# DakeQQ/Text-to-Speech-TTS-ONNX

Hardware: AMD Instinct MI355X
Metric: audio_seconds_per_second (higher is better)
Workload: dtype f32

## Files before the change

### text-to-speech-tts-onnx_amd/csrc/attention.hip

```cpp
#include "common.h"
#include <functional>
#include <map>
#include <mutex>
#include "mfma.h"
#include "f5_kernels.h"
#include "x3_split.h"
#include <type_traits>
#include <string>
#include <algorithm>

namespace mi {

#define ATTN_XCD_MAP                                                                          \
    int bx_ = (int)blockIdx.x, by_ = (int)blockIdx.y;                                         \
    if (xmap) {                                                                               \
        const int l2 = bx_ + (int)gridDim.x * by_, slot = l2 >> 3;                            \
        by_ = (l2 & 7) + 8 * (slot / (int)gridDim.x);                                         \
        bx_ = slot % (int)gridDim.x;                                                          \
    }

#define ATTN_VARLEN_PROLOGUE                                                                  \
    const int NL = VARLEN ? lens[(bh / H) >> 1] : N;                                          \
    const bool dead = VARLEN && (SPLIT2 ? bx_ * 64 : bx_ * 128) >= NL;                        \
    if (dead && blockIdx.z != 0) return;
// ... 226 lines not shown
            } else {
#pragma unroll
                for (int s2 = 0; s2 < 2; ++s2) {
                    T pb[8];
#pragma unroll
                    for (int e = 0; e < 8; ++e) pb[e] = from_f32<T>(p[8 * s2 + e]);
                    const typename MF::Frag bfrag = *reinterpret_cast<const typename MF::Frag*>(pb);
#pragma unroll
                    for (int dt = 0; dt < 2; ++dt) {
                        const T* row = Vs + (dt * 32 + lr) * LDV + kt * 32 + 16 * s2 + 4 * hi;
                        uint2 a2[2];
                        a2[0] = *reinterpret_cast<const uint2*>(row);
                        a2[1] = *reinterpret_cast<const uint2*>(row + 8);
                        oacc[dt] = MF::mma(*reinterpret_cast<const typename MF::Frag*>(a2), bfrag, oacc[dt]);
                    }
                }
            }
        };
        if constexpr (SPLIT2) {
            if (st * KT + (wave & 1) * 32 < NL) tile(wave & 1);
        } else {
#pragma unroll
            for (int kt = 0; kt < KT / 32; ++kt) {
                const int key0 = st * KT + kt * 32;
                if (key0 < NL) tile(kt);
            }
        }
        __syncthreads();
        if (st + 1 < nstage) {
            store_lds();
            __syncthreads();
        }
    }

    bool owner = true;
    if constexpr (SPLIT2) {
        __syncthreads();
        float* comb = reinterpret_cast<float*>(smem);
        float* stats = comb + 2 * 32 * 64;
        static_assert(sizeof(smem) >= (2 * 32 * 64 + 2 * 64 * 2 + 4) * sizeof(float), "merge buffer fits the stage");
        const int grp = wave >> 1;
        owner = !(wave & 1);
        if (!owner) {
            stats[(grp * 64 + lane) * 2] = m_run; stats[(grp * 64 + lane) * 2 + 1] = l_run;
#pragma unroll
            for (int dt = 0; dt < 2; ++dt)
#pragma unroll
                for (int r = 0; r < 16; ++r) comb[((grp * 2 + dt) * 16 + r) * 64 + lane] = oacc[dt][r];
        }
        __syncthreads();
        if (owner) {
            const float m1 = stats[(grp * 64 + lane) * 2], l1 = stats[(grp * 64 + lane) * 2 + 1];
            const float m = fmaxf(m_run, m1);
            const float s0 = m_run == -INFINITY ? 0.f : __builtin_amdgcn_exp2f(m_run - m);
            const float s1 = m1 == -INFINITY ? 0.f : __builtin_amdgcn_exp2f(m1 - m);
            l_run = l_run * s0 + l1 * s1;
            m_run = m;
#pragma unroll
            for (int dt = 0; dt < 2; ++dt)
#pragma unroll
                for (int r = 0; r < 16; ++r) oacc[dt][r] = oacc[dt][r] * s0 + comb[((grp * 2 + dt) * 16 + r) * 64 + lane] * s1;
        }
        const int Z = (int)gridDim.z;
        if (Z > 1) {
            const int z = (int)blockIdx.z;
            const int unit = (int)(by_ * gridDim.x + bx_);
            constexpr int SLOT = 2 * 32 * 64 + 2 * 64 * 2;
            typedef unsigned int u4 __attribute__((ext_vector_type(4)));
            typedef unsigned int u2 __attribute__((ext_vector_type(2)));
            __amdgpu_buffer_rsrc_t rsw = __builtin_amdgcn_make_buffer_rsrc((void*)(ws + (long)unit * Z * SLOT), 0, Z * SLOT * 4, 0x00020000);
            if (owner) {
#pragma unroll
                for (int dt = 0; dt < 2; ++dt)
#pragma unroll
                    for (int g4 = 0; g4 < 4; ++g4) {
                        u4 val;
                        val.x = __float_as_uint(oacc[dt][4 * g4]); val.y = __float_as_uint(oacc[dt][4 * g4 + 1]);
                        val.z = __float_as_uint(oacc[dt][4 * g4 + 2]); val.w = __float_as_uint(oacc[dt][4 * g4 + 3]);
                        __builtin_amdgcn_raw_buffer_store_b128(val, rsw, (z * SLOT + (((grp * 2 + dt) * 4 + g4) * 64 + lane) * 4) * 4, 0, 16);
                    }
                u2 st2; st2.x = __float_as_uint(m_run); st2.y = __float_as_uint(l_run);
                __builtin_amdgcn_raw_buffer_store_b64(st2, rsw, (z * SLOT + 2 * 32 * 64 + (grp * 64 + lane) * 2) * 4, 0, 16);
            }
            asm volatile("s_waitcnt vmcnt(0)" ::: "memory");
            __syncthreads();
            int* ticket = reinterpret_cast<int*>(stats + 2 * 64 * 2);
            if (tid == 0) *ticket = __hip_atomic_fetch_add(cnt + unit, 1, __ATOMIC_RELAXED, __HIP_MEMORY_SCOPE_AGENT);
            __syncthreads();
            if (*ticket != Z - 1) return;
            if (tid == 0) __hip_atomic_store(cnt + unit, 0, __ATOMIC_RELAXED, __HIP_MEMORY_SCOPE_AGENT);
            if (!owner) return;
            float mz[4], lz[4], M = -INFINITY;
#pragma unroll
            for (int zz = 0; zz < 4; ++zz) {
                mz[zz] = -INFINITY; lz[zz] = 0.f;
                if (zz < Z) {
                    if (zz == z) { mz[zz] = m_run; lz[zz] = l_run; }
                    else {
                        const u2 st2 = __builtin_amdgcn_raw_buffer_load_b64(rsw, (zz * SLOT + 2 * 32 * 64 + (grp * 64 + lane) * 2) * 4, 0, 16);
                        mz[zz] = __uint_as_float(st2.x); lz[zz] = __uint_as_float(st2.y);
                    }
                    M = fmaxf(M, mz[zz]);
                }
            }
            f32x16 osum[2];
#pragma unroll
            for (int r = 0; r < 16; ++r) { osum[0][r] = 0.f; osum[1][r] = 0.f; }
            float lsum = 0.f;
#pragma unroll
            for (int zz = 0; zz < 4; ++zz) {
                if (zz >= Z) break;
                const float sc = mz[zz] == -INFINITY ? 0.f : __builtin_amdgcn_exp2f(mz[zz] - M);
                lsum += lz[zz] * sc;
                if (zz == z) {
#pragma unroll
                    for (int dt = 0; dt < 2; ++dt)
#pragma unroll
                        for (int r = 0; r < 16; ++r) osum[dt][r] += oacc[dt][r] * sc;
                } else {
#pragma unroll
                    for (int dt = 0; dt < 2; ++dt)
#pragma unroll
                        for (int g4 = 0; g4 < 4; ++g4) {
                            const u4 val = __builtin_amdgcn_raw_buffer_load_b128(rsw, (zz * SLOT + (((grp * 2 + dt) * 4 + g4) * 64 + lane) * 4) * 4, 0, 16);
                            osum[dt][4 * g4] += __uint_as_float(val.x) * sc; osum[dt][4 * g4 + 1] += __uint_as_float(val.y) * sc;
                            osum[dt][4 * g4 + 2] += __uint_as_float(val.z) * sc; osum[dt][4 * g4 + 3] += __uint_as_float(val.w) * sc;
                        }
                }
            }
            oacc[0] = osum[0]; oacc[1] = osum[1];
            l_run = lsum;
        }
    }
    if (!owner) return;
    const int qr = q0 + lr;
    if (qr < N) {
        const float inv = VARLEN && qr >= NL ? 0.f : 1.0f / l_run;
        const int b = bh / H, h = bh - b * H;
        T* ob = o + ((long)b * N + qr) * H * D + h * D;
#pragma unroll
        for (int dt = 0; dt < 2; ++dt)
#pragma unroll
            for (int g = 0; g < 4; ++g) {
                T vals[4];
#pragma unroll
                for (int e = 0; e < 4; ++e) vals[e] = from_f32<T>(oacc[dt][g * 4 + e] * inv);
                T* dst = ob + dt * 32 + 8 * g + 4 * hi;
                if constexpr (sizeof(T) == 4) *reinterpret_cast<uint4*>(dst) = *reinterpret_cast<const uint4*>(vals);
                else *reinterpret_cast<uint2*>(dst) = *reinterpret_cast<const uint2*>(vals);
            }
    }
}

#if defined(MI355TTS_ATTN_TRACE)
#define TSTAMP(v) do { __builtin_amdgcn_sched_barrier(0); asm volatile("s_memtime %0\n\ts_waitcnt lgkmcnt(0)" : "=s"(v) :: "memory"); __builtin_amdgcn_sched_barrier(0); } while (0)
#define TACC(k, t1, t0) tr_[k] += (t1) - (t0)
#else
#define TSTAMP(v) do { } while (0)
#define TACC(k, t1, t0) do { } while (0)
#endif
template <bool SPLIT2, bool KVP = false, int NP = 3, bool VARLEN = false>
__global__ __launch_bounds__(256, NP == 2 ? 3 : 2) void attn_x3f_kernel(const float* __restrict__ q, const float* __restrict__ k,
                                                       const float* __restrict__ v, float* __restrict__ o, int H, int N,
                                                       float* __restrict__ ws, int* __restrict__ cnt,
                                                       unsigned char* __restrict__ o_planes, int o_np, int xmap = 0,
                                                       int cut1 = 0, int cut2 = 0, int cut3 = 0, const int* __restrict__ lens = nullptr) {
    ATTN_XCD_MAP
    static_assert(NP == 3 || (NP == 2 && KVP), "attn_x3f: the two-plane form reads pre-split K / V");
    using MF = std::conditional_t<NP == 3, Mfma<bf16>, Mfma<f16>>;
    using Frag = typename MF::Frag;
    constexpr int D = 64, KT = 64;
    constexpr int LDK = D + 8, LDV = KT + 4;
    constexpr int KPL = KT * LDK, VPL = D * LDV;
    __shared__ __attribute__((aligned(16))) bf16 smem[NP * KPL + NP * VPL];
    static_assert(sizeof(smem) >= (2 * 32 * 64 + 2 * 64 * 2 + 4) * sizeof(float), "merge buffer fits the stage");
    bf16* Ks = smem;
    bf16* Vs = smem + NP * KPL;

    const int tid = threadIdx.x, wave = tid >> 6, lane = tid & 63, lr = lane & 31, hi = lane >> 5;
    const int bh = by_;
    ATTN_VARLEN_PROLOGUE
    const int q0 = SPLIT2 ? bx_ * 64 + (wave >> 1) * 32 : bx_ * 128 + wave * 32;
    const float* qb = q + (long)bh * N * D;
    const float* kb = k + (long)bh * N * D;
    const long vld = KVP ? (long)((N + 63) / 64 * 64) : (long)((N + 7) / 8 * 8);
    const float* vb = v + (long)bh * D * vld;
    const bf16* kpb = reinterpret_cast<const bf16*>(k) + (long)bh * NP * vld * D;
    const bf16* vpb = reinterpret_cast<const bf16*>(v) + (long)bh * NP * D * vld;

    auto split4 = [&](const float4 a, uint2& w1, uint2& w2, uint2& w3) __attribute__((always_inline)) {
        x3_split_pair(a.x, a.y, w1.x, w2.x, w3.x);
        x3_split_pair(a.z, a.w, w1.y, w2.y, w3.y);
    };
    auto split8 = [&](const float4 a, const float4 b, Frag& f1, Frag& f2, Frag& f3) __attribute__((always_inline)) {
        uint2 a1, a2, a3, b1, b2, b3;
        split4(a, a1, a2, a3); split4(b, b1, b2, b3);
        f1 = __builtin_bit_cast(Frag, x3_u4{a1.x, a1.y, b1.x, b1.y});
        f2 = __builtin_bit_cast(Frag, x3_u4{a2.x, a2.y, b2.x, b2.y});
        f3 = __builtin_bit_cast(Frag, x3_u4{a3.x, a3.y, b3.x, b3.y});
    };

    auto split8h = [&](const float4 a, const float4 b, Frag& f1, Frag& f2) __attribute__((always_inline)) {
        unsigned h[4], l[4];
        x2u_split_pair(a.x, a.y, h[0], l[0]); x2u_split_pair(a.z, a.w, h[1], l[1]);
        x2u_split_pair(b.x, b.y, h[2], l[2]); x2u_split_pair(b.z, b.w, h[3], l[3]);
        f1 = __builtin_bit_cast(Frag, x3_u4{h[0], h[1], h[2], h[3]});
        f2 = __builtin_bit_cast(Frag, x3_u4{l[0], l[1], l[2], l[3]});
    };
    auto split8p = [&](const float4 a, const float4 b, Frag& f1, Frag& f2) __attribute__((always_inline)) {
        unsigned h[4], l[4];
        x2u_split_pair_raw_mix(a.x, a.y, h[0], l[0]); x2u_split_pair_raw_mix(a.z, a.w, h[1], l[1]);
        x2u_split_pair_raw_mix(b.x, b.y, h[2], l[2]); x2u_split_pair_raw_mix(b.z, b.w, h[3], l[3]);
        f1 = __builtin_bit_cast(Frag, x3_u4{h[0], h[1], h[2], h[3]});
        f2 = __builtin_bit_cast(Frag, x3_u4{l[0], l[1], l[2], l[3]});
    };

    Frag qf3[4][NP];
    {
        const int qr = q0 + lr;
        const bool ok = qr < NL;
        constexpr float L2E = 1.4426950408889634f;
#pragma unroll
        for (int ks = 0; ks < 4; ++ks) {
            float4 a = float4{0.f, 0.f, 0.f, 0.f}, b = a;
            if (ok) {
                a = *reinterpret_cast<const float4*>(qb + (long)qr * D + ks * 16 + hi * 8);
                b = *reinterpret_cast<const float4*>(qb + (long)qr * D + ks * 16 + hi * 8 + 4);
            }
            a.x *= L2E; a.y *= L2E; a.z *= L2E; a.w *= L2E; b.x *= L2E; b.y *= L2E; b.z *= L2E; b.w *= L2E;
            if constexpr (NP == 3) split8(a, b, qf3[ks][0], qf3[ks][1], qf3[ks][2]); else split8h(a, b, qf3[ks][0], qf3[ks][1]);
        }
    }

    float4 kreg[KVP ? 1 : 4], vreg[KVP ? 1 : 4];
    constexpr int NU = 2 * NP;
    x3_u4 kpl[KVP ? NU : 1], vpl[KVP ? NU : 1];
    auto load_regs = [&](int key0) {
        if constexpr (KVP) {
#pragma unroll
            for (int i = 0; i < NU; ++i) {
                const int u = tid + i * 256, pl = u >> 9, r = (u & 511) >> 3, c = u & 7;
                kpl[i] = *reinterpret_cast<const x3_u4*>(kpb + ((long)pl * vld + key0 + r) * D + c * 8);
                vpl[i] = *reinterpret_cast<const x3_u4*>(vpb + ((long)pl * D + r) * vld + key0 + c * 8);
            }
            if (key0 + KT > NL) {
#pragma unroll
                for (int i = 0; i < NU; ++i) {
                    const int keep = NL - (key0 + ((tid + i * 256) & 7) * 8);
                    if (keep < 8) {
                        unsigned w[4] = {vpl[i].x, vpl[i].y, vpl[i].z, vpl[i].w};
#pragma unroll
                        for (int e = 0; e < 4; ++e) w[e] &= (2 * e < keep ? 0x0000ffffu : 0u) | (2 * e + 1 < keep ? 0xffff0000u : 0u);
                        vpl[i] = x3_u4{w[0], w[1], w[2], w[3]};
                    }
                }
            }
        } else {
#pragma unroll
        for (int i = 0; i < 4; ++i) {
            const int vi = tid + i * 256;
            const int key = vi >> 4, dv = vi & 15;
            const int d = vi >> 4, kv = vi & 15;
            float4 a = float4{0.f, 0.f, 0.f, 0.f}, b = a;
            if (key0 + key < NL) a = *reinterpret_cast<const float4*>(kb + (long)(key0 + key) * D + dv * 4);
            if (key0 + kv * 4 < NL) b = *reinterpret_cast<const float4*>(vb + (long)d * vld + key0 + kv * 4);
            if constexpr (VARLEN) {
                const int keep = NL - (key0 + kv * 4);
                if (keep < 2) b.y = 0.f;
                if (keep < 3) b.z = 0.f;
                if (keep < 4) b.w = 0.f;
            }
            kreg[i] = a; vreg[i] = b;
        }
        }
    };
    auto store_lds = [&]() {
        if constexpr (KVP) {
#pragma unroll
            for (int i = 0; i < NU; ++i) {
                const int u = tid + i * 256, pl = u >> 9, r = (u & 511) >> 3, c = u & 7;
                *reinterpret_cast<x3_u4*>(Ks + pl * KPL + r * LDK + c * 8) = kpl[i];
                uint2* vd = reinterpret_cast<uint2*>(Vs + pl * VPL + r * LDV + c * 8);
                vd[0] = uint2{vpl[i].x, vpl[i].y}; vd[1] = uint2{vpl[i].z, vpl[i].w};
            }
        } else {
#pragma unroll
        for (int i = 0; i < 4; ++i) {
            const int vi = tid + i * 256;
            const int r = vi >> 4, c = vi & 15;
            uint2 w1, w2, w3;
            split4(kreg[i], w1, w2, w3);
            *reinterpret_cast<uint2*>(Ks + r * LDK + c * 4) = w1;
            *reinterpret_cast<uint2*>(Ks + KPL + r * LDK + c * 4) = w2;
            *reinterpret_cast<uint2*>(Ks + 2 * KPL + r * LDK + c * 4) = w3;
            split4(vreg[i], w1, w2, w3);
            *reinterpret_cast<uint2*>(Vs + r * LDV + c * 4) = w1;
            *reinterpret_cast<uint2*>(Vs + VPL + r * LDV + c * 4) = w2;
            *reinterpret_cast<uint2*>(Vs + 2 * VPL + r * LDV + c * 4) = w3;
        }
        }
    };

    f32x16 oacc[2];
#pragma unroll
    for (int r = 0; r < 16; ++r) { oacc[0][r] = 0.f; oacc[1][r] = 0.f; }
    float m_run = -INFINITY, l_run = 0.f;
#if defined(MI355TTS_ATTN_TRACE)
    unsigned long long tr_[8] = {0, 0, 0, 0, 0, 0, 0, 0}, ta_ = 0, tb_ = 0, tc_ = 0, td_ = 0, te_ = 0, tk_ = 0;
    TSTAMP(tk_);
#endif

    const int nstage_all = dead ? 0 : (NL + KT - 1) / KT;
    int st0 = (int)((long)blockIdx.z * nstage_all / gridDim.z);
    int nstage = (int)((long)(blockIdx.z + 1) * nstage_all / gridDim.z);
    if (cut1 > 0) {
        const int zz = (int)blockIdx.z, ZZ = (int)gridDim.z;
        st0 = zz == 0 ? 0 : zz == 1 ? cut1 : zz == 2 ? cut2 : cut3;
        nstage = zz + 1 == ZZ ? nstage_all : zz == 0 ? cut1 : zz == 1 ? cut2 : cut3;
    }
    if constexpr (VARLEN) { st0 = min(st0, nstage_all); nstage = min(nstage, nstage_all); }
    if (st0 < nstage) {
        load_regs(st0 * KT);
        store_lds();
        __syncthreads();
    }
    constexpr int TA[6] = {0, 1, 2, 0, 1, 0}, TB[6] = {2, 1, 0, 1, 0, 0};
    for (int st = st0; st < nstage; ++st) {
        if (st + 1 < nstage) load_regs((st + 1) * KT);
        auto tile = [&](int kt) {
            const int key0 = st * KT + kt * 32;
            TSTAMP(ta_);
            f32x16 sacc;
#pragma unroll
            for (int r = 0; r < 16; ++r) sacc[r] = 0.f;
#pragma unroll
            for (int ks = 0; ks < 4; ++ks) {
                Frag kf[NP];
#pragma unroll
                for (int pl = 0; pl < NP; ++pl)
                    kf[pl] = *reinterpret_cast<const Frag*>(Ks + pl * KPL + (kt * 32 + lr) * LDK + ks * 16 + hi * 8);
                if constexpr (NP == 3) {
#pragma unroll
                    for (int t = 0; t < 6; ++t) sacc = MF::mma(kf[TA[t]], qf3[ks][TB[t]], sacc);
                } else {
                    sacc = MF::mma(kf[1], qf3[ks][0], sacc);
                    sacc = MF::mma(kf[0], qf3[ks][1], sacc);
                    sacc = MF::mma(kf[0], qf3[ks][0], sacc);
                }
            }
            if (key0 + 32 > NL) {
#pragma unroll
                for (int r = 0; r < 16; ++r) {
                    const int key = key0 + (r & 3) + 8 * (r >> 2) + 4 * hi;
                    if (key >= NL) sacc[r] = -INFINITY;
                }
            }
            float mloc = -INFINITY;
#pragma unroll
            for (int r = 0; r < 16; ++r) mloc = fmaxf(mloc, sacc[r]);
            mloc = xor32_max(mloc);
#if defined(MI355TTS_ATTN_TRACE)
            { const float keep_ = mloc; asm volatile("" :: "v"(keep_)); }
#endif
            TSTAMP(tb_); TACC(0, tb_, ta_);
            float alpha = 1.f;
            if (!__all(mloc - m_run <= 8.0f)) {
                const float m_new = fmaxf(m_run, mloc);
                alpha = __builtin_amdgcn_exp2f(m_run - m_new);
                m_run = m_new;
#pragma unroll
                for (int r = 0; r < 16; ++r) { oacc[0][r] *= alpha; oacc[1][r] *= alpha; }
            }
            typedef float f2 __attribute__((ext_vector_type(2)));
            float p[16];
            f2 ls2 = f2{0.f, 0.f};
            const f2 m2 = f2{m_run, m_run};
#pragma unroll
            for (int r = 0; r < 16; r += 2) {
                const f2 dd = f2{sacc[r], sacc[r + 1]} - m2;
                const f2 e = f2{__builtin_amdgcn_exp2f(dd.x), __builtin_amdgcn_exp2f(dd.y)};
                p[r] = e.x; p[r + 1] = e.y;
                ls2 += e;
            }
            float lsum = ls2.x + ls2.y;
            lsum = xor32_sum(lsum);
            l_run = l_run * alpha + lsum;
#if defined(MI355TTS_ATTN_TRACE)
            { const float keep_ = l_run + p[0] + p[15]; asm volatile("" :: "v"(keep_)); }
#endif
            TSTAMP(tc_); TACC(1, tc_, tb_);
#pragma unroll
            for (int s2 = 0; s2 < 2; ++s2) {
                Frag pf[NP];
                if constexpr (NP == 3)
                    split8(float4{p[8 * s2], p[8 * s2 + 1], p[8 * s2 + 2], p[8 * s2 + 3]},
                           float4{p[8 * s2 + 4], p[8 * s2 + 5], p[8 * s2 + 6], p[8 * s2 + 7]}, pf[0], pf[1], pf[2]);
                else
                    split8p(float4{p[8 * s2], p[8 * s2 + 1], p[8 * s2 + 2], p[8 * s2 + 3]},
                            float4{p[8 * s2 + 4], p[8 * s2 + 5], p[8 * s2 + 6], p[8 * s2 + 7]}, pf[0], pf[1]);
                Frag vf[2][NP];
#pragma unroll
                for (int dt = 0; dt < 2; ++dt)
#pragma unroll
                    for (int pl = 0; pl < NP; ++pl) {
                        const bf16* row = Vs + pl * VPL + (dt * 32 + lr) * LDV + kt * 32 + 16 * s2 + 4 * hi;
                        uint2 a2[2];
                        a2[0] = *reinterpret_cast<const uint2*>(row);
                        a2[1] = *reinterpret_cast<const uint2*>(row + 8);
                        vf[dt][pl] = __builtin_bit_cast(Frag, x3_u4{a2[0].x, a2[0].y, a2[1].x, a2[1].y});
                    }
                if constexpr (NP == 3) {
#pragma unroll
                    for (int t = 0; t < 6; ++t)
#pragma unroll
                        for (int dt = 0; dt < 2; ++dt) oacc[dt] = MF::mma(vf[dt][TA[t]], pf[TB[t]], oacc[dt]);
                } else {
                    oacc[0] = MF::mma(vf[0][1], pf[0], oacc[0]);
                    oacc[1] = MF::mma(vf[1][1], pf[0], oacc[1]);
                    oacc[0] = MF::mma(vf[0][0], pf[1], oacc[0]);
                    oacc[1] = MF::mma(vf[1][0], pf[1], oacc[1]);
                    oacc[0] = MF::mma(vf[0][0], pf[0], oacc[0]);
                    oacc[1] = MF::mma(vf[1][0], pf[0], oacc[1]);
                }
            }
            TSTAMP(td_); TACC(2, td_, tc_);
        };
        if constexpr (SPLIT2) {
            if (st * KT + (wave & 1) * 32 < NL) tile(wave & 1);
        } else {
#pragma unroll
            for (int kt = 0; kt < KT / 32; ++kt) {
                const int key0 = st * KT + kt * 32;
                if (key0 < NL) tile(kt);
            }
        }
        TSTAMP(ta_);
        __syncthreads();
        TSTAMP(tb_); TACC(3, tb_, ta_);
        if (st + 1 < nstage) {
            store_lds();
            TSTAMP(tc_); TACC(4, tc_, tb_);
            __syncthreads();
            TSTAMP(te_); TACC(5, te_, tc_);
        }
    }
#if defined(MI355TTS_ATTN_TRACE)
    TSTAMP(te_);
    if (blockIdx.x == 3 && blockIdx.y == 5 && (threadIdx.x & 63) == 0)
        printf("ATTN_TRACE z %d wave %d stages %d total %llu | S+max %llu exp %llu PV %llu bar1 %llu store %llu bar2 %llu\n", (int)blockIdx.z, wave, nstage - st0,
               te_ - tk_, tr_[0], tr_[1], tr_[2], tr_[3], tr_[4], tr_[5]);
#endif
    bool owner = true;
    constexpr int NG = SPLIT2 ? 2 : 4;
    int grp = wave;
    float* comb = reinterpret_cast<float*>(smem);
    float* stats = comb + 2 * 32 * 64;
    if constexpr (SPLIT2) {
        __syncthreads();
        grp = wave >> 1;
        owner = !(wave & 1);
        if (!owner) {
            stats[(grp * 64 + lane) * 2] = m_run; stats[(grp * 64 + lane) * 2 + 1] = l_run;
#pragma unroll
            for (int dt = 0; dt < 2; ++dt)
#pragma unroll
                for (int r = 0; r < 16; ++r) comb[((grp * 2 + dt) * 16 + r) * 64 + lane] = oacc[dt][r];
        }
        __syncthreads();
        if (owner) {
            const float m1 = stats[(grp * 64 + lane) * 2], l1 = stats[(grp * 64 + lane) * 2 + 1];
            const float m = fmaxf(m_run, m1);
            const float s0 = m_run == -INFINITY ? 0.f : __builtin_amdgcn_exp2f(m_run - m);
            const float s1 = m1 == -INFINITY ? 0.f : __builtin_amdgcn_exp2f(m1 - m);
            l_run = l_run * s0 + l1 * s1;
            m_run = m;
#pragma unroll
            for (int dt = 0; dt < 2; ++dt)
#pragma unroll
                for (int r = 0; r < 16; ++r) oacc[dt][r] = oacc[dt][r] * s0 + comb[((grp * 2 + dt) * 16 + r) * 64 + lane] * s1;
        }
    }
    {
        const int Z = (int)gridDim.z;
        if (Z > 1 && !dead) {
            const int z = (int)blockIdx.z;
            const int unit = (int)(by_ * gridDim.x + bx_);
            constexpr int SLOT = NG * (32 * 64 + 64 * 2);
            typedef unsigned int u4 __attribute__((ext_vector_type(4)));
            typedef unsigned int u2 __attribute__((ext_vector_type(2)));
            __amdgpu_buffer_rsrc_t rsw = __builtin_amdgcn_make_buffer_rsrc((void*)(ws + (long)unit * Z * SLOT), 0, Z * SLOT * 4, 0x00020000);
            if (owner) {
#pragma unroll
                for (int dt = 0; dt < 2; ++dt)
#pragma unroll
                    for (int g4 = 0; g4 < 4; ++g4) {
                        u4 val;
                        val.x = __float_as_uint(oacc[dt][4 * g4]); val.y = __float_as_uint(oacc[dt][4 * g4 + 1]);
                        val.z = __float_as_uint(oacc[dt][4 * g4 + 2]); val.w = __float_as_uint(oacc[dt][4 * g4 + 3]);
                        __builtin_amdgcn_raw_buffer_store_b128(val, rsw, (z * SLOT + (((grp * 2 + dt) * 4 + g4) * 64 + lane) * 4) * 4, 0, 16);
                    }
                u2 st2; st2.x = __float_as_uint(m_run); st2.y = __float_as_uint(l_run);
                __builtin_amdgcn_raw_buffer_store_b64(st2, rsw, (z * SLOT + NG * 32 * 64 + (grp * 64 + lane) * 2) * 4, 0, 16);
            }
            asm volatile("s_waitcnt vmcnt(0)" ::: "memory");
            __syncthreads();
            int* ticket = reinterpret_cast<int*>(stats + 2 * 64 * 2);
            if (tid == 0) *ticket = __hip_atomic_fetch_add(cnt + unit, 1, __ATOMIC_RELAXED, __HIP_MEMORY_SCOPE_AGENT);
            __syncthreads();
            if (*ticket != Z - 1) return;
            if (tid == 0) __hip_atomic_store(cnt + unit, 0, __ATOMIC_RELAXED, __HIP_MEMORY_SCOPE_AGENT);
            if (!owner) return;
            float mz[4], lz[4], M = -INFINITY;
#pragma unroll
            for (int zz = 0; zz < 4; ++zz) {
                mz[zz] = -INFINITY; lz[zz] = 0.f;
                if (zz < Z) {
                    if (zz == z) { mz[zz] = m_run; lz[zz] = l_run; }
                    else {
                        const u2 st2 = __builtin_amdgcn_raw_buffer_load_b64(rsw, (zz * SLOT + NG * 32 * 64 + (grp * 64 + lane) * 2) * 4, 0, 16);
                        mz[zz] = __uint_as_float(st2.x); lz[zz] = __uint_as_float(st2.y);
                    }
                    M = fmaxf(M, mz[zz]);
                }
            }
            f32x16 osum[2];
#pragma unroll
            for (int r = 0; r < 16; ++r) { osum[0][r] = 0.f; osum[1][r] = 0.f; }
            float lsum = 0.f;
#pragma unroll
            for (int zz = 0; zz < 4; ++zz) {
                if (zz >= Z) break;
                const float sc = mz[zz] == -INFINITY ? 0.f : __builtin_amdgcn_exp2f(mz[zz] - M);
                lsum += lz[zz] * sc;
                if (zz == z) {
#pragma unroll
                    for (int dt = 0; dt < 2; ++dt)
#pragma unroll
                        for (int r = 0; r < 16; ++r) osum[dt][r] += oacc[dt][r] * sc;
                } else {
#pragma unroll
                    for (int dt = 0; dt < 2; ++dt)
#pragma unroll
                        for (int g4 = 0; g4 < 4; ++g4) {
                            const u4 val = __builtin_amdgcn_raw_buffer_load_b128(rsw, (zz * SLOT + (((grp * 2 + dt) * 4 + g4) * 64 + lane) * 4) * 4, 0, 16);
                            osum[dt][4 * g4] += __uint_as_float(val.x) * sc; osum[dt][4 * g4 + 1] += __uint_as_float(val.y) * sc;
                            osum[dt][4 * g4 + 2] += __uint_as_float(val.z) * sc; osum[dt][4 * g4 + 3] += __uint_as_float(val.w) * sc;
                        }
                }
            }
            oacc[0] = osum[0]; oacc[1] = osum[1];
            l_run = lsum;
        }
    }
    if (!owner) return;
    const int qr = q0 + lr;
    if (qr < N) {
        const float inv = VARLEN && qr >= NL ? 0.f : 1.0f / l_run;
        const int b = bh / H, h = bh - b * H;
        float* ob = o + ((long)b * N + qr) * H * D + h * D;
        const long row = (long)b * N + qr;
#pragma unroll
        for (int dt = 0; dt < 2; ++dt)
#pragma unroll
            for (int g = 0; g < 4; ++g) {
                float vals[4];
#pragma unroll
                for (int e = 0; e < 4; ++e) vals[e] = (oacc[dt][g * 4 + e] * inv);
                if (o_planes) {
                    uint2 w1, w2, w3;
                    unsigned char* dst = o_planes + x3p_slot_offset(row, h * 8 + dt * 4 + g, (H * D) >> 5, o_np) + 8 * hi;
                    if (o_np == 3) {
                        x3_split_pair(vals[0], vals[1], w1.x, w2.x, w3.x);
                        x3_split_pair(vals[2], vals[3], w1.y, w2.y, w3.y);
                        *reinterpret_cast<uint2*>(dst + 2 * X3P_PLANE) = w3;
                    } else {
                        x2_split_pair(vals[0], vals[1], w1.x, w2.x);
                        x2_split_pair(vals[2], vals[3], w1.y, w2.y);
                    }
                    *reinterpret_cast<uint2*>(dst) = w1;
                    *reinterpret_cast<uint2*>(dst + X3P_PLANE) = w2;
                } else {
                    float* dst = ob + dt * 32 + 8 * g + 4 * hi;
                    *reinterpret_cast<uint4*>(dst) = *reinterpret_cast<const uint4*>(vals);
                }
            }
    }
}

static inline int opt_attn_x3() { const int o = arith_tls().attn_x3; return o >= 0 ? o : (int)opt(OPT_ATTN_F32_X3); }
static inline int opt_attn_np() { const int o = arith_tls().attn_np; return (o == 2 || o == 3) ? o : (int)opt(OPT_ATTN_F32_PLANES); }
long attention_v_ld(int N, int dtype) {
    return (dtype == MI_F32 && opt_attn_x3() != 2) ? 0 : (long)((N + 7) / 8 * 8);
}
bool attention_takes_kv_planes(int N, int BH, int dtype) {
    (void)N; (void)BH;
    return dtype == MI_F32 && opt_attn_x3() == 2 && opt(OPT_ATTN_KV_PLANES) != 0;
}

int attention_kv_planes_format() { return opt_attn_np(); }

bool attention_can_write_planes(int N, int BH, int dtype) {
    (void)N; (void)BH;
    return dtype == MI_F32 && opt_attn_x3() == 2;
}

struct AttnSlices { int Z = 1, cut[3] = {0, 0, 0}; };
static AttnSlices attn_pick_slices(long units, int S, int slots, int zmax) {
    AttnSlices best;
    double best_t = 1e30;
    auto makespan = [&](const int* len, int Z) -> double {
        std::map<double, long> free_at;
        free_at[0.0] = slots;
        double end = 0.0;
        for (int z = 0; z < Z; ++z) {
            const double cost = len[z] + (Z > 1 ? 0.6 : 0.3);
            long left = units;
            while (left > 0) {
                auto it = free_at.begin();
                const long take = std::min(left, it->second);
                const double t = it->first + cost;
                it->second -= take;
                if (it->second == 0) free_at.erase(it);
                free_at[t] += take;
                end = std::max(end, t);
                left -= take;
            }
        }
        return end;
    };
    int len[4];
    for (int Z = 1; Z <= zmax; ++Z) {
        if (S < 2 * Z && Z > 1) break;
        std::function<void(int, int, int)> rec = [&](int i, int left, int cap) {
            if (i == Z - 1) {
                if (left < 1 || left > cap) return;
                len[i] = left;
                const double t = makespan(len, Z);
                if (t < best_t - 1e-9) {
                    best_t = t; best.Z = Z;
                    int acc = 0;
                    for (int c = 0; c < 3; ++c) { acc += c < Z ? len[c] : 0; best.cut[c] = c + 1 < Z ? acc : S; }
                }
                return;
            }
            for (int a = std::min(cap, left - (Z - 1 - i)); a >= (left + (Z - i) - 1) / (Z - i); --a) { len[i] = a; rec(i + 1, left - a, a); }
        };
        rec(0, S, S);
    }
    return best;
}

template <bool SPLIT2, bool KVP, int NP>
static void go_x3f(dim3 grid, hipStream_t s, const void* q, const void* k, const void* v, void* o, int H, int N, float* ws, int* cnt,
                   void* o_planes, int o_np, int xm, int c1, int c2, int c3, const int* lens) {
    const float *qf = (const float*)q, *kf = (const float*)k, *vf = (const float*)v;
    if (lens) prof_kernel_suffix(" + lengths");
    if (lens) hipLaunchKernelGGL((attn_x3f_kernel<SPLIT2, KVP, NP, true>), grid, dim3(256), 0, s, qf, kf, vf, (float*)o, H, N, ws, cnt, (unsigned char*)o_planes, o_np, xm, c1, c2, c3, lens);
    else hipLaunchKernelGGL((attn_x3f_kernel<SPLIT2, KVP, NP>), grid, dim3(256), 0, s, qf, kf, vf, (float*)o, H, N, ws, cnt, (unsigned char*)o_planes, o_np, xm, c1, c2, c3);
}
template <typename T, bool SPLIT2, bool X3S = false, bool REFH = false>
static void go_attn(dim3 grid, hipStream_t s, const void* q, const void* k, const void* v, void* o, int H, int N, float* ws, int* cnt,
                    float sscale, int xm, const int* lens) {
    const T *qt = (const T*)q, *kt = (const T*)k, *vt = (const T*)v;
    if (lens) prof_kernel_suffix(" + lengths");
    if (lens) hipLaunchKernelGGL((attn_kernel<T, SPLIT2, X3S, REFH, true>), grid, dim3(256), 0, s, qt, kt, vt, (T*)o, H, N, ws, cnt, sscale, xm, lens);
    else hipLaunchKernelGGL((attn_kernel<T, SPLIT2, X3S, REFH>), grid, dim3(256), 0, s, qt, kt, vt, (T*)o, H, N, ws, cnt, sscale, xm);
}

void launch_attention(const void* q, const void* k, const void* v, void* o, int BH, int H, int N, int dtype, hipStream_t s,
                      float* ws, long ws_floats, int* cnt, long cnt_n, void* o_planes, int kv_planes, int o_np, float ref_fp16_scale,
                      const int* lens) {
    MI_REQUIRE(ref_fp16_scale == 0.f || (dtype == MI_F16 && ref_fp16_scale > 0.f), "attention: the reference-fp16 score form needs f16 operands");
    MI_REQUIRE(o_np == 2 || o_np == 3, "attention: 2 or 3 output planes");
    MI_REQUIRE(!o_planes || attention_can_write_planes(N, BH, dtype), "attention: panel-plane output needs the fp32 split kernel");
    MI_REQUIRE(!kv_planes || attention_can_write_planes(N, BH, dtype), "attention: pre-split K / V need the fp32 split kernel");
    MI_REQUIRE(kv_planes == 0 || kv_planes == 1 || kv_planes == 2 || kv_planes == 3, "attention: kv_planes is 0, 2 or 3 (1 = 3)");
    MI_REQUIRE(BH % H == 0 && N > 0, "attention: bad shape");
    const double esz = (double)dtype_size(dtype);
    ProfScope ps(FAM_ATTN, s, 4.0 * BH * N * 64.0 * esz, 4.0 * BH * (double)N * N * 64.0);
#define ATTN_LAUNCH(TT, SP, GRID, SSCALE, XM)                                    \
    do {                                                                        \
        prof_set_kernel("attn_kernel<T, " #SP ">", type_label<TT>());           \
        go_attn<TT, SP>(GRID, s, q, k, v, o, H, N, ws, cnt, SSCALE, XM, lens);  \
    } while (0)
    const int xm = (opt(OPT_ATTN_XCD_MAP) != 0 && BH % 8 == 0) ? 1 : 0;
    const int zmax = opt(OPT_ATTN_Z);
    auto pick_z = [&](int zlimit16, bool wide = false) -> int {
        const long units = (long)(wide ? (N + 127) / 128 : (N + 63) / 64) * BH;
        const long slot = wide ? 4 * (32 * 64 + 64 * 2) : 2 * 32 * 64 + 2 * 64 * 2;
        const int nstage = (N + 63) / 64;
        int dev = 0, cus = 256;
        MI_HIP(hipGetDevice(&dev));
        {
            static int cu_count[16] = {0};
            if (!cu_count[dev & 15]) { hipDeviceProp_t pr; MI_HIP(hipGetDeviceProperties(&pr, dev)); cu_count[dev & 15] = pr.multiProcessorCount; }
            cus = cu_count[dev & 15];
        }
        if (opt(OPT_ATTN_Z_FORCE) > 0)
            return (ws && cnt && units * opt(OPT_ATTN_Z_FORCE) * slot <= ws_floats && units <= cnt_n) ? (int)opt(OPT_ATTN_Z_FORCE) : 1;
        int Z = 1;
        double best = 1e30;
        const int zm = dtype == MI_F32 ? zmax : std::min(zmax, zlimit16);
        for (int z = 1; z <= zm; ++z) {
            if (z > 1 && (!ws || !cnt || units * z * slot > ws_floats || units > cnt_n || nstage < 2 * z)) break;
            const double cost = (double)((units * z + cus - 1) / cus) / z * (1.0 + (dtype == MI_F32 ? 0.09 : 0.06) * (z - 1));
            if (cost < best - 1e-9) { best = cost; Z = z; }
        }
        return Z;
    };
    const int z16 = opt(OPT_ATTN_Z16);
    if (dtype == MI_F32) {
        if (opt(OPT_ATTN_SPLIT) && (long)((N + 127) / 128) * BH < 1024 && N >= 64) {
            const bool wide = opt(OPT_ATTN_SPLIT) == 2 && opt_attn_x3() == 2 && kv_planes == 2;
            const int Z = pick_z(1, wide);
            if (wide) {
                AttnSlices sl;
                sl.Z = Z;
                if (opt(OPT_ATTN_LPT) && opt(OPT_ATTN_Z_FORCE) == 0 && Z >= 1 && ws && cnt) {
                    static std::mutex mu;
                    static std::map<std::pair<int, int>, AttnSlices> cache;
                    std::lock_guard<std::mutex> lk(mu);
                    auto key = std::make_pair(N, BH);
                    auto it = cache.find(key);
                    if (it == cache.end()) {
                        int dev = 0, cus = 256;
                        MI_HIP(hipGetDevice(&dev));
                        hipDeviceProp_t pr; MI_HIP(hipGetDeviceProperties(&pr, dev)); cus = pr.multiProcessorCount;
                        const long units = (long)((N + 127) / 128) * BH;
                        const long slot = 4 * (32 * 64 + 64 * 2);
                        int zm = std::min((int)opt(OPT_ATTN_Z), 4);
                        while (zm > 1 && (units * zm * slot > ws_floats || units > cnt_n)) --zm;
                        it = cache.emplace(key, attn_pick_slices(units, (N + 63) / 64, 3 * cus, zm)).first;
                    }
                    sl = it->second;
                    if (const AttnCuts& e = opt_attn_cuts(); e.n) {
                        const int S = (N + 63) / 64, n = e.n;
                        const int* c = e.c;
                        const long units = (long)((N + 127) / 128) * BH;
                        if (n >= 1 && c[0] > 0 && c[0] < S && units * (n + 1) * 4 * (32 * 64 + 64 * 2) <= ws_floats && units <= cnt_n) {
                            sl.Z = n + 1; sl.cut[0] = c[0]; sl.cut[1] = n >= 2 ? c[1] : S; sl.cut[2] = n >= 3 ? c[2] : S;
                        }
                    }
                }
                prof_set_kernel("attn_x3f_kernel<false, pre-split K V, fp16 pairs> + key slices", "", "");
                go_x3f<false, true, 2>(dim3((N + 127) / 128, BH, sl.Z), s, q, k, v, o, H, N, ws, cnt, o_planes, o_np, xm,
                                       sl.Z > 1 ? sl.cut[0] : 0, sl.cut[1], sl.cut[2], lens);
            } else if (opt_attn_x3() == 2) {
                if (kv_planes == 2) {
                    prof_set_kernel("attn_x3f_kernel<true, pre-split K V, fp16 pairs>", "", "");
                    go_x3f<true, true, 2>(dim3((N + 63) / 64, BH, Z), s, q, k, v, o, H, N, ws, cnt, o_planes, o_np, xm, 0, 0, 0, lens);
                } else if (kv_planes) {
                    prof_set_kernel("attn_x3f_kernel<true, pre-split K V>", "", "");
                    go_x3f<true, true, 3>(dim3((N + 63) / 64, BH, Z), s, q, k, v, o, H, N, ws, cnt, o_planes, o_np, 0, 0, 0, 0, lens);
                } else {
                prof_set_kernel("attn_x3f_kernel<true>", "", "");
                go_x3f<true, false, 3>(dim3((N + 63) / 64, BH, Z), s, q, k, v, o, H, N, ws, cnt, o_planes, o_np, 0, 0, 0, 0, lens);
                }
            } else if (opt_attn_x3() == 1) {
                prof_set_kernel("attn_kernel<float, true, x3>", "", "");
                go_attn<float, true, true>(dim3((N + 63) / 64, BH, Z), s, q, k, v, o, H, N, ws, cnt, 1.f, 0, lens);
            } else
                ATTN_LAUNCH(float, true, dim3((N + 63) / 64, BH, Z), 1.f, 0);
        } else if (opt_attn_x3() == 2) {
            if (kv_planes == 2) {
                prof_set_kernel("attn_x3f_kernel<false, pre-split K V, fp16 pairs>", "", "");
                go_x3f<false, true, 2>(dim3((N + 127) / 128, BH), s, q, k, v, o, H, N, ws, cnt, o_planes, o_np, xm, 0, 0, 0, lens);
            } else if (kv_planes) {
                prof_set_kernel("attn_x3f_kernel<false, pre-split K V>", "", "");
                go_x3f<false, true, 3>(dim3((N + 127) / 128, BH), s, q, k, v, o, H, N, ws, cnt, o_planes, o_np, 0, 0, 0, 0, lens);
            } else {
            prof_set_kernel("attn_x3f_kernel<false>", "", "");
            go_x3f<false, false, 3>(dim3((N + 127) / 128, BH), s, q, k, v, o, H, N, ws, cnt, o_planes, o_np, 0, 0, 0, 0, lens);
            }
        } else if (opt_attn_x3() == 1) {
            prof_set_kernel("attn_kernel<float, false, x3>", "", "");
            go_attn<float, false, true>(dim3((N + 127) / 128, BH), s, q, k, v, o, H, N, ws, cnt, 1.f, 0, lens);
        } else
            ATTN_LAUNCH(float, false, dim3((N + 127) / 128, BH), 1.f, 0);
    } else {
        const bool sp = opt(OPT_ATTN_SPLIT) && (long)((N + 127) / 128) * BH < 512 && N >= 64;
        const dim3 grid(sp ? (N + 63) / 64 : (N + 127) / 128, BH, sp ? pick_z(z16) : 1);
        if (dtype == MI_F16 && ref_fp16_scale != 0.f) {
            prof_set_kernel(sp ? "attn_kernel<T, true, reference-fp16 scores>" : "attn_kernel<T, false, reference-fp16 scores>", type_label<f16>());
            if (sp) go_attn<f16, true, false, true>(grid, s, q, k, v, o, H, N, ws, cnt, ref_fp16_scale, 0, lens);
            else go_attn<f16, false, false, true>(grid, s, q, k, v, o, H, N, ws, cnt, ref_fp16_scale, 0, lens);
        } else if (dtype == MI_F16) {
            if (sp) ATTN_LAUNCH(f16, true, grid, 1.f, xm);
            else ATTN_LAUNCH(f16, false, grid, 1.f, xm);
        } else {
            if (sp) ATTN_LAUNCH(bf16, true, grid, 1.f, xm);
            else ATTN_LAUNCH(bf16, false, grid, 1.f, xm);
        }
    }
#undef ATTN_LAUNCH
    MI_HIP(hipGetLastError());
}

}
```

### text-to-speech-tts-onnx_amd/csrc/capi.hip

```cpp
#include "common.h"
#include "bigvgan.h"
#include "f5.h"
#include "gpt.h"
#include "cond.h"
#include <algorithm>
#include <mutex>
#include <exception>

using namespace mi;

struct mi_bigvgan { BigVGAN* impl; std::mutex mu; };
struct mi_f5 { F5* impl; std::mutex mu; };
struct mi_gpt { Gpt* impl; std::mutex mu; };
struct mi_cond { Cond* impl; std::mutex mu; };

template <typename F> static int guard(F&& f, bool exclusive = false) {
    try {
        options_init();
        std::shared_lock<std::shared_mutex> rd(option_lock(), std::defer_lock);
        std::unique_lock<std::shared_mutex> wr(option_lock(), std::defer_lock);
        if (exclusive) wr.lock(); else rd.lock();
        f();
        return MI_OK;
    } catch (const mi::Error& e) {
// ... 121 lines not shown

int mi_bigvgan_forward_latent(mi_bigvgan* h, const float* latent, int T_codes, const float* conds, int64_t n_conds,
                              int16_t* out, float* out_f32, int mem) {
    return guard([&] {
        MI_REQUIRE(h && h->impl, "mi_bigvgan_forward_latent: null handle");
        std::lock_guard<std::mutex> lk_(h->mu);
        MI_REQUIRE(mem == MI_HOST || mem == MI_DEVICE, "mi_bigvgan_forward_latent: bad mem kind");
        h->impl->run_latent(latent, T_codes, conds, (long)n_conds, out_f32, out, mem);
    });
}

static std::vector<int> bigvgan_lengths(const int64_t* lens, int B, int64_t lo, const char* what) {
    MI_REQUIRE(lens && B >= 1, what);
    std::vector<int> v(B);
    for (int b = 0; b < B; ++b) {
        MI_REQUIRE(lens[b] >= lo && lens[b] < (1L << 30), what);
        v[b] = (int)lens[b];
    }
    return v;
}

int mi_bigvgan_forward_ragged(mi_bigvgan* h, int B, const float* mel, const int64_t* frames, int16_t* out_i16, float* out_f32,
                              int64_t out_cap, int64_t* out_lens, int mem) {
    return guard([&] {
        MI_REQUIRE(h && h->impl, "mi_bigvgan_forward_ragged: null handle");
        std::lock_guard<std::mutex> lk_(h->mu);
        MI_REQUIRE(mem == MI_HOST || mem == MI_DEVICE, "mi_bigvgan_forward_ragged: bad mem kind");
        MI_REQUIRE(out_i16, "mi_bigvgan_forward_ragged: null out_i16");
        const std::vector<int> F = bigvgan_lengths(frames, B, 1, "mi_bigvgan_forward_ragged: B >= 1 items of >= 1 frames");
        h->impl->run_ragged(mel, B, F.data(), out_f32, out_i16, (long)out_cap, out_lens, mem);
    });
}

int mi_bigvgan_forward_latent_ragged(mi_bigvgan* h, int B, const float* latent, const int64_t* t_codes, const float* conds,
                                     int64_t n_conds, int16_t* out_i16, float* out_f32, int64_t out_cap, int64_t* out_lens, int mem) {
    return guard([&] {
        MI_REQUIRE(h && h->impl, "mi_bigvgan_forward_latent_ragged: null handle");
        std::lock_guard<std::mutex> lk_(h->mu);
        MI_REQUIRE(mem == MI_HOST || mem == MI_DEVICE, "mi_bigvgan_forward_latent_ragged: bad mem kind");
        MI_REQUIRE(out_i16, "mi_bigvgan_forward_latent_ragged: null out_i16");
        const std::vector<int> T = bigvgan_lengths(t_codes, B, 3, "mi_bigvgan_forward_latent_ragged: B >= 1 items of >= 3 latent rows");
        h->impl->run_latent_ragged(latent, B, T.data(), conds, (long)n_conds, out_f32, out_i16, (long)out_cap, out_lens, mem);
    });
}

int mi_aa_activation1d(const float* x, int B, int C, int T, const float* alpha_log, const float* beta_log,
                       int logscale, int post, int dtype, float* y) {
    return guard([&] {
        MI_REQUIRE(x && y && alpha_log && beta_log && B > 0 && C > 0 && T > 0, "mi_aa_activation1d: bad arguments");
        unit_aa_activation1d(x, B, C, T, alpha_log, beta_log, logscale, post, dtype, y);
    });
}

int mi_aa_conv1d(const float* x, int B, int C, int T, const float* alpha_log, const float* beta_log, int logscale,
                 const float* w, const float* bias, int k, int dilation, const float* res, int dtype, float* y) {
    return guard([&] {
        MI_REQUIRE(x && y && w && bias && alpha_log && beta_log && B > 0 && C > 0 && T > 0 && k > 0 && (k & 1) && dilation > 0,
                   "mi_aa_conv1d: bad arguments");
        unit_aa_conv1d(x, B, C, T, alpha_log, beta_log, logscale, w, bias, k, dilation, res, dtype, 1, y);
    });
}

int mi_conv1d(const float* x, int B, int Cin, int T, const float* w, const float* bias, int Cout, int k, int dilation,
              int padding, int groups, int dtype, float* y) {
    return guard([&] {
        MI_REQUIRE(x && w && y && B > 0 && Cin > 0 && Cout > 0 && T > 0 && k > 0 && dilation > 0 && groups > 0 && padding >= 0,
                   "mi_conv1d: bad arguments");
        unit_conv1d(x, B, Cin, T, w, bias, Cout, k, dilation, padding, groups, dtype, y);
    });
}

int mi_conv_transpose1d(const float* x, int B, int Cin, int T, const float* w, const float* bias, int Cout, int k,
                        int stride, int padding, int dtype, float* y) {
    return guard([&] {
        MI_REQUIRE(x && w && y && B > 0 && Cin > 0 && Cout > 0 && T > 0, "mi_conv_transpose1d: bad arguments");
        unit_conv_transpose1d(x, B, Cin, T, w, bias, Cout, k, stride, padding, dtype, y);
    });
}

int64_t mi_f5_param_count(const int32_t* cfg_i, int n_i, const float* cfg_f, int n_f) {
    int64_t n = -1;
    int rc = guard([&] { n = f5_param_count(parse_f5_cfg(cfg_i, n_i, cfg_f, n_f)); });
    return rc == MI_OK ? n : (int64_t)rc;
}

mi_f5* mi_f5_create(const int32_t* cfg_i, int n_i, const float* cfg_f, int n_f, const float* weights, int64_t n_weights,
                    int dtype, int device) {
    mi_f5* h = nullptr;
    int rc = guard([&] {
        MI_REQUIRE(weights != nullptr, "mi_f5_create: null weights");
        F5Cfg c = parse_f5_cfg(cfg_i, n_i, cfg_f, n_f);
        F5* impl = new F5(c, weights, n_weights, dtype, device);
        h = new mi_f5; h->impl = impl;
    });
    return rc == MI_OK ? h : nullptr;
}

mi_f5* mi_f5_create_mem(const int32_t* cfg_i, int n_i, const float* cfg_f, int n_f, const float* weights, int64_t n_weights,
                        int dtype, int device, int mem) {
    mi_f5* h = nullptr;
    int rc = guard([&] {
        MI_REQUIRE(weights != nullptr && (mem == MI_HOST || mem == MI_DEVICE), "mi_f5_create_mem: null weights / bad mem kind");
        F5Cfg c = parse_f5_cfg(cfg_i, n_i, cfg_f, n_f);
        F5* impl = new F5(c, weights, n_weights, dtype, device, mem);
        h = new mi_f5; h->impl = impl;
    });
    return rc == MI_OK ? h : nullptr;
}

void mi_f5_destroy(mi_f5* h) {
    if (!h) return;
    delete h->impl;
    delete h;
}

struct F5Recover {
    F5* e; int n;
    explicit F5Recover(F5* e_) : e(e_), n(std::uncaught_exceptions()) {}
    ~F5Recover() { if (std::uncaught_exceptions() > n) e->recover(); }
};
#define F5_CHECK(h, mem, name)                                                     \
    MI_REQUIRE((h) && (h)->impl, name ": null handle");                            \
    std::lock_guard<std::mutex> lk_((h)->mu);                                      \
    F5Recover rec_((h)->impl);                                                     \
    ArithScope arith_((h)->impl->arith);                                           \
    MI_REQUIRE((mem) == MI_HOST || (mem) == MI_DEVICE, name ": bad mem kind")

static void copy_out(void* dst, const void* src, size_t bytes, int mem, hipStream_t s) {
    if (!dst) return;
    MI_HIP(hipMemcpyAsync(dst, src, bytes, mem == MI_HOST ? hipMemcpyDeviceToHost : hipMemcpyDeviceToDevice, s));
}

int mi_f5_tables(mi_f5* h, float* time_expand, float* delta_t) {
    return guard([&] {
        MI_REQUIRE(h && h->impl, "mi_f5_tables: null handle");
        std::lock_guard<std::mutex> lk_(h->mu);
        F5& e = *h->impl;
        if (time_expand) std::memcpy(time_expand, e.h_time_expand.data(), e.h_time_expand.size() * 4);
        if (delta_t) std::memcpy(delta_t, e.h_delta.data(), e.h_delta.size() * 4);
    });
}

int64_t mi_f5_info(mi_f5* h, const char* key) {
    int64_t v = -1;
    int rc = guard([&] {
        MI_REQUIRE(h && h->impl && key, "mi_f5_info: null handle / key");
        std::lock_guard<std::mutex> lk_(h->mu);
        F5& e = *h->impl;
        ArithScope as(e.arith);
        const std::string k(key);
        if (k == "f32_arithmetic") v = e.dtype != MI_F32 ? -1 : !gemm_x3_enabled() ? ARITH_NATIVE : (gemm_x3p_enabled() ? e.np : ARITH_BF16X3);
        else if (k == "saturation_events") v = e.sat_events;
        else if (k == "adaln_fold") v = (e.fold_built && e.cfg.ln_fold != 0) ? 1 : 0;
        else MI_REQUIRE(false, "mi_f5_info: unknown key");
    });
    return rc == MI_OK ? v : (int64_t)rc;
}

int mi_f5_preprocess(mi_f5* h, const int16_t* audio, int64_t L, const int32_t* text_ids, int64_t T, int64_t max_duration,
                     const float* noise_in, uint64_t seed, float* noise, float* rope_cos, float* rope_sin,
                     float* cat_mel_text, float* cat_mel_text_drop, int64_t* ref_signal_len, int mem) {
    return guard([&] {
        F5_CHECK(h, mem, "mi_f5_preprocess");
        F5& e = *h->impl;
        MI_REQUIRE(max_duration > 0 && max_duration <= e.cfg.max_len && T >= 0 && T < (1 << 20) && L > 0 && L < (1L << 31),
                   "mi_f5_preprocess: sizes");
        const int N = (int)max_duration;
        const int R = e.preprocess(1, audio, L, text_ids, (int)T, N, noise_in, seed, mem);
        hipStream_t s = e.stream;
        const size_t cd = e.cfg.cond_dim(), D = e.cfg.dim_head;
        copy_out(noise, e.d_noise.p, (size_t)N * e.cfg.mel * 4, mem, s);
        copy_out(rope_cos, e.rope_cos.p, (size_t)N * D * 4, mem, s);
        copy_out(rope_sin, e.rope_sin.p, (size_t)N * D * 4, mem, s);
        copy_out(cat_mel_text, e.d_cmt.p, (size_t)N * cd * 4, mem, s);
        copy_out(cat_mel_text_drop, e.d_cmtd.p, (size_t)N * cd * 4, mem, s);
        MI_HIP(hipStreamSynchronize(s));
        e.finish_call();
        if (ref_signal_len) *ref_signal_len = R;
    });
}

int mi_f5_transformer_step(mi_f5* h, float* noise, const float* cmt, const float* cmtd, int U, int64_t N,
                           int32_t* time_step, int fuse, int mem) {
    return guard([&] {
        F5_CHECK(h, mem, "mi_f5_transformer_step");
        MI_REQUIRE(noise && cmt && cmtd && time_step && fuse >= 1 && U >= 1 && N > 0, "mi_f5_transformer_step: bad arguments");
        F5& e = *h->impl;
        f5_run_checked(e, [&] {
            e.load_cond(noise, cmt, cmtd, U, (int)N, mem);
            e.build_cat_cond(U, (int)N);
            e.steps(U, (int)N, *time_step, fuse);
            MI_HIP(hipStreamSynchronize(e.stream));
        });
        copy_out(noise, e.d_noise.p, (size_t)U * N * e.cfg.mel * 4, mem, e.stream);
        MI_HIP(hipStreamSynchronize(e.stream));
        e.finish_call();
        *time_step += fuse;
    });
}

int mi_f5_sample(mi_f5* h, float* noise, const float* cmt, const float* cmtd, int U, int64_t N, int k0, int n_steps, int mem) {
    return guard([&] {
        F5_CHECK(h, mem, "mi_f5_sample");
        MI_REQUIRE(noise && cmt && cmtd && U >= 1 && N > 0, "mi_f5_sample: bad arguments");
        F5& e = *h->impl;
        f5_run_checked(e, [&] {
            e.load_cond(noise, cmt, cmtd, U, (int)N, mem);
            e.build_cat_cond(U, (int)N);
            e.steps(U, (int)N, k0, n_steps);
            MI_HIP(hipStreamSynchronize(e.stream));
        });
        copy_out(noise, e.d_noise.p, (size_t)U * N * e.cfg.mel * 4, mem, e.stream);
        MI_HIP(hipStreamSynchronize(e.stream));
        e.finish_call();
    });
}

int mi_f5_dit_eval(mi_f5* h, const float* noise, const float* cmt, const float* cmtd, int U, int64_t N, int k, float* pred, int mem) {
    return guard([&] {
        F5_CHECK(h, mem, "mi_f5_dit_eval");
        MI_REQUIRE(noise && cmt && cmtd && pred && U >= 1 && N > 0, "mi_f5_dit_eval: bad arguments");
        F5& e = *h->impl;
        f5_run_checked(e, [&] {
            e.load_cond(noise, cmt, cmtd, U, (int)N, mem);
            e.build_cat_cond(U, (int)N);
            e.dit_eval(U, (int)N, k);
            MI_HIP(hipStreamSynchronize(e.stream));
        });
        copy_out(pred, e.pred_rows(U, (int)N), (size_t)2 * U * N * e.cfg.mel * 4, mem, e.stream);
        MI_HIP(hipStreamSynchronize(e.stream));
        e.finish_call();
    });
}

int mi_f5_decode(mi_f5* h, const float* denoised, int U, int64_t N, int64_t ref_signal_len, int16_t* out, float* out_f32,
                 int64_t* out_len, int mem) {
    return guard([&] {
        F5_CHECK(h, mem, "mi_f5_decode");
        MI_REQUIRE(denoised && (out || out_f32) && U >= 1 && N > 0 && ref_signal_len >= 0 && ref_signal_len < N,
                   "mi_f5_decode: bad arguments");
        F5& e = *h->impl;
        e.load_cond(denoised, nullptr, nullptr, U, (int)N, mem);
        const long len = e.decode(e.d_noise.as<float>(), U, (int)N, (int)ref_signal_len, out_f32 ? e.v_outf.as<float>() : nullptr,
                                  out ? e.v_outi.as<int16_t>() : nullptr);
        copy_out(out, e.v_outi.p, (size_t)U * len * 2, mem, e.stream);
        copy_out(out_f32, e.v_outf.p, (size_t)U * len * 4, mem, e.stream);
        MI_HIP(hipStreamSynchronize(e.stream));
        e.finish_call();
        if (out_len) *out_len = len;
    });
}

int mi_f5_synthesize(mi_f5* h, int U, const int16_t* audio, int64_t L, const int32_t* text_ids, int64_t T,
                     int64_t max_duration, const float* noise_in, uint64_t seed, int16_t* out, int64_t* out_len, int mem) {
    return guard([&] {
        F5_CHECK(h, mem, "mi_f5_synthesize");
        MI_REQUIRE(audio && text_ids && out && U >= 1 && max_duration > 0, "mi_f5_synthesize: bad arguments");
        F5& e = *h->impl;
        const int N = (int)max_duration;
        long len = 0;
        f5_run_checked(e, [&] {
            const int R = e.preprocess(U, audio, L, text_ids, (int)T, N, noise_in, seed, mem);
            e.build_cat_cond(U, N);
            e.steps(U, N, 0, e.cfg.nfe - 1);
            len = e.decode(e.d_noise.as<float>(), U, N, R, nullptr, e.v_outi.as<int16_t>());
            copy_out(out, e.v_outi.p, (size_t)U * len * 2, mem, e.stream);
            MI_HIP(hipStreamSynchronize(e.stream));
        });
        e.finish_call();
        if (out_len) *out_len = len;
    });
}

int mi_f5_synthesize_mel(mi_f5* h, int U, const int16_t* audio, int64_t L, const int32_t* text_ids, int64_t T,
                         int64_t max_duration, const float* noise_in, uint64_t seed, float* mel_out, int64_t* n_frames, int mem) {
    return guard([&] {
        F5_CHECK(h, mem, "mi_f5_synthesize_mel");
        MI_REQUIRE(audio && text_ids && mel_out && U >= 1 && max_duration > 0, "mi_f5_synthesize_mel: bad arguments");
        F5& e = *h->impl;
        const int N = (int)max_duration;
        int F = 0;
        f5_run_checked(e, [&] {
            const int R = e.preprocess(U, audio, L, text_ids, (int)T, N, noise_in, seed, mem);
            const int mel = e.cfg.mel;
            F = N - R;
            MI_REQUIRE(F >= 1, "mi_f5_synthesize_mel: max_duration leaves no generated frames");
            e.build_cat_cond(U, N);
            e.steps(U, N, 0, e.cfg.nfe - 1);
            float* dst = mel_out;
            if (mem == MI_HOST) { e.v_outf.ensure((size_t)U * mel * F * 4); dst = e.v_outf.as<float>(); }
            for (int u = 0; u < U; ++u)
                launch_nlc_to_ncl(e.d_noise.as<float>() + ((size_t)u * N + R) * mel, dst + (size_t)u * mel * F, 1, mel, F, MI_F32, e.stream);
            if (mem == MI_HOST) copy_out(mel_out, dst, (size_t)U * mel * F * 4, mem, e.stream);
            MI_HIP(hipStreamSynchronize(e.stream));
        });
        e.finish_call();
        if (n_frames) *n_frames = F;
    });
}

static std::vector<int> f5_lengths(const int64_t* lens, int U, int64_t lo, int64_t hi, const char* what) {
    MI_REQUIRE(lens && U >= 1, what);
    std::vector<int> v(U);
    for (int u = 0; u < U; ++u) {
        MI_REQUIRE(lens[u] >= lo && lens[u] <= hi, what);
        v[u] = (int)lens[u];
// ... 566 lines not shown
```

### text-to-speech-tts-onnx_amd/csrc/common.h

```cpp
#pragma once
#include <hip/hip_runtime.h>
#include <hip/hip_fp16.h>
#include <cstdint>
#include <cstdio>
#include <cstring>
#include <cmath>
#include <string>
#include <vector>
#include <stdexcept>
#include <map>
#include <shared_mutex>

#include "../../include/mi355tts.h"
#include "options.h"

namespace mi {

struct Error : std::runtime_error {
    int code;
    Error(int c, const std::string& m) : std::runtime_error(m), code(c) {}
};
void set_last_error(const std::string& m);

#define MI_HIP(expr)                                                                              \
    do {                                                                                          \
        hipError_t _e = (expr);                                                                   \
        if (_e != hipSuccess)                                                                     \
            throw mi::Error(MI_EHIP, std::string(#expr) + ": " + hipGetErrorString(_e) + " @" +   \
                                         __FILE__ + ":" + std::to_string(__LINE__));              \
    } while (0)

#define MI_REQUIRE(cond, msg)                                                                     \
    do {                                                                                          \
        if (!(cond)) throw mi::Error(MI_EINVAL, std::string(msg) + " [" #cond "]");               \
    } while (0)

using f16 = _Float16;
using bf16 = __bf16;

template <typename T> struct DT;
template <> struct DT<float> { static constexpr int id = MI_F32; };
template <> struct DT<f16>   { static constexpr int id = MI_F16; };
template <> struct DT<bf16>  { static constexpr int id = MI_BF16; };

inline size_t dtype_size(int dt) { return dt == MI_F32 ? 4 : 2; }

template <typename T> __host__ __device__ inline float to_f32(T v) { return (float)v; }
template <typename T> __host__ __device__ inline T from_f32(float v) { return (T)v; }

struct DevBuf {
    void* p = nullptr;
    size_t bytes = 0;
    DevBuf() = default;
    DevBuf(const DevBuf&) = delete;
    DevBuf& operator=(const DevBuf&) = delete;
    DevBuf(DevBuf&& o) noexcept : p(o.p), bytes(o.bytes) { o.p = nullptr; o.bytes = 0; }
    DevBuf& operator=(DevBuf&& o) noexcept {
        if (this != &o) { release(); p = o.p; bytes = o.bytes; o.p = nullptr; o.bytes = 0; }
        return *this;
    }
    ~DevBuf() { release(); }
    void release() { if (p) { (void)hipFree(p); p = nullptr; bytes = 0; } }
    void ensure(size_t n) {
        if (n <= bytes) return;
        release();
        MI_HIP(hipMalloc(&p, n));
        bytes = n;
    }
    template <typename T> T* as() const { return reinterpret_cast<T*>(p); }
};

void upload_as(DevBuf& dst, const float* src, size_t n, int dt, hipStream_t s);
void upload_f32(DevBuf& dst, const float* src, size_t n, hipStream_t s);

struct BlobReader {
    int mem; hipStream_t s;
    std::vector<std::vector<float>> keep;
    BlobReader(int mem_, hipStream_t s_) : mem(mem_), s(s_) {}
    const float* host(const float* p, size_t n);
    void put(DevBuf& dst, const float* p, size_t n, int dt, size_t dst_off = 0);
};

struct ProfScope {
    int fam; hipStream_t s; hipEvent_t e0 = nullptr, e1 = nullptr; bool on; double bytes_ = 0, flops_ = 0;
    ProfScope(int family, hipStream_t stream, double bytes, double flops);
    ~ProfScope();
};
enum { FAM_CONV_GEMM = 0, FAM_AA = 1, FAM_CONV_POST = 2, FAM_ATTN = 3, FAM_NORM = 4, FAM_OTHER = 5, FAM_COUNT = 6 };
void prof_set_kernel(const char* expr, const char* t = nullptr, const char* to = nullptr);
void prof_kernel_suffix(const char* sfx);
template <typename T> inline const char* type_label();
template <> inline const char* type_label<float>() { return "float"; }
template <> inline const char* type_label<f16>() { return "_Float16"; }
template <> inline const char* type_label<bf16>() { return "__bf16"; }
#define MI_LAUNCH(K, T_, TO_, grid, blk, lds, s, ...)                                                  \
    do {                                                                                               \
        mi::prof_set_kernel(#K, mi::type_label<T_>(), mi::type_label<TO_>());                          \
        hipLaunchKernelGGL(K, grid, blk, lds, s, __VA_ARGS__);                                         \
    } while (0)
void prof_collect();
unsigned prof_mask();

enum Act { ACT_NONE = 0, ACT_GELU_TANH = 1, ACT_GELU_ERF = 2, ACT_MISH = 3, ACT_SILU = 4 };
enum EpiMode { EPI_PLAIN = 0, EPI_CONVT = 1, EPI_QKV_ROPE = 2 };

struct ConvGemm {
    int dtype = MI_F32;
    int out_dtype = -1;
    const void* x = nullptr;
    const void* w = nullptr;
    const float* bias = nullptr;
    void* out = nullptr;
    const void* res = nullptr;
    const float* gate = nullptr;
    long gate_bstride = 0;
    int B = 1, G = 1;
    int T_in = 0;
    int M = 0, N = 0, Cin = 0, taps = 1, dil = 1, pad = 0;
    long x_bstride = 0, x_rstride = 0;
    long out_bstride = 0, out_rstride = 0;
    long x_goff = 0;
    int act = ACT_NONE;
    float alpha = 1.f;
    int accumulate = 0;
    int epi = EPI_PLAIN;
    int u = 1, Cout = 0, padT = 0, T_out = 0;
    const float* rope_cos = nullptr; const float* rope_sin = nullptr; int heads = 0, head_dim = 0;
    const void* rope_pack = nullptr;
    void* out2 = nullptr; void* out3 = nullptr;
    int rows_per_item = 0;
    int m_off = 0;
    long v_ld = 0;
    int kv_planes = 0; long k_ld = 0;
    float* sk_ws = nullptr; int* sk_flags = nullptr; int sk_slots = 0;
    const void* w3 = nullptr;
    const void* xp = nullptr; const void* w3p = nullptr; int np = 3;
    const void* gcp_w = nullptr;
    void* out_planes = nullptr;
    const float* ln_scale = nullptr; void* ln_out = nullptr; float* ln_stats_out = nullptr; int ln_out_np = 0;
    const float* ln_stats_in = nullptr; const float* ln_p = nullptr; const float* ln_c = nullptr; int ln_dim = 0; float ln_eps = 0.f;
    int ln_final = 0;
    int* sat = nullptr;
    const int* lens = nullptr; int len_mul = 1, len_add = 0;
};
constexpr int LN_BLK = 32;
void launch_conv_gemm(const ConvGemm& p, hipStream_t s);
bool gemm_ln_fold_ok(const ConvGemm& p);
constexpr int X3P_PLANE = 128 * 32 * 2;
constexpr int X3P_CHUNK = 3 * X3P_PLANE;
__host__ __device__ inline int x3p_chunk_bytes(int np) { return np * X3P_PLANE; }
__host__ __device__ inline long x3p_slot_offset(long row, int s8, int nch, int np = 3) {
    const int r = (int)(row & 127);
    return ((row >> 7) * nch + (s8 >> 2)) * (long)(np * X3P_PLANE) + r * 64 + (((s8 & 3) ^ ((r >> 2) & 3)) << 4);
}
long x3p_bytes(long rows, long K, int np = 3);
void x3p_split_rows(const float* x, long ld, void* planes, int rows, int K, hipStream_t s, int np = 3, int* sat = nullptr);
size_t gconv_pairs_planes_bytes(int G, int taps);
void gconv_pairs_split_weights(const float* w, void* wp, int G, int taps, hipStream_t s);
size_t gconv16_image_bytes(int G, int taps);
void gconv16_build_weights(const void* w, int dtype, void* img, int G, int taps, hipStream_t s);
int x3p_planes();
bool gemm_x3p_enabled();
bool gemm_x3p_would_run(const ConvGemm& p);
bool gemm_x3p_can_write_planes(const ConvGemm& p);
struct SkWorkspace {
    DevBuf ws, flags; int slots = 0;
    void ensure(int n_slots, hipStream_t s);
    void reset(hipStream_t s);
    bool tripped() const;
    void attach(ConvGemm& g) const { g.sk_ws = ws.as<float>(); g.sk_flags = flags.as<int>(); g.sk_slots = slots; }
};

struct ArithOverride {
    int gemm_x3 = -1;
    int gemm_x3p = -1;
    int planes = -1;
    int n64_pairs = -1;
    int gconv = -1;
    int attn_x3 = -1;
    int attn_np = -1;
};
enum { ARITH_DEFAULT = -1, ARITH_NATIVE = 0, ARITH_PAIRS = 2, ARITH_BF16X3 = 3 };
ArithOverride arith_for(int kind);
ArithOverride& arith_tls();
struct ArithScope {
    ArithOverride saved;
    explicit ArithScope(const ArithOverride& a) : saved(arith_tls()) { arith_tls() = a; }
    ~ArithScope() { arith_tls() = saved; }
    ArithScope(const ArithScope&) = delete;
    ArithScope& operator=(const ArithScope&) = delete;
};

struct AAAct {
    int dtype = MI_F32;
    const void* x = nullptr; void* y = nullptr;
    const float* alpha = nullptr;
    const float* inv_beta = nullptr;
    int B = 1, T = 0, C = 0;
    int post = 0;
    const int* lens = nullptr; int len_mul = 1, len_add = 0;
};
void launch_aa_act(const AAAct& p, hipStream_t s);
const float* aa_filter_host();

struct AAConv {
    int dtype = MI_F32;
    const void* x = nullptr; const void* w = nullptr;
    const float* bias = nullptr;
    const float* snake_alpha = nullptr; const float* snake_inv_beta = nullptr;
    void* out = nullptr; const void* res = nullptr;
    int B = 1, T = 0, C = 0, k = 3, dil = 1;
    float alpha = 1.f; int accumulate = 0;
    const int* lens = nullptr; int len_mul = 1, len_add = 0;
};
void launch_aa_conv(const AAConv& p, hipStream_t s);
void split3_planes(const float* w, void* planes, long n, hipStream_t s);
bool gemm_x3_enabled();

void launch_ncl_to_nlc(const float* x, void* y, int B, int C, int T, int Cpad, int dtype, hipStream_t s);
void launch_ncl_to_nlc_len(const float* x, void* y, int B, int C, int T, int Cpad, int dtype, const int* lens, const long* offs,
                           hipStream_t s);
void launch_nlc_to_ncl(const void* x, float* y, int B, int C, int T, int dtype, hipStream_t s);
void launch_conv_post(const void* x, const float* w , float bias, int B, int T, int C, int dtype,
                      int use_tanh, float* out_f32, int16_t* out_i16, hipStream_t s);
void launch_conv_post_len(const void* x, const float* w, float bias, int B, int T, int C, int dtype, int use_tanh, float* out_f32,
                          int16_t* out_i16, const int* lens, int len_mul, int len_add, const long* offs, hipStream_t s);

}
```

### text-to-speech-tts-onnx_amd/csrc/f5.hip

```cpp
#include "f5.h"

namespace mi {

static int rup(int a, int b) { return (a + b - 1) / b * b; }

F5Cfg parse_f5_cfg(const int32_t* ci, int ni, const float* cf, int nf) {
    MI_REQUIRE(ci && ni >= 21 && ni <= 24 && cf && (nf == 2 || nf == 3),
               "f5 cfg: expected 21 ints (+ up to 3 optional: fp32 arithmetic, mel type, AdaLN fold) + 2 floats (+ the optional attention score scale)");
    F5Cfg c;
    int i = 0;
    c.dim = ci[i++]; c.depth = ci[i++]; c.heads = ci[i++]; c.dim_head = ci[i++]; c.ff_mult = ci[i++]; c.mel = ci[i++];
    c.text_dim = ci[i++]; c.vocab = ci[i++]; c.conv_layers = ci[i++]; c.conv_mult = ci[i++]; c.pos_k = ci[i++];
    c.pos_g = ci[i++]; c.freq_dim = ci[i++]; c.nfe = ci[i++]; c.max_len = ci[i++]; c.n_fft = ci[i++]; c.hop = ci[i++];
    c.sr = ci[i++]; c.vd = ci[i++]; c.vi = ci[i++]; c.vlayers = ci[i++];
    if (ni > 21) c.f32_arith = ci[21];
    if (ni > 22) c.mel_type = ci[22];
    if (ni > 23) c.ln_fold = ci[23];
    MI_REQUIRE(c.f32_arith == ARITH_DEFAULT || c.f32_arith == ARITH_NATIVE || c.f32_arith == ARITH_PAIRS || c.f32_arith == ARITH_BF16X3,
               "f5 cfg: fp32 arithmetic is -1 (process default), 0 (native fp32 MFMA), 2 (fp16 pairs) or 3 (three bf16 planes)");
    MI_REQUIRE((c.mel_type == 0 || c.mel_type == 1) && c.ln_fold >= -1 && c.ln_fold <= 1, "f5 cfg: mel type is 0 (vocos) or 1 (bigvgan); AdaLN fold is -1, 0 or 1");
    c.cfg_strength = cf[0]; c.sway = cf[1];
    if (nf == 3) { c.score_scale = cf[2]; MI_REQUIRE(c.score_scale > 0.f && c.score_scale <= 1e4f, "f5 cfg: attention score scale"); }
    MI_REQUIRE(c.dim == c.heads * c.dim_head, "f5 cfg: dim != heads*dim_head");
    MI_REQUIRE(c.dim_head == 64, "f5: the attention kernel is built for head_dim 64");
// ... 525 lines not shown
    if (mem == MI_HOST)
        for (long i = 0; i < (long)U * T; ++i) {
            const long id = (long)text_ids[i] + 1;
            MI_REQUIRE(id >= 0 && id <= c.vocab, "f5_preprocess: text id out of range");
        }
    MI_HIP(hipSetDevice(device));
    ensure_workspace(U, N);
    hipStream_t s = stream;
    const int nf = c.n_fft, nb = c.nb(), ldm = rup(nb, 8), cd = c.cond_dim();
    const long Lp = L + nf;
    p_audio.ensure((size_t)U * L * 2); p_pad.ensure((size_t)U * Lp * 4 + 64);
    p_spec.ensure((size_t)U * R * 2 * nb * 4); p_mag.ensure((size_t)U * R * ldm * 4); p_mel.ensure((size_t)U * R * c.mel * 4);
    p_tid.ensure((size_t)U * std::max(T, 1) * 4); p_err.ensure(4);
    const int16_t* da = audio;
    const int32_t* dt_ids = text_ids;
    if (mem == MI_HOST) {
        MI_HIP(hipMemcpyAsync(p_audio.p, audio, (size_t)U * L * 2, hipMemcpyHostToDevice, s));
        da = p_audio.as<int16_t>();
        if (T > 0) MI_HIP(hipMemcpyAsync(p_tid.p, text_ids, (size_t)U * T * 4, hipMemcpyHostToDevice, s));
        dt_ids = p_tid.as<int32_t>();
    }
    MI_HIP(hipMemsetAsync(p_err.p, 0, 4, s));
    stft(da, U, L, mel_pad);
    launch_spec_mag(p_spec.as<float>(), p_mag.as<float>(), U * R, nb, ldm, c.mel_type == 1 ? 1e-9f : 0.f, s);
    {
        ConvGemm g;
        g.dtype = MI_F32; g.x = p_mag.p; g.w = fbank.p; g.out = p_mel.p;
        g.B = 1; g.T_in = U * R; g.M = U * R; g.N = c.mel; g.Cin = ldm; g.x_rstride = ldm; g.out_rstride = c.mel;
        launch_conv_gemm(g, s);
    }
    launch_logmel(p_mel.as<float>(), d_cmt.as<float>(), d_cmtd.as<float>(), U, N, R, c.mel, cd, s);
    const int td = c.text_dim, ti = td * c.conv_mult;
    int* dids = p_ids.as<int>();
    launch_text_ids(dt_ids, dids, U, T, N, c.vocab, p_err.as<int>(), s);
    float* tx = p_tx.as<float>(); float* ty = p_ty.as<float>(); float* ty2 = p_ty2.as<float>();
    launch_text_gather(dids, text_emb.as<float>(), text_pos.as<float>(), tx, U, N, td, s);
    const int B2 = 2 * U;
    for (auto& tb : tblocks) {
        launch_dwconv7(tx, ty, tb.dw_w.as<float>(), tb.dw_b.as<float>(), B2, N, td, s);
        launch_rownorm(NORM_LN_AFFINE, ty, ty, MI_F32, tb.ln_w.as<float>(), tb.ln_b.as<float>(), (long)B2 * N, td, 1e-6f, s);
        gemm(MI_F32, ty, (long)N * td, td, td, tb.pw1, ty2, MI_F32, (long)N * ti, ti, B2, N, ACT_GELU_ERF);
        launch_grn(ty2, p_ss.as<float>(), tb.grn_g.as<float>(), tb.grn_b.as<float>(), B2, N, ti, s);
        gemm(MI_F32, ty2, (long)N * ti, ti, ti, tb.pw2, tx, MI_F32, (long)N * td, td, B2, N, ACT_NONE, tx);
        launch_mask_rows(dids, tx, B2, N, td, s);
    }
    for (int u = 0; u < U; ++u) {
        launch_copy2d(tx + (size_t)(2 * u) * N * td, td, d_cmt.as<float>() + (size_t)u * N * cd + c.mel, cd, N, td, MI_F32, s);
        launch_copy2d(tx + (size_t)(2 * u + 1) * N * td, td, d_cmtd.as<float>() + (size_t)u * N * cd + c.mel, cd, N, td, MI_F32, s);
    }
    const size_t nn = (size_t)N * c.mel;
    if (noise_in) {
        MI_HIP(hipMemcpyAsync(d_noise.p, noise_in, (size_t)U * nn * 4, mem == MI_HOST ? hipMemcpyHostToDevice : hipMemcpyDeviceToDevice, s));
    } else {
        h_noise.resize((size_t)U * nn);
        for (int u = 0; u < U; ++u) host_normal(h_noise.data() + (size_t)u * nn, nn, seed + (uint64_t)u);
        MI_HIP(hipMemcpyAsync(d_noise.p, h_noise.data(), h_noise.size() * 4, hipMemcpyHostToDevice, s));
    }
    return R;
}

void F5::stft(const int16_t* audio_dev, int U, long L, int pad) {
    const F5Cfg& c = cfg;
    if (pad < 0) pad = c.n_fft / 2;
    const int nf = c.n_fft, nb = c.nb(), R = (int)((L + 2 * pad - nf) / c.hop) + 1;
    const long Lp = L + 2 * pad;
    launch_pad_reflect(audio_dev, p_pad.as<float>(), U, L, pad, stream);
    ConvGemm g;
    g.dtype = MI_F32; g.x = p_pad.p; g.w = stft_w.p; g.out = p_spec.p;
    g.B = U; g.T_in = R; g.M = R; g.N = 2 * nb; g.Cin = nf; g.x_rstride = c.hop; g.x_bstride = Lp;
    g.out_rstride = 2 * nb; g.out_bstride = (long)R * 2 * nb;
    launch_conv_gemm(g, stream);
}

void F5::check_text_ids() {
    if (sk.tripped()) {
        recover();
        MI_REQUIRE(false, "f5: a split-tile hand-off timed out on the device (workspace reset; results of this call discarded)");
    }
    if (!p_err.p) return;
    int flag = 0;
    MI_HIP(hipMemcpy(&flag, p_err.p, 4, hipMemcpyDeviceToHost));
    if (flag != 0) {
        MI_HIP(hipMemset(p_err.p, 0, 4));
        MI_REQUIRE(false, "f5_preprocess: text id out of range");
    }
}

void F5::load_cond(const float* noise, const float* cmt, const float* cmtd, int U, int N, int mem) {
    const F5Cfg& c = cfg;
    MI_REQUIRE(U > 0 && N > 0 && N <= c.max_len, "f5: bad batch / length");
    MI_HIP(hipSetDevice(device));
    ensure_workspace(U, N);
    const hipMemcpyKind kind = mem == MI_HOST ? hipMemcpyHostToDevice : hipMemcpyDeviceToDevice;
    if (noise && noise != d_noise.p) MI_HIP(hipMemcpyAsync(d_noise.p, noise, (size_t)U * N * c.mel * 4, kind, stream));
    if (cmt && cmt != d_cmt.p) MI_HIP(hipMemcpyAsync(d_cmt.p, cmt, (size_t)U * N * c.cond_dim() * 4, kind, stream));
    if (cmtd && cmtd != d_cmtd.p) MI_HIP(hipMemcpyAsync(d_cmtd.p, cmtd, (size_t)U * N * c.cond_dim() * 4, kind, stream));
}

void F5::build_cat_cond(int U, int N) {
    const F5Cfg& c = cfg;
    const size_t es = dtype_size(dtype);
    const int cd = c.cond_dim(), ld = cat_ld();
    for (int u = 0; u < U; ++u)
        for (int br = 0; br < 2; ++br) {
            const float* src = (br == 0 ? d_cmt.as<float>() : d_cmtd.as<float>()) + (size_t)u * N * cd;
            char* dst = (char*)cat.p + ((size_t)(2 * u + br) * N * ld + c.mel) * es;
            launch_copy2d(src, cd, dst, ld, N, cd, dtype, stream);
        }
}

void F5::dit_eval(int U, int N, int k, const int* lens) {
    const F5Cfg& c = cfg;
    MI_REQUIRE(k >= 0 && k < c.nfe, "f5: time step out of range");
    hipStream_t s = stream;
    const int B = 2 * U, d = c.dim, ld = cat_ld(), ff = c.ff(), H = c.heads, D = c.dim_head;
    const long rows = (long)B * N;
    const float* modk = mod.as<float>() + (size_t)k * mod_ld;
    launch_cat_noise(d_noise.as<float>(), cat.p, U, N, c.mel, ld, dtype, s);
    gemm(dtype, cat.p, (long)N * ld, ld, ld, in_proj, h32.p, MI_F32, (long)N * d, d, B, N);
    const void* hin = h32.p;
    if (dtype != MI_F32) { launch_copy2d(h32.as<float>(), d, hT.p, d, rows, d, dtype, s); hin = hT.p; }
    const long row_bytes = (long)d * (long)dtype_size(dtype);
    if (lens) launch_zero_pad_rows(const_cast<void*>(hin), row_bytes, B, N, lens, 2, s);
    {
        ConvGemm g;
        g.dtype = dtype; g.x = hin; g.w = gconv1.w.p; g.bias = gconv1.b.as<float>(); g.out = c1.p;
        g.B = B; g.G = c.pos_g; g.T_in = N; g.M = N; g.N = d / c.pos_g; g.Cin = d / c.pos_g; g.taps = c.pos_k; g.pad = c.pos_k / 2;
        g.x_bstride = (long)N * d; g.x_rstride = d; g.x_goff = d / c.pos_g; g.out_bstride = (long)N * d; g.out_rstride = d;
        g.act = ACT_MISH; g.sat = d_sat.as<int>(); g.gcp_w = gconv1.w3p.p;
        launch_conv_gemm(g, s);
        if (lens) launch_zero_pad_rows(c1.p, row_bytes, B, N, lens, 2, s);
        g.x = c1.p; g.w = gconv2.w.p; g.bias = gconv2.b.as<float>(); g.out = X.p; g.out_dtype = MI_F32; g.res = h32.p; g.gcp_w = gconv2.w3p.p;
        launch_conv_gemm(g, s);
    }
    const bool f32 = dtype == MI_F32;
    auto lin = [&](const Lin& L, int K, int odt, void* out) {
        ConvGemm g;
        g.dtype = dtype; g.out_dtype = odt; g.w = L.w.p; g.w3 = L.w3.p; g.bias = L.b.p ? L.b.as<float>() : nullptr; g.out = out;
        g.B = 1; g.T_in = (int)rows; g.M = (int)rows; g.N = L.n; g.Cin = K; g.taps = 1;
        g.x_bstride = rows * K; g.x_rstride = K; g.out_bstride = rows * L.n; g.out_rstride = L.n;
        g.sat = d_sat.as<int>();
        sk.attach(g);
        return g;
    };
    auto with_planes = [&](ConvGemm& g, const Lin& L, const void* xp) { g.xp = xp; g.w3p = L.w3p.p; g.np = np; };
    auto qkv_gemm = [&](const Block& bk) {
        ConvGemm g = lin(bk.qkv, d, -1, qb.p);
        g.out2 = kb.p; g.out3 = vb.p; g.rows_per_item = N;
        g.epi = EPI_QKV_ROPE; g.rope_cos = rope_cos.as<float>(); g.rope_sin = rope_sin.as<float>(); g.rope_pack = rope_pack.p; g.heads = H; g.head_dim = D;
        g.v_ld = attention_v_ld(N, dtype);
        return g;
    };
    const int kvp_fmt = attention_kv_planes_format();
    bool planes = false, fold = false;
    {
        const Block& b0 = blocks[0];
        if (f32 && Ap.p && gemm_x3p_enabled() && b0.qkv.w3p.p && b0.o.w3p.p && b0.ff1.w3p.p && b0.ff2.w3p.p && attention_can_write_planes(N, B * H, dtype)) {
            ConvGemm gq = qkv_gemm(b0); gq.x = Ub.p; with_planes(gq, b0.qkv, Ap.p);
            ConvGemm go = lin(b0.o, d, MI_F32, X.p); go.x = Ob.p; go.res = X.p; go.gate = modk; with_planes(go, b0.o, Ap.p);
            ConvGemm g1 = lin(b0.ff1, d, dtype, Hff.p); g1.x = Ub.p; g1.act = ACT_GELU_TANH; with_planes(g1, b0.ff1, Ap.p);
            ConvGemm g2 = lin(b0.ff2, ff, MI_F32, X.p); g2.x = Hff.p; g2.res = X.p; g2.gate = modk; with_planes(g2, b0.ff2, Ap2.p);
            planes = gemm_x3p_would_run(gq) && gemm_x3p_would_run(go) && gemm_x3p_can_write_planes(g1) && gemm_x3p_would_run(g2);
        }
        if (fold_built && cfg.ln_fold != 0 && (planes || !f32) && (!f32 || ApN.p) && ln_stats.p && (f32 || ln_fin.p)) {
            ConvGemm gq = qkv_gemm(b0); gq.x = Ub.p;
            ConvGemm go = lin(b0.o, d, MI_F32, X.p); go.x = Ob.p; go.res = X.p; go.gate = modk;
            ConvGemm g1 = lin(b0.ff1, d, dtype, Hff.p); g1.x = Ub.p; g1.act = ACT_GELU_TANH;
            ConvGemm g2 = lin(b0.ff2, ff, MI_F32, X.p); g2.x = Hff.p; g2.res = X.p; g2.gate = modk;
            if (f32) { with_planes(gq, b0.qkv, ApN.p); with_planes(go, b0.o, Ap.p); with_planes(g1, b0.ff1, ApN.p); with_planes(g2, b0.ff2, Ap2.p); }
            fold = gemm_ln_fold_ok(gq) && gemm_ln_fold_ok(go) && gemm_ln_fold_ok(g1) && gemm_ln_fold_ok(g2);
        }
    }
    float* stats = ln_stats.as<float>();
    const float* lnk = fold ? ln_tab.as<float>() + (size_t)k * ln_ld : nullptr;
    const bool fin = fold && !f32;
    auto finalize = [&] { if (fin) launch_ln_finalize(stats, ln_fin.as<float>(), rows, d, 1e-6f, s); };
    auto consume = [&](ConvGemm& g) { g.ln_stats_in = fin ? ln_fin.as<float>() : stats; g.ln_final = fin ? 1 : 0; g.ln_dim = d; g.ln_eps = 1e-6f; };
    if (fold) {
        launch_ln_prologue(X.as<float>(), f32 ? ApN.p : Ub.p, dtype, np, stats, modk + d, rows, d, d_sat.as<int>(), s);
        finalize();
    }
    for (int i = 0; i < c.depth; ++i) {
        const Block& bk = blocks[i];
        const float* m = modk + (size_t)i * 6 * d;
        if (fold) {
            const float* lt = lnk + (size_t)i * ln_blk;
            const bool kvp = f32 && attention_takes_kv_planes(N, B * H, dtype);
            {
                ConvGemm g = qkv_gemm(bk);
                g.x = Ub.p; g.bias = nullptr;
                if (f32) with_planes(g, bk.qkv, ApN.p);
                consume(g); g.ln_p = lt; g.ln_c = lt + 3 * d;
                if (kvp) { g.kv_planes = kvp_fmt; g.k_ld = g.v_ld = (long)((N + 63) / 64 * 64); }
                launch_conv_gemm(g, s);
            }
            launch_attention(qb.p, kb.p, vb.p, Ob.p, B * H, H, N, dtype, s, attn_ws.as<float>(), attn_ws_floats, attn_cnt.as<int>(), attn_cnt_n,
                             f32 ? Ap.p : nullptr, kvp ? kvp_fmt : 0, np, cfg.score_scale != 1.f ? cfg.score_scale : 0.f, lens);
            {
                ConvGemm g = lin(bk.o, d, MI_F32, X.p);
                g.x = Ob.p; g.res = X.p; g.gate = m + 2 * d;
                if (f32) with_planes(g, bk.o, Ap.p);
                g.ln_scale = m + 4 * d; g.ln_out = f32 ? ApN.p : Ub.p; g.ln_out_np = np; g.ln_stats_out = stats;
                launch_conv_gemm(g, s);
                finalize();
            }
            {
                ConvGemm g = lin(bk.ff1, d, dtype, Hff.p);
                g.x = Ub.p; g.bias = nullptr; g.act = ACT_GELU_TANH;
                if (f32) { with_planes(g, bk.ff1, ApN.p); g.out_planes = Ap2.p; }
                consume(g); g.ln_p = lt + 6 * d; g.ln_c = lt + 6 * d + ff;
                launch_conv_gemm(g, s);
            }
            {
                ConvGemm g = lin(bk.ff2, ff, MI_F32, X.p);
                g.x = Hff.p; g.res = X.p; g.gate = m + 5 * d;
                if (f32) with_planes(g, bk.ff2, Ap2.p);
                if (i + 1 < c.depth) {
                    g.ln_scale = m + 6 * d + d; g.ln_out = f32 ? ApN.p : Ub.p; g.ln_out_np = np; g.ln_stats_out = stats;
                }
                launch_conv_gemm(g, s);
                if (i + 1 < c.depth) finalize();
            }
            continue;
        }
        if (planes) {
            const bool kvp = attention_takes_kv_planes(N, B * H, dtype);
            launch_rownorm_x3p(X.as<float>(), Ap.p, m + d, m, rows, d, 1e-6f, s, np, d_sat.as<int>());
            {
                ConvGemm g = qkv_gemm(bk);
                g.x = Ub.p; with_planes(g, bk.qkv, Ap.p);
                if (kvp) { g.kv_planes = kvp_fmt; g.k_ld = g.v_ld = (long)((N + 63) / 64 * 64); }
                MI_REQUIRE(gemm_x3p_would_run(g), "f5: the QKV layer left the panel-plane kernel between the decision and the launch");
                launch_conv_gemm(g, s);
            }
            launch_attention(qb.p, kb.p, vb.p, Ob.p, B * H, H, N, dtype, s, attn_ws.as<float>(), attn_ws_floats, attn_cnt.as<int>(), attn_cnt_n,
                             Ap.p, kvp ? kvp_fmt : 0, np, 0.f, lens);
            {
                ConvGemm g = lin(bk.o, d, MI_F32, X.p);
                g.x = Ob.p; g.res = X.p; g.gate = m + 2 * d; with_planes(g, bk.o, Ap.p);
                MI_REQUIRE(gemm_x3p_would_run(g), "f5: the O projection left the panel-plane kernel between the decision and the launch");
                launch_conv_gemm(g, s);
            }
            launch_rownorm_x3p(X.as<float>(), Ap.p, m + 4 * d, m + 3 * d, rows, d, 1e-6f, s, np, d_sat.as<int>());
            {
                ConvGemm g = lin(bk.ff1, d, dtype, Hff.p);
                g.x = Ub.p; g.act = ACT_GELU_TANH; with_planes(g, bk.ff1, Ap.p); g.out_planes = Ap2.p;
                MI_REQUIRE(gemm_x3p_would_run(g), "f5: the FF1 layer left the panel-plane kernel between the decision and the launch");
                launch_conv_gemm(g, s);
            }
            {
                ConvGemm g = lin(bk.ff2, ff, MI_F32, X.p);
                g.x = Hff.p; g.res = X.p; g.gate = m + 5 * d; with_planes(g, bk.ff2, Ap2.p);
                MI_REQUIRE(gemm_x3p_would_run(g), "f5: the FF2 layer left the panel-plane kernel between the decision and the launch");
                launch_conv_gemm(g, s);
            }
            continue;
        }
        launch_rownorm(NORM_LN_MOD, X.as<float>(), Ub.p, dtype, m + d, m, rows, d, 1e-6f, s);
        {
            ConvGemm g = qkv_gemm(bk);
            g.x = Ub.p; g.x_bstride = (long)B * N * d;
            launch_conv_gemm(g, s);
        }
        launch_attention(qb.p, kb.p, vb.p, Ob.p, B * H, H, N, dtype, s, attn_ws.as<float>(), attn_ws_floats, attn_cnt.as<int>(), attn_cnt_n,
                         nullptr, 0, np, cfg.score_scale != 1.f ? cfg.score_scale : 0.f, lens);
        gemm(dtype, Ob.p, (long)N * d, d, d, bk.o, X.p, MI_F32, (long)N * d, d, B, N, ACT_NONE, X.p, m + 2 * d);
        launch_rownorm(NORM_LN_MOD, X.as<float>(), Ub.p, dtype, m + 4 * d, m + 3 * d, rows, d, 1e-6f, s);
        gemm(dtype, Ub.p, (long)N * d, d, d, bk.ff1, Hff.p, dtype, (long)N * ff, ff, B, N, ACT_GELU_TANH);
        gemm(dtype, Hff.p, (long)N * ff, ff, ff, bk.ff2, X.p, MI_F32, (long)N * d, d, B, N, ACT_NONE, X.p, m + 5 * d);
    }
    const float* mf = modk + (size_t)c.depth * 6 * d;
    launch_rownorm(NORM_LN_MOD, X.as<float>(), Ub.p, dtype, mf, mf + d, rows, d, 1e-6f, s);
    if (proj_parts > 1) {
        ConvGemm g;
        g.dtype = dtype; g.out_dtype = MI_F32; g.x = Ub.p; g.w = proj_out_k.w.p; g.bias = proj_out_k.b.as<float>(); g.out = pred.p;
        g.B = 1; g.G = proj_parts; g.T_in = (int)rows; g.M = (int)rows; g.N = c.mel; g.Cin = d / proj_parts; g.taps = 1;
        g.x_bstride = rows * d; g.x_rstride = d; g.x_goff = d / proj_parts;
        g.out_bstride = rows * proj_parts * c.mel; g.out_rstride = (long)proj_parts * c.mel;
        launch_conv_gemm(g, s);
    } else
        gemm(dtype, Ub.p, (long)N * d, d, d, proj_out, pred.p, MI_F32, (long)N * c.mel, c.mel, B, N);
}

const float* F5::pred_rows(int U, int N) {
    if (proj_parts <= 1) return pred.as<float>();
    launch_sum_parts(pred.as<float>(), pred_sum.as<float>(), (long)2 * U * N, cfg.mel, proj_parts, stream);
    return pred_sum.as<float>();
}

void F5::steps_eager(int U, int N, int k0, int nsteps, const int* lens) {
    for (int k = k0; k < k0 + nsteps; ++k) {
        dit_eval(U, N, k, lens);
        if (lens)
            launch_cfg_update_len(d_noise.as<float>(), pred.as<float>(), U, N, cfg.mel, cfg.cfg_strength, delta_t.as<float>(), k, lens, stream,
                                  proj_parts);
        else
            launch_cfg_update(d_noise.as<float>(), pred.as<float>(), U, N, cfg.mel, cfg.cfg_strength, delta_t.as<float>(), k, stream, proj_parts);
    }
}

void F5::drop_graphs() {
    for (auto& kv : graphs)
        if (kv.second.exec) (void)hipGraphExecDestroy(kv.second.exec);
    graphs.clear();
}

void F5::recover() {
    (void)hipSetDevice(device);
    (void)hipStreamSynchronize(stream);
    (void)hipGetLastError();
    drop_graphs();
    sk.reset(stream);
    if (attn_cnt.p && attn_cnt_n > 0) {
        (void)hipMemsetAsync(attn_cnt.p, 0, (size_t)attn_cnt_n * 4, stream);
        (void)hipStreamSynchronize(stream);
    }
    if (p_err.p) (void)hipMemset(p_err.p, 0, 4);
    if (d_sat.p) (void)hipMemset(d_sat.p, 0, 4);
}

void F5::steps(int U, int N, int k0, int nsteps, const int* lens) {
    MI_REQUIRE(k0 >= 0 && nsteps >= 0 && k0 + nsteps <= cfg.nfe - 1, "f5: step range exceeds the NFE grid");
    MI_REQUIRE(!lens || lens == d_len.p, "f5: ragged steps read the handle's length table");
    if (!use_graph || prof_mask() != 0 || nsteps < 2) { steps_eager(U, N, k0, nsteps, lens); return; }
    if (graph_epoch != option_epoch()) { drop_graphs(); graph_epoch = option_epoch(); }
    GraphEntry& e = graphs[{U, N, k0, nsteps, lens ? 1 : 0}];
    if (e.exec) { MI_HIP(hipGraphLaunch(e.exec, stream)); return; }
    if (e.uses++ == 0) { steps_eager(U, N, k0, nsteps, lens); return; }
    hipGraph_t graph = nullptr;
    MI_HIP(hipStreamBeginCapture(stream, hipStreamCaptureModeThreadLocal));
    try {
        steps_eager(U, N, k0, nsteps, lens);
    } catch (...) {
        (void)hipStreamEndCapture(stream, &graph);
        if (graph) (void)hipGraphDestroy(graph);
        throw;
    }
    MI_HIP(hipStreamEndCapture(stream, &graph));
    hipError_t err = hipGraphInstantiate(&e.exec, graph, nullptr, nullptr, 0);
    (void)hipGraphDestroy(graph);
    if (err != hipSuccess) { e.exec = nullptr; use_graph = false; steps_eager(U, N, k0, nsteps, lens); return; }
    MI_HIP(hipGraphLaunch(e.exec, stream));
}

int F5::ref_frames(long L) const {
    const int mel_pad = cfg.mel_type == 1 ? (cfg.n_fft - cfg.hop) / 2 : cfg.n_fft / 2;
    return (int)((L + 2 * mel_pad - cfg.n_fft) / cfg.hop) + 1;
}

const int* F5::set_lengths(int U, const int* lens) {
    h_len.assign(lens, lens + U);
    if ((size_t)U * 4 > d_len.bytes) { drop_graphs(); d_len.ensure((size_t)std::max(U, 8) * 4); }
    MI_HIP(hipMemcpyAsync(d_len.p, h_len.data(), (size_t)U * 4, hipMemcpyHostToDevice, stream));
    return d_len.as<int>();
}

void F5::zero_pad_rows_cond(int U, int Nmax, const int* lens) {
    const size_t cd = cfg.cond_dim(), M = cfg.mel;
    for (int u = 0; u < U; ++u) {
        const size_t n = (size_t)lens[u], pad = (size_t)(Nmax - lens[u]);
        if (pad == 0) continue;
        MI_HIP(hipMemsetAsync(d_noise.as<float>() + ((size_t)u * Nmax + n) * M, 0, pad * M * 4, stream));
        MI_HIP(hipMemsetAsync(d_cmt.as<float>() + ((size_t)u * Nmax + n) * cd, 0, pad * cd * 4, stream));
        MI_HIP(hipMemsetAsync(d_cmtd.as<float>() + ((size_t)u * Nmax + n) * cd, 0, pad * cd * 4, stream));
    }
}

void F5::preprocess_ragged(int U, const int16_t* audio, const long* L, const int32_t* text_ids, const int* T, const int* Ns, int Nmax,
                           const float* noise_in, uint64_t seed, int mem, int* R) {
    const size_t M = cfg.mel, cd = cfg.cond_dim();
    MI_HIP(hipSetDevice(device));
    ensure_workspace(U, Nmax);
    std::vector<long> a_off(U + 1, 0), t_off(U + 1, 0), n_off(U + 1, 0);
    for (int u = 0; u < U; ++u) { a_off[u + 1] = a_off[u] + L[u]; t_off[u + 1] = t_off[u] + T[u]; n_off[u + 1] = n_off[u] + Ns[u]; }
    const hipMemcpyKind d2d = hipMemcpyDeviceToDevice;
    for (int u = U - 1; u >= 0; --u) {
        const int N = Ns[u];
        R[u] = preprocess(1, audio + a_off[u], L[u], text_ids + t_off[u], T[u], N, noise_in ? noise_in + (size_t)n_off[u] * M : nullptr,
                          seed + (uint64_t)u, mem);
        if (u > 0) {
            MI_HIP(hipMemcpyAsync(d_noise.as<float>() + (size_t)u * Nmax * M, d_noise.p, (size_t)N * M * 4, d2d, stream));
            MI_HIP(hipMemcpyAsync(d_cmt.as<float>() + (size_t)u * Nmax * cd, d_cmt.p, (size_t)N * cd * 4, d2d, stream));
            MI_HIP(hipMemcpyAsync(d_cmtd.as<float>() + (size_t)u * Nmax * cd, d_cmtd.p, (size_t)N * cd * 4, d2d, stream));
        }
        MI_HIP(hipStreamSynchronize(stream));
        check_text_ids();
    }
    zero_pad_rows_cond(U, Nmax, Ns);
}
// ... 34 lines not shown
```

### text-to-speech-tts-onnx_amd/csrc/f5_kernels.h

```cpp
#pragma once
#include "common.h"

namespace mi {

enum { NORM_LN_MOD = 0, NORM_LN_AFFINE = 1, NORM_L2 = 2 };
void launch_rownorm(int mode, const float* x, void* y, int out_dtype, const float* a, const float* b, long rows, int D,
                    float eps, hipStream_t s);
void launch_rownorm_len(int mode, const float* x, void* y, int out_dtype, const float* a, const float* b, int items, int Fmax, int D,
                        float eps, const int* lens, const long* offs, hipStream_t s);
void launch_rownorm_x3p(const float* x, void* planes, const float* a, const float* b, long rows, int D, float eps, hipStream_t s,
                        int np = 3, int* sat = nullptr);
void launch_ln_prologue(const float* x, void* aout, int a_dtype, int np, float* stats, const float* scale, long rows, int D, int* sat,
                        hipStream_t s);
void launch_ln_finalize(const float* partials, float* fin, long rows, int D, float eps, hipStream_t s);
void launch_ln_gather(const float* mod, long mod_ld, long col_scale, long col_shift, float* G, float* S, int steps, int D, hipStream_t s);
void launch_cast_to_f32(const void* src, int dtype, float* dst, long n, hipStream_t s);
void launch_absmax(const float* x, long n, unsigned* out_bits, hipStream_t s);
void launch_dwconv7(const float* x, float* y, const float* w, const float* bias, int B, int T, int C, hipStream_t s);
void launch_grn(float* y, float* ss_scratch, const float* gamma, const float* beta, int B, int T, int C, hipStream_t s);
void launch_text_gather(const int* ids, const float* emb, const float* pos, float* out, int U, int N, int C, hipStream_t s);
void launch_text_ids(const int32_t* in, int* out, int U, int T, int N, int vocab, int* err, hipStream_t s);
void launch_mask_rows(const int* ids, float* x, int V, int N, int C, hipStream_t s);
void launch_copy2d(const float* src, long lds_, void* dst, long ldd, long rows, int cols, int out_dtype, hipStream_t s);
void launch_pad_reflect(const int16_t* a, float* out, int U, long L, int half, hipStream_t s);
void launch_spec_mag(const float* spec, float* mag, int F, int nb, int ldm, float eps, hipStream_t s);
void launch_logmel(const float* melraw, float* cmt, float* cmtd, int U, int N, int R, int M, int ld, hipStream_t s);
void launch_vocos_head(const float* sp, float* c, long rows, int nb, int ldc, hipStream_t s);
void launch_istft_ola(const float* frames, const float* wsi, int U, int F, int nfft, int hop, float* out_f,
                      int16_t* out_i, hipStream_t s);
void launch_cat_noise(const float* noise, void* cat, int U, int N, int M, int ldc, int dtype, hipStream_t s);
void launch_cfg_update(float* noise, const float* pred, int U, int N, int M, float cfg, const float* dt, int k, hipStream_t s, int parts = 1);
void launch_cfg_update_len(float* noise, const float* pred, int U, int N, int M, float cfg, const float* dt, int k, const int* len,
                           hipStream_t s, int parts = 1);
void launch_zero_pad_rows(void* x, long row_bytes, int items, int N, const int* len, int per, hipStream_t s);
void launch_sum_parts(const float* in, float* out, long rows, int M, int parts, hipStream_t s);

void launch_attention(const void* q, const void* k, const void* v, void* o, int BH, int H, int N, int dtype, hipStream_t s,
                      float* ws = nullptr, long ws_floats = 0, int* cnt = nullptr, long cnt_n = 0, void* o_planes = nullptr,
                      int kv_planes = 0, int o_np = 3, float ref_fp16_scale = 0.f, const int* lens = nullptr);
bool attention_takes_kv_planes(int N, int BH, int dtype);
int attention_kv_planes_format();
bool attention_can_write_planes(int N, int BH, int dtype);
long attention_v_ld(int N, int dtype);

}
```

### text-to-speech-tts-onnx_amd/csrc/gemm_conv.hip

```cpp
#include "common.h"
#include <mutex>
#include "mfma.h"
#include "gemm_epilogue.h"

namespace mi {

template <typename T, typename TO, int BM, int BN, int WGM, int WGN, int KC, bool LENS = false>
__global__ __launch_bounds__(256, 2) void conv_gemm_kernel(const ConvGemmDev p) {
    using MF = Mfma<T>;
    constexpr int KP = MF::KP;
    constexpr int VEC = 16 / (int)sizeof(T);
    constexpr int KV = KC / VEC;
    constexpr int RPP = 256 / KV;
    constexpr int AP = (BM + RPP - 1) / RPP, BP = (BN + RPP - 1) / RPP;
    constexpr int LDA = KC + (sizeof(T) == 4 ? 1 : 8);
    constexpr int WM = BM / WGM, WN = BN / WGN, TM = WM / 32, TN = WN / 32;
    static_assert(WGM * WGN == 4 && WM % 32 == 0 && WN % 32 == 0, "tile");
    static_assert(KC % (2 * KP) == 0, "KC");

    __shared__ __attribute__((aligned(16))) T smem[(BM + BN) * LDA];
    T* As = smem;
    T* Bs = smem + BM * LDA;

    const int tid = threadIdx.x;
// ... 601 lines not shown
                    else MI_LAUNCH_LN((conv_gemm_dma_kernel<T, TO, false, 2, 64>), (conv_gemm_dma_kernel<T, TO, false, 2, 64, false, true>), T, TO, g2, blk, 0, s, e);
                    MI_HIP(hipGetLastError());
                    return;
                }
                if (opt(OPT_GEMM_RING4) && (long)g1.x * g1.y <= opt(OPT_GEMM_RING4_MAX) && nchunks >= 6) {
                    if (!LENS && e.lds_epi) MI_LAUNCH((conv_gemm_dma_kernel<T, TO, true, 4>), T, TO, g1, blk, 0, s, e);
                    else MI_LAUNCH_LN((conv_gemm_dma_kernel<T, TO, false, 4>), (conv_gemm_dma_kernel<T, TO, false, 4, 128, false, true>), T, TO, g1, blk, 0, s, e);
                } else if (!LENS && e.lds_epi) MI_LAUNCH((conv_gemm_dma_kernel<T, TO, true>), T, TO, g1, blk, 0, s, e);
                else MI_LAUNCH_LN((conv_gemm_dma_kernel<T, TO, false>), (conv_gemm_dma_kernel<T, TO, false, 2, 128, false, true>), T, TO, g1, blk, 0, s, e);
                MI_HIP(hipGetLastError());
                return;
            }
        }
        if constexpr (sizeof(T) == 4) {
            if (opt(OPT_GEMM_USE_DMA) && opt(OPT_GEMM_F32_DMA) && d.Cin % 4 == 0 && d.K % d.Cin == 0) {
                no_fold();
                ConvGemmDev e = d;
                e.Tm = (d.M + 127) / 128; e.Tn = (d.N + 127) / 128; e.RT = B * e.Tm;
                e.RC = opt(OPT_GEMM_XCD_ORDER) ? (e.RT + 7) / 8 : 0;
                e.use_buf = buf_ok(d, 4);
                if (opt(OPT_GEMM_F32_SMALL) && (long)e.RT * e.Tn * d.G < opt(OPT_GEMM_F32_SMALL_MAX)) {
                    e.Tm = (d.M + 63) / 64; e.Tn = (d.N + 63) / 64; e.RT = B * e.Tm; e.RC = 0;
                    dim3 g2(e.RT * e.Tn, d.G);
                    if (!LENS && e.lds_epi) MI_LAUNCH((conv_gemm_dma_kernel<T, TO, true, 2, 64>), T, TO, g2, blk, 0, s, e);
                    else MI_LAUNCH_LN((conv_gemm_dma_kernel<T, TO, false, 2, 64>), (conv_gemm_dma_kernel<T, TO, false, 2, 64, false, true>), T, TO, g2, blk, 0, s, e);
                    MI_HIP(hipGetLastError());
                    return;
                }
                dim3 g1(e.RC > 0 ? 8 * e.RC * e.Tn : e.RT * e.Tn, d.G);
                if (!LENS && e.lds_epi) MI_LAUNCH((conv_gemm_dma_kernel<T, TO, true>), T, TO, g1, blk, 0, s, e);
                else MI_LAUNCH_LN((conv_gemm_dma_kernel<T, TO, false>), (conv_gemm_dma_kernel<T, TO, false, 2, 128, false, true>), T, TO, g1, blk, 0, s, e);
                MI_HIP(hipGetLastError());
                return;
            }
        }
        no_fold();
        MI_LAUNCH_LN((conv_gemm_kernel<T, TO, 128, 128, 2, 2, KC>), (conv_gemm_kernel<T, TO, 128, 128, 2, 2, KC, true>), T, TO, grid, blk, 0, s, d);
    }
    MI_HIP(hipGetLastError());
}

static bool x3_eligible(const ConvGemm& p) {
    if (!opt_x3() || !p.w3 || p.dtype != MI_F32 || (p.out_dtype >= 0 && p.out_dtype != MI_F32)) return false;
    if (!p.sk_ws || !p.sk_flags || p.sk_slots < 256 || p.B != 1 || p.G != 1 || p.taps != 1 || p.pad != 0 || p.Cin % 32 != 0 || p.M <= 128) return false;
    if (p.epi != EPI_PLAIN && p.epi != EPI_QKV_ROPE) return false;
    if (p.epi == EPI_QKV_ROPE && !(p.head_dim == 64 && p.rope_pack && (p.rows_per_item == 0 ? p.M : p.rows_per_item) >= 64 &&
                                   ((uintptr_t)p.out % 16) == 0 && ((uintptr_t)p.out2 % 16) == 0 && ((uintptr_t)p.out3 % 16) == 0)) return false;
    const long tiles = (long)((p.M + 127) / 128) * ((p.N + 127) / 128);
    if (tiles < 64 || tiles > g_sk_max_tiles) return false;
    const long a_bytes = (((long)p.T_in - 1) * p.x_rstride + p.Cin) * 4, b_bytes = (long)3 * p.N * p.Cin * 2;
    return opt(OPT_GEMM_BUF) && a_bytes + (long)512 * p.x_rstride * 4 < 0x7fff0000L && b_bytes < 0x7fff0000L;
}

static bool x3p_eligible(const ConvGemm& p) {
    if (!opt_x3p() || !p.xp || !p.w3p) return false;
    ConvGemm q = p;
    q.w3 = p.w3p;
    if (!x3_eligible(q)) return false;
    const long nch = p.Cin / 32;
    const long chb = x3p_chunk_bytes(p.np);
    return (p.np == 2 || p.np == 3) && p.N % 128 == 0 && ((long)(p.M + 127) / 128) * nch * chb < 0x7fff0000L && ((long)p.N / 128) * nch * chb < 0x7fff0000L;
}

bool gemm_x3p_would_run(const ConvGemm& p) { return x3p_eligible(p) && p.B == 1 && p.G == 1; }

static bool lds_epi_for(const ConvGemm& p, int odt, bool use_x3) {
    if (!opt(OPT_GEMM_LDS_EPI)) return false;
    const int ch = 16 / (int)dtype_size(odt);
    const bool qkv_lds = p.epi == EPI_QKV_ROPE && p.head_dim == 64 && (dtype_size(odt) == 2 || use_x3) && p.G == 1 &&
                         (p.rows_per_item == 0 ? p.M : p.rows_per_item) >= 64 && ((uintptr_t)p.out % 16) == 0 &&
                         ((uintptr_t)p.out2 % 16) == 0;
    if (qkv_lds) return true;
    return p.epi == EPI_PLAIN && p.taps == 1 && p.N >= 1024 && p.N % ch == 0 && p.out_rstride % ch == 0 &&
           p.out_bstride % ch == 0 && ((uintptr_t)p.out % 16) == 0 && (!p.res || ((uintptr_t)p.res % 16) == 0);
}

bool gemm_x3p_can_write_planes(const ConvGemm& p) {
    return gemm_x3p_would_run(p) && p.epi == EPI_PLAIN && !p.res && !p.gate && !p.accumulate && p.alpha == 1.f && p.N % 32 == 0 &&
           lds_epi_for(p, MI_F32, true);
}

bool gemm_ln_fold_ok(const ConvGemm& p) {
    const int odt = p.out_dtype < 0 ? p.dtype : p.out_dtype;
    if (p.B != 1 || p.G != 1 || p.taps != 1 || p.pad != 0 || p.alpha != 1.f || p.accumulate || p.gate_bstride != 0 || p.N % 64 != 0 || p.M <= 128) return false;
    if (p.epi != EPI_PLAIN && p.epi != EPI_QKV_ROPE) return false;
    if (p.dtype == MI_F32) return gemm_x3p_would_run(p) && lds_epi_for(p, odt, true);
    if (!lds_epi_for(p, odt, false) || !opt(OPT_GEMM_USE_DMA) || p.Cin % 64 != 0 || p.N <= 64) return false;
    if (opt(OPT_GEMM_USE_DMA3) && p.Cin > opt(OPT_GEMM_DMA3_K_MIN)) return false;
    return true;
}

void launch_conv_gemm(const ConvGemm& p_in, hipStream_t s) {
    ConvGemm p = p_in;
    if (!p.lens && p.B > 1 && p.taps == 1 && p.G == 1 && p.pad == 0 && p.epi == EPI_PLAIN && p.M == p.T_in && p.gate_bstride == 0 &&
        p.x_bstride == (long)p.M * p.x_rstride && p.out_bstride == (long)p.M * p.out_rstride) {
        p.T_in = p.M = p.B * p.M; p.B = 1;
    }
    const int odt = p.out_dtype < 0 ? p.dtype : p.out_dtype;
    const bool split_plain = p.epi == EPI_PLAIN && p.gate_bstride == 0 && !p.out_planes && !p.accumulate;
    const bool split_qkv = p.epi == EPI_QKV_ROPE && p.rows_per_item >= 32 && !p.kv_planes && p.m_off == 0;
    if (!p.lens && opt(OPT_GEMM_ROW_SPLIT) != 0 && opt(OPT_GEMM_PH8) != 0 && dtype_size(p.dtype) == 2 && p.B == 1 && p.G == 1 && p.taps == 1 && p.pad == 0 &&
        (split_plain || split_qkv) && p.M == p.T_in && p.N % 256 == 0 && !p.xp) {
        int dev = 0, cus = 256;
        MI_HIP(hipGetDevice(&dev));
        {
            static int cu_count[16] = {0};
            if (!cu_count[dev & 15]) { hipDeviceProp_t pr; MI_HIP(hipGetDeviceProperties(&pr, dev)); cu_count[dev & 15] = pr.multiProcessorCount; }
            cus = cu_count[dev & 15];
        }
        const long ntn = p.N / 256;
        long gc = cus, t = ntn;
        while (t) { const long u = gc % t; gc = t; t = u; }
        const long rstep = cus / gc;
        const long r = (p.M / 256) / rstep * rstep;
        const long rem = p.M - 256 * r;
        const long rem_tiles = (rem + 255) / 256 * ntn;
        if (r >= 1 && rem > 0 && rem_tiles * 2 < cus && r * ntn >= opt(OPT_GEMM_PH8_MIN_TILES)) {
            ConvGemm a = p, b = p;
            a.M = a.T_in = (int)(256 * r);
            b.M = b.T_in = (int)rem;
            b.x = (const char*)p.x + (size_t)(256 * r) * p.x_rstride * dtype_size(p.dtype);
            if (split_qkv) b.m_off = (int)(256 * r);
            else {
                b.out = (char*)p.out + (size_t)(256 * r) * p.out_rstride * dtype_size(odt);
                if (p.res) b.res = (const char*)p.res + (size_t)(256 * r) * p.out_rstride * dtype_size(odt);
                if (p.ln_stats_in) b.ln_stats_in = p.ln_stats_in + (size_t)(256 * r) * (p.ln_final ? 1 : p.ln_dim / LN_BLK) * 2;
                if (p.ln_stats_out) {
                    b.ln_stats_out = p.ln_stats_out + (size_t)(256 * r) * (p.N / LN_BLK) * 2;
                    b.ln_out = (char*)p.ln_out + (size_t)(256 * r) * p.N * dtype_size(p.dtype);
                }
            }
            launch_conv_gemm(a, s);
            launch_conv_gemm(b, s);
            return;
        }
    }
    const int vec = 16 / (int)dtype_size(p.dtype);
    MI_REQUIRE(p.Cin % vec == 0, "conv_gemm: Cin must be a multiple of the 16-byte vector");
    MI_REQUIRE(p.x_rstride % vec == 0 && p.x_bstride % vec == 0 && p.x_goff % vec == 0, "conv_gemm: x strides");
    MI_REQUIRE(((uintptr_t)p.x % 16) == 0 && ((uintptr_t)p.w % 16) == 0, "conv_gemm: 16-byte alignment");
    MI_REQUIRE(odt == p.dtype || odt == MI_F32, "conv_gemm: out dtype");
    MI_REQUIRE(p.M > 0 && p.N > 0 && p.B > 0 && p.G > 0, "conv_gemm: empty problem");
    ConvGemmDev d;
    d.x = p.x; d.w = p.w; d.bias = p.bias; d.out = p.out; d.res = p.res; d.gate = p.gate;
    d.gate_bstride = p.gate_bstride;
    d.G = p.G; d.T_in = p.T_in; d.M = p.M; d.N = p.N; d.Cin = p.Cin; d.K = p.taps * p.Cin; d.dil = p.dil; d.pad = p.pad;
    d.x_bstride = p.x_bstride; d.x_rstride = p.x_rstride; d.out_bstride = p.out_bstride; d.out_rstride = p.out_rstride;
    d.x_goff = p.x_goff;
    d.act = p.act; d.alpha = p.alpha; d.accumulate = p.accumulate; d.epi = p.epi;
    d.u = p.u; d.Cout = p.Cout; d.padT = p.padT; d.T_out = p.T_out;
    d.rope_cos = p.rope_cos; d.rope_sin = p.rope_sin; d.rope_pack = p.rope_pack; d.heads = p.heads; d.head_dim = p.head_dim;
    d.out2 = p.out2; d.out3 = p.out3; d.v_ld = p.v_ld; d.Mb = p.rows_per_item; d.m_off = p.m_off;
    MI_REQUIRE(p.m_off == 0 || (p.epi == EPI_QKV_ROPE && p.rows_per_item >= 32), "conv_gemm: a row offset needs the flattened QKV epilogue");
    d.kv_planes = p.kv_planes; d.k_ld = p.k_ld;
    d.sk_ws = p.sk_ws; d.sk_flags = p.sk_flags; d.sk_slots = p.sk_slots;
    const bool use_x3p = x3p_eligible(p);
    const bool use_x3 = use_x3p || x3_eligible(p);
    d.w3 = use_x3 ? p.w3 : nullptr;
    d.xp = use_x3p ? p.xp : nullptr; d.w3p = use_x3p ? p.w3p : nullptr; d.np = p.np;
    d.out_planes = nullptr;
    if (p.out_planes) {
        MI_REQUIRE(use_x3p && p.epi == EPI_PLAIN && !p.res && !p.gate && !p.accumulate && p.alpha == 1.f && p.N % 32 == 0,
                   "conv_gemm: out_planes needs the panel-plane kernel and a plain bias + activation epilogue");
        d.out_planes = p.out_planes;
    }
    d.ln_scale = p.ln_scale; d.ln_out = p.ln_out; d.ln_stats_out = p.ln_stats_out; d.ln_out_np = p.ln_out_np;
    d.ln_stats_in = p.ln_stats_in; d.ln_p = p.ln_p; d.ln_c = p.ln_c; d.ln_dim = p.ln_dim; d.ln_eps = p.ln_eps; d.ln_final = p.ln_final;
    d.sat = p.sat;
    d.lens = p.lens; d.len_mul = p.len_mul; d.len_add = p.len_add;
    if (p.lens)
        MI_REQUIRE((p.epi == EPI_PLAIN || p.epi == EPI_CONVT) && !p.ln_stats_in && !p.ln_stats_out && !p.out_planes && !p.xp && !p.w3 &&
                       !p.gcp_w && p.G == 1 && !p.gate,
                   "conv_gemm: a launch with lengths is a plain or ConvTranspose1d convolution over padded slabs");
    if (p.ln_stats_in || p.ln_stats_out) {
        MI_REQUIRE(!(p.ln_stats_in && p.ln_stats_out), "conv_gemm: a launch is the producer OR the consumer of the AdaLN fold");
        MI_REQUIRE(p.B == 1 && p.G == 1 && p.taps == 1 && p.alpha == 1.f && !p.accumulate && p.gate_bstride == 0 && p.N % 64 == 0,
                   "conv_gemm: AdaLN fold needs a plain linear layer over one M axis");
        if (p.ln_stats_out)
            MI_REQUIRE(p.epi == EPI_PLAIN && odt == MI_F32 && p.res && p.ln_scale && p.ln_out && p.act == ACT_NONE && !p.out_planes &&
                           ((uintptr_t)p.ln_out % 16) == 0 && ((uintptr_t)p.ln_stats_out % 8) == 0 && ((uintptr_t)p.ln_scale % 16) == 0 &&
                           (p.dtype != MI_F32 || p.ln_out_np == p.np),
                       "conv_gemm: AdaLN fold producer: fp32 residual rows out, (1 + scale) and the next operand's buffer");
        else
            MI_REQUIRE(p.ln_p && p.ln_c && p.ln_dim >= 128 && p.ln_dim % 128 == 0 && !p.res && !p.gate && ((uintptr_t)p.ln_stats_in % 8) == 0 && (p.ln_final || ((uintptr_t)p.ln_stats_in % 16) == 0) &&
                           ((uintptr_t)p.ln_p % 16) == 0 && ((uintptr_t)p.ln_c % 16) == 0 && (odt != MI_F32 || p.epi == EPI_QKV_ROPE || p.out_planes),
                       "conv_gemm: AdaLN fold consumer: statistics, W(1 + scale) and W shift + b vectors");
    }
    d.tail_tiles = 0; d.tail_split = 1;
    d.use_buf = 0;
    {
        int dev = 0;
        MI_HIP(hipGetDevice(&dev));
        {
            static std::mutex zero_mu;
            std::lock_guard<std::mutex> lk(zero_mu);
            DevBuf& z = g_zero_page[dev & 15];
            if (!z.p) { z.ensure(4096); MI_HIP(hipMemset(z.p, 0, 4096)); MI_HIP(hipDeviceSynchronize()); }
            d.zero = z.p;
        }
        d.dbg = (int)env_int("MI355TTS_GEMM_DBG", 0);
        d.lds_epi = (!p.lens && lds_epi_for(p, odt, use_x3)) ? 1 : 0;
    }
    if (p.ln_stats_in || p.ln_stats_out)
        MI_REQUIRE(d.lds_epi && (p.dtype != MI_F32 || use_x3p), "conv_gemm: the AdaLN fold lives in the LDS-staged epilogues of linear_x3p / linear_ph8 / conv_gemm_dma (gemm_ln_fold_ok)");
    if (p.kv_planes) MI_REQUIRE(p.epi == EPI_QKV_ROPE && p.dtype == MI_F32 && d.lds_epi && p.v_ld > 0 && p.k_ld > 0 && p.v_ld % 8 == 0,
                                "conv_gemm: kv_planes needs the fp32 LDS-staged QKV epilogue with transposed V");
    if (p.epi == EPI_CONVT) MI_REQUIRE(p.Cout > 0 && p.N == p.u * p.Cout, "conv_gemm: convT shape");
    if (p.epi == EPI_QKV_ROPE)
        MI_REQUIRE((p.rows_per_item == 0 || p.rows_per_item >= 32) && p.G == 1 && p.heads > 0 && p.head_dim % 2 == 0 && p.N == 3 * p.heads * p.head_dim && p.N % 32 == 0 &&
                       p.rope_cos && p.rope_sin && p.out2 && p.out3, "conv_gemm: qkv-rope epilogue arguments");

    const double esz = (double)dtype_size(p.dtype), osz = (double)dtype_size(odt);
    const double rows_out = p.epi == EPI_CONVT ? (double)p.T_out : (double)p.M;
    const double ncols = p.epi == EPI_CONVT ? (double)p.Cout : (double)p.N * p.G;
    double bytes = (double)p.B * p.T_in * (double)p.Cin * p.G * esz + (double)p.G * p.N * d.K * esz +
                   (double)p.B * rows_out * ncols * osz * (1.0 + (p.res ? 1.0 : 0.0) + (p.accumulate ? 1.0 : 0.0));
    double flops = 2.0 * p.B * p.G * (double)p.M * p.N * d.K;
    ProfScope ps(FAM_CONV_GEMM, s, bytes, flops);

    if (!p.lens && p.dtype == MI_F32 && opt_x3() != 0 && opt_n64_pairs() != 0 && opt_gconv() != 0 && opt(OPT_GEMM_USE_DMA) && launch_gconv_pairs(p, s)) return;
    if (!p.lens && p.dtype != MI_F32 && p.gcp_w && opt(OPT_GEMM_USE_DMA) && launch_gconv16(p, s)) return;
    if (p.lens) {
        MI_REQUIRE(odt == p.dtype, "conv_gemm: a launch with lengths writes the engine dtype");
        if (p.dtype == MI_F32) dispatch_tiles<float, float, true>(d, p.B, s);
        else if (p.dtype == MI_F16) dispatch_tiles<f16, f16, true>(d, p.B, s);
        else dispatch_tiles<bf16, bf16, true>(d, p.B, s);
        return;
    }
    if (p.dtype == MI_F32) {
        dispatch_tiles<float, float, false>(d, p.B, s);
    } else if (p.dtype == MI_F16) {
        if (odt == MI_F32) dispatch_tiles<f16, float, false>(d, p.B, s);
        else dispatch_tiles<f16, f16, false>(d, p.B, s);
    } else {
        if (odt == MI_F32) dispatch_tiles<bf16, float, false>(d, p.B, s);
        else dispatch_tiles<bf16, bf16, false>(d, p.B, s);
    }
}

void SkWorkspace::ensure(int n_slots, hipStream_t s) {
    if (n_slots <= slots) return;
    ws.ensure((size_t)n_slots * 128 * 128 * 4);
    flags.ensure((size_t)n_slots * 4);
    MI_HIP(hipMemsetAsync(flags.p, 0, (size_t)n_slots * 4, s));
    MI_HIP(hipStreamSynchronize(s));
    slots = n_slots;
}

bool SkWorkspace::tripped() const {
    if (!flags.p || slots <= 0) return false;
    int v = 0;
    if (hipMemcpy(&v, (const int*)flags.p + slots - 1, 4, hipMemcpyDeviceToHost) != hipSuccess) return false;
    return v != 0;
}

void SkWorkspace::reset(hipStream_t s) {
    if (!flags.p || slots <= 0) return;
    (void)hipMemsetAsync(flags.p, 0, (size_t)slots * 4, s);
    (void)hipStreamSynchronize(s);
}

}
```

### text-to-speech-tts-onnx_amd/csrc/gemm_epilogue.h

```cpp
#pragma once
#include "common.h"
#include <type_traits>
#include "mfma.h"
#include "x3_split.h"
#include "wave_reduce.h"

namespace mi {

__device__ __forceinline__ float act_apply(float v, int act) {
    switch (act) {
        case ACT_GELU_TANH: {
            const float k0 = 0.7978845608028654f, k1 = 0.044715f;
            return 0.5f * v * (1.f + tanhf(k0 * (v + k1 * v * v * v)));
        }
        case ACT_GELU_ERF: return 0.5f * v * (1.f + erff(v * 0.7071067811865476f));
        case ACT_MISH: {
            float sp = v > 20.f ? v : log1pf(expf(v));
            return v * tanhf(sp);
        }
        case ACT_SILU: return v / (1.f + expf(-v));
        default: return v;
    }
}

struct ConvGemmDev {
    const void* x; const void* w; const float* bias; void* out; const void* res; const float* gate;
    long gate_bstride;
    int G, T_in, M, N, Cin, K, dil, pad;
    long x_bstride, x_rstride, out_bstride, out_rstride, x_goff;
    int act; float alpha; int accumulate; int epi;
    int u, Cout, padT, T_out;
    const float* rope_cos; const float* rope_sin; const void* rope_pack; int heads, head_dim; void* out2; void* out3;
    long v_ld; int Mb;
    int m_off = 0;
    const void* zero;
    int dbg;
    int lds_epi;
    int use_buf;
    int Tm, Tn, RT, RC;
    float* sk_ws; int* sk_flags; int sk_slots;
    const void* w3;
    const void* xp; const void* w3p; int np;
    void* out_planes;
    int kv_planes; long k_ld;
    int tail_tiles, tail_split;
    const float* ln_scale = nullptr; void* ln_out = nullptr; float* ln_stats_out = nullptr; int ln_out_np = 0;
    const float* ln_stats_in = nullptr; const float* ln_p = nullptr; const float* ln_c = nullptr; int ln_dim = 0; float ln_eps = 0.f;
    int ln_final = 0;
    int* sat = nullptr;
    const int* lens = nullptr; int len_mul = 1, len_add = 0;
};

__device__ __forceinline__ float gelu_tanh_fast(float v) {
    const float c0 = -2.0f * 0.7978845608028654f * 1.4426950408889634f;
    const float c1 = c0 * 0.044715f;
    const float u = v * v;
    const float e = __builtin_amdgcn_exp2f(v * __builtin_fmaf(c1, u, c0));
    return v * __builtin_amdgcn_rcpf(1.f + e);
}

template <int ACT, bool FAST = false>
__device__ __forceinline__ void act16(float (&v)[16]) {
    if constexpr (FAST && ACT == ACT_GELU_TANH) {
#pragma unroll
        for (int r = 0; r < 16; ++r) v[r] = gelu_tanh_fast(v[r]);
        return;
    }
#pragma unroll
    for (int q = 0; q < 4; ++q) {
#pragma unroll
        for (int r = 0; r < 4; ++r) v[q * 4 + r] = act_apply(v[q * 4 + r], ACT);
        __builtin_amdgcn_sched_barrier(0);
    }
}

template <typename TO, int TM, int TN, int WM, int WN, bool LENS = false>
__device__ __forceinline__ void gemm_epilogue(f32x16 (&acc)[TM][TN], const ConvGemmDev& p, int m0, int n0, int b, int g,
                                              int wm, int wn, int lr, int lk, int vb = 0) {
    if (!LENS && p.epi == EPI_QKV_ROPE) {
        const int dm = p.heads * p.head_dim;
#pragma unroll
        for (int j = 0; j < TN; ++j) {
            const int n = n0 + wn * WN + j * 32 + lr;
            const int which = n / dm;
            const int rem = n - which * dm;
            const int hh = rem / p.head_dim, dd = rem - hh * p.head_dim;
            const float bv = p.bias ? p.bias[n] : 0.f;
            const float sgn = (dd & 1) ? 1.f : -1.f;
            const bool vt = which == 2 && p.v_ld > 0;
            TO* base = (TO*)(which == 0 ? p.out : which == 1 ? p.out2 : p.out3);
            const long mstride = vt ? 1 : p.head_dim;
            const int Mb = p.Mb > 0 ? p.Mb : p.M;
            const long item_stride = vt ? (long)p.heads * p.head_dim * p.v_ld : (long)p.heads * Mb * p.head_dim;
            const long head_off = vt ? ((long)hh * p.head_dim + dd) * p.v_ld : (long)hh * Mb * p.head_dim + dd;
#pragma unroll
            for (int i = 0; i < TM; ++i) {
                const int mb = p.m_off + m0 + wm * WM + i * 32 + 4 * lk;
                const int bi0 = p.Mb > 0 ? mb / Mb : 0;
                const int mloc0 = mb - bi0 * Mb;
                TO* dst0 = base + ((long)b + bi0) * item_stride + head_off;
                TO* dst1 = dst0 + item_stride;
#pragma unroll
                for (int r = 0; r < 16; ++r) {
                    const int off = (r & 3) + 8 * (r >> 2);
                    const int mg = mb + off;
                    float v = acc[i][j][r] + bv;
                    const float partner = __shfl_xor(v, 1);
                    int m = mloc0 + off, bi = bi0;
                    if (m >= Mb) { m -= Mb; ++bi; }
                    if (mg - p.m_off >= p.M) { m = 0; bi = 0; }
                    const float c = which < 2 ? p.rope_cos[(long)m * p.head_dim + dd] : 1.f;
                    const float sn = which < 2 ? p.rope_sin[(long)m * p.head_dim + dd] : 0.f;
                    v = v * c + sgn * partner * sn;
                    if (mg - p.m_off < p.M) (bi == bi0 ? dst0 : dst1)[(long)m * mstride] = from_f32<TO>(v);
                }
                __builtin_amdgcn_sched_barrier(0);
            }
        }
        return;
    }
    TO* outp = (TO*)p.out + (long)b * p.out_bstride;
    const TO* resp = p.res ? (const TO*)p.res + (long)b * p.out_bstride : nullptr;
#pragma unroll
    for (int j = 0; j < TN; ++j) {
        const int n = n0 + wn * WN + j * 32 + lr;
        const bool nok = n < p.N;
        const int nc = nok ? n : 0;
        int col, ph = 0;
        if (p.epi == EPI_CONVT) { ph = nc / p.Cout; col = nc - ph * p.Cout; }
        else col = g * p.N + nc;
        const float bv = p.bias ? p.bias[col] : 0.f;
        const float gv = p.gate ? p.gate[(long)b * p.gate_bstride + col] : 1.f;
        int mlim = 0;
        if constexpr (LENS) mlim = p.epi == EPI_CONVT ? (vb + p.padT - ph + p.u - 1) / p.u : vb;
#pragma unroll
        for (int i = 0; i < TM; ++i) {
            const int mb = m0 + wm * WM + i * 32 + 4 * lk;
            float v[16];
            auto row_of = [&](int r, bool& o) -> long {
                const int m = mb + (r & 3) + 8 * (r >> 2);
                long row = m;
                o = nok && m < p.M;
                if (p.epi == EPI_CONVT) { row = (long)m * p.u + ph - p.padT; o = o && row >= 0 && row < p.T_out; }
                return (o ? row : 0) * p.out_rstride + col;
            };
            auto live = [&](int r) -> bool { return mb + (r & 3) + 8 * (r >> 2) < mlim; };
#pragma unroll
            for (int r = 0; r < 16; ++r) v[r] = acc[i][j][r] + bv;
            switch (p.act) {
                case ACT_GELU_TANH: act16<ACT_GELU_TANH, sizeof(TO) == 2>(v); break;
                case ACT_GELU_ERF: act16<ACT_GELU_ERF>(v); break;
                case ACT_MISH: act16<ACT_MISH>(v); break;
                case ACT_SILU: act16<ACT_SILU>(v); break;
                default: break;
            }
#pragma unroll
            for (int r = 0; r < 16; ++r) v[r] *= gv;
            if (resp) {
#pragma unroll
                for (int r = 0; r < 16; ++r) {
                    bool o; const long ix = row_of(r, o);
                    if constexpr (LENS) o = o && live(r);
                    v[r] += o ? to_f32(resp[ix]) : 0.f;
                }
            }
#pragma unroll
            for (int r = 0; r < 16; ++r) v[r] *= p.alpha;
            if (p.accumulate) {
#pragma unroll
                for (int r = 0; r < 16; ++r) {
                    bool o; const long ix = row_of(r, o);
                    if constexpr (LENS) o = o && live(r);
                    v[r] += o ? to_f32(outp[ix]) : 0.f;
                }
            }
            if constexpr (LENS) {
#pragma unroll
                for (int r = 0; r < 16; ++r) if (!live(r)) v[r] = 0.f;
            }
#pragma unroll
            for (int r = 0; r < 16; ++r) { bool o; const long ix = row_of(r, o); if (o) outp[ix] = from_f32<TO>(v[r]); }
            __builtin_amdgcn_sched_barrier(0);
        }
    }
}

__device__ __forceinline__ int gemm_live_rows(const ConvGemmDev& p, int b) {
    return __builtin_amdgcn_readfirstlane(p.lens[b] * p.len_mul + p.len_add);
}
__device__ __forceinline__ bool gemm_tile_dead(const ConvGemmDev& p, int m0, int vb) {
    return (p.epi == EPI_CONVT ? m0 * p.u - p.padT : m0) >= vb;
}

template <typename TO, int TM, int TN, int WM, int WN>
__device__ __forceinline__ void gemm_epilogue_lds(f32x16 (&acc)[TM][TN], const ConvGemmDev& p, int m0, int n0, int b, int g,
                                                  int wm, int wn, int lr, int lk, float* stage, int m_end = -1) {
    const int Mlim = m_end >= 0 ? m_end : p.M;
    constexpr int CH = sizeof(TO) == 2 ? 8 : 4;
    constexpr int LPR = WN / CH;
    constexpr int RPI = 64 / LPR;
    constexpr int RT = (WN <= 64 && TM % 2 == 0) ? 2 : 1;
    const int lane = lk * 32 + lr;
    TO* outp = (TO*)p.out + (long)b * p.out_bstride;
    const TO* resp = p.res ? (const TO*)p.res + (long)b * p.out_bstride : nullptr;
    const int cl = (lane % LPR) * CH, rl0 = lane / LPR;
    const int nchunk = n0 + wn * WN + cl;
    int ccol = g * p.N + nchunk, cph = 0;
    if (p.epi == EPI_CONVT) { cph = nchunk / p.Cout; ccol = nchunk - cph * p.Cout; }
    const bool cok = nchunk < p.N && lane < RPI * LPR;
#pragma unroll
    for (int i0 = 0; i0 < TM; i0 += RT) {
#pragma unroll
        for (int j = 0; j < TN; ++j) {
            const int n = n0 + wn * WN + j * 32 + lr;
            const int nc = n < p.N ? n : 0;
            const int col = p.epi == EPI_CONVT ? nc % p.Cout : g * p.N + nc;
            const float bv = p.bias ? p.bias[col] : 0.f;
            const float gv = p.gate ? p.gate[(long)b * p.gate_bstride + col] : 1.f;
#pragma unroll
            for (int ii = 0; ii < RT; ++ii) {
                float v[16];
#pragma unroll
                for (int r = 0; r < 16; ++r) v[r] = acc[i0 + ii][j][r] + bv;
                switch (p.act) {
                    case ACT_GELU_TANH: act16<ACT_GELU_TANH, sizeof(TO) == 2>(v); break;
                    case ACT_GELU_ERF: act16<ACT_GELU_ERF>(v); break;
                    case ACT_MISH: act16<ACT_MISH>(v); break;
                    case ACT_SILU: act16<ACT_SILU>(v); break;
                    default: break;
                }
#pragma unroll
                for (int r = 0; r < 16; ++r)
                    stage[(ii * 32 + (r & 3) + 8 * (r >> 2) + 4 * lk) * WN + j * 32 + lr] = v[r] * gv;
            }
        }
        __builtin_amdgcn_fence(__ATOMIC_RELEASE, "wavefront");
        __builtin_amdgcn_wave_barrier();
        constexpr int NIT = (RT * 32 + RPI - 1) / RPI, GRP = NIT % 4 == 0 ? 4 : (NIT % 2 == 0 ? 2 : 1);
        struct alignas(16) Pk { TO v[CH]; };
#pragma unroll
        for (int it0 = 0; it0 < NIT; it0 += GRP) {
            Pk rv[GRP], ov[GRP];
            long ixv[GRP];
            bool okv[GRP];
#pragma unroll
            for (int gi = 0; gi < GRP; ++gi) {
                const int rr = rl0 + (it0 + gi) * RPI;
                const int m = m0 + wm * WM + i0 * 32 + rr;
                long row = m;
                bool ok = cok && rr < RT * 32 && m < Mlim;
                if (p.epi == EPI_CONVT) { row = (long)m * p.u + cph - p.padT; ok = ok && row >= 0 && row < p.T_out; }
                okv[gi] = ok;
                ixv[gi] = ok ? row * p.out_rstride + ccol : 0;
            }
            if (resp) {
#pragma unroll
                for (int gi = 0; gi < GRP; ++gi) rv[gi] = *reinterpret_cast<const Pk*>(resp + ixv[gi]);
            }
            if (p.accumulate) {
#pragma unroll
                for (int gi = 0; gi < GRP; ++gi) ov[gi] = *reinterpret_cast<const Pk*>(outp + ixv[gi]);
            }
#pragma unroll
            for (int gi = 0; gi < GRP; ++gi) {
                const int rr = min(rl0 + (it0 + gi) * RPI, RT * 32 - 1);
                float x[CH];
#pragma unroll
                for (int q = 0; q < CH; q += 4) {
                    const float4 t = *reinterpret_cast<const float4*>(&stage[rr * WN + cl + q]);
                    x[q] = t.x; x[q + 1] = t.y; x[q + 2] = t.z; x[q + 3] = t.w;
                }
                if (resp) {
#pragma unroll
                    for (int q = 0; q < CH; ++q) x[q] += to_f32(rv[gi].v[q]);
                }
#pragma unroll
                for (int q = 0; q < CH; ++q) x[q] *= p.alpha;
                if (p.accumulate) {
#pragma unroll
                    for (int q = 0; q < CH; ++q) x[q] += to_f32(ov[gi].v[q]);
                }
                Pk o;
#pragma unroll
                for (int q = 0; q < CH; ++q) o.v[q] = from_f32<TO>(x[q]);
                if (okv[gi]) *reinterpret_cast<Pk*>(outp + ixv[gi]) = o;
            }
        }
        __builtin_amdgcn_fence(__ATOMIC_ACQUIRE, "wavefront");
        __builtin_amdgcn_wave_barrier();
    }
}


__device__ __forceinline__ void ln_rows32(const ConvGemmDev& p, long row0, long row_last, int lr, int lk, float& rstd, float& mrstd) {
    const int nb = p.ln_dim / LN_BLK;
    long row = row0 + lr;
    row = row < row_last ? row : row_last;
    if (p.ln_final) {
        const float2 t = reinterpret_cast<const float2*>(p.ln_stats_in)[row];
        rstd = t.x; mrstd = t.y;
        return;
    }
    const float* rowp = p.ln_stats_in + row * (long)(nb * 2);
    const float m0 = rowp[0] * (1.0f / 32.0f);
    const float4* sp = reinterpret_cast<const float4*>(rowp) + lk * (nb >> 2);
    LnMerge t;
    for (int i = 0; i < (nb >> 2); ++i) {
        const float4 v = sp[i];
        ln_merge_add(t, v.x, v.y, m0);
        ln_merge_add(t, v.z, v.w, m0);
    }
    LnMerge o;
    o.a = __shfl_xor(t.a, 32); o.b = __shfl_xor(t.b, 32); o.c = __shfl_xor(t.c, 32);
    if (lk) ln_merge_finish(o, t, m0, nb, p.ln_eps, rstd, mrstd);
    else ln_merge_finish(t, o, m0, nb, p.ln_eps, rstd, mrstd);
}

template <typename TO, int TMQ = 2, bool LN = false, bool PRE = false>
__device__ __forceinline__ void gemm_epilogue_qkv_lds(f32x16 (&acc)[TMQ][2], const ConvGemmDev& p, int m0, int n0, int b,
                                                      int wm, int wn, int lr, int lk, float* stage,
                                                      const float* pre_rs = nullptr, const float* pre_mr = nullptr, int m_end = -1) {
    const int Mlim = m_end >= 0 ? m_end : p.M;
    const int lane = lk * 32 + lr;
    const int dm = p.heads * 64;
    const int nbase = n0 + wn * 64;
    const int which = nbase / dm, hh = (nbase - which * dm) >> 6;
    const int Mb = p.Mb > 0 ? p.Mb : p.M;
    const int mrow = m0 + wm * (32 * TMQ);
    const int mbase = mrow + p.m_off;
    const int bi0 = mbase / Mb, mloc0 = mbase - bi0 * Mb;
    const bool vt = which == 2 && p.v_ld > 0;
    TO* base = (TO*)(which == 0 ? p.out : which == 1 ? p.out2 : p.out3);
    struct alignas(16) Pk { TO v[8]; };
    unsigned qkv_sat = 0;
    float ln_rs[TMQ], ln_mr[TMQ];
    if constexpr (LN) {
#pragma unroll
        for (int i = 0; i < TMQ; ++i) {
            if constexpr (PRE) { ln_rs[i] = pre_rs[i]; ln_mr[i] = pre_mr[i]; }
            else ln_rows32(p, (long)mbase + i * 32, (long)p.m_off + p.M - 1, lr, lk, ln_rs[i], ln_mr[i]);
        }
    }
    if (!vt) {
        float ln_pv[8], ln_cv[8];
        if constexpr (LN) {
            const int cc = nbase + (lane & 7) * 8;
            const float4 a0 = *reinterpret_cast<const float4*>(p.ln_p + cc), a1 = *reinterpret_cast<const float4*>(p.ln_p + cc + 4);
            const float4 b0 = *reinterpret_cast<const float4*>(p.ln_c + cc), b1 = *reinterpret_cast<const float4*>(p.ln_c + cc + 4);
            ln_pv[0] = a0.x; ln_pv[1] = a0.y; ln_pv[2] = a0.z; ln_pv[3] = a0.w; ln_pv[4] = a1.x; ln_pv[5] = a1.y; ln_pv[6] = a1.z; ln_pv[7] = a1.w;
            ln_cv[0] = b0.x; ln_cv[1] = b0.y; ln_cv[2] = b0.z; ln_cv[3] = b0.w; ln_cv[4] = b1.x; ln_cv[5] = b1.y; ln_cv[6] = b1.z; ln_cv[7] = b1.w;
        }
#pragma unroll
        for (int j = 0; j < 2; ++j) {
            const float bv = (!LN && p.bias) ? p.bias[nbase + j * 32 + lr] : 0.f;
#pragma unroll
            for (int i = 0; i < TMQ; ++i)
#pragma unroll
                for (int r = 0; r < 16; ++r)
                    stage[(i * 32 + (r & 3) + 8 * (r >> 2) + 4 * lk) * 64 + j * 32 + lr] = acc[i][j][r] + bv;
        }
        __builtin_amdgcn_fence(__ATOMIC_RELEASE, "wavefront");
        __builtin_amdgcn_wave_barrier();
        const int c8 = (lane & 7) * 8;
        struct alignas(16) H8 { f16 v[8]; };
        constexpr int GRP = 4;
#pragma unroll
        for (int it0 = 0; it0 < 4 * TMQ; it0 += GRP) {
            int mv[GRP], biv[GRP];
            bool okv[GRP];
            H8 cs[GRP];
#pragma unroll
            for (int gi = 0; gi < GRP; ++gi) {
                const int rr = (lane >> 3) + (it0 + gi) * 8;
                okv[gi] = mrow + rr < Mlim;
                int m = mloc0 + rr, bi = bi0;
                if (m >= Mb) { m -= Mb; ++bi; }
                if (!okv[gi]) { m = 0; bi = bi0; }
                mv[gi] = m; biv[gi] = bi;
            }
            if (which < 2 && p.rope_pack) {
#pragma unroll
                for (int gi = 0; gi < GRP; ++gi) cs[gi] = *reinterpret_cast<const H8*>((const f16*)p.rope_pack + (long)mv[gi] * 64 + c8);
            }
#pragma unroll
            for (int gi = 0; gi < GRP; ++gi) {
                const int rr = (lane >> 3) + (it0 + gi) * 8;
                float x[8];
#pragma unroll
                for (int q = 0; q < 8; q += 4) {
                    const float4 t = *reinterpret_cast<const float4*>(&stage[rr * 64 + c8 + q]);
                    x[q] = t.x; x[q + 1] = t.y; x[q + 2] = t.z; x[q + 3] = t.w;
                }
                if constexpr (LN) {
                    const float rs = __shfl(ln_rs[(it0 + gi) >> 2], rr & 31), mr = __shfl(ln_mr[(it0 + gi) >> 2], rr & 31);
#pragma unroll
                    for (int q = 0; q < 8; ++q) x[q] = __builtin_fmaf(rs, x[q], __builtin_fmaf(-mr, ln_pv[q], ln_cv[q]));
                }
                if (which < 2 && p.rope_pack) {
#pragma unroll
                    for (int q = 0; q < 8; q += 2) {
                        const float cc = (float)cs[gi].v[q], ss = (float)cs[gi].v[q + 1];
                        const float e = x[q], o = x[q + 1];
                        x[q] = e * cc - o * ss;
                        x[q + 1] = o * cc + e * ss;
                    }
                } else if (which < 2) {
                    float c[8], sn[8];
#pragma unroll
                    for (int q = 0; q < 8; q += 4) {
                        const float4 tc = *reinterpret_cast<const float4*>(p.rope_cos + (long)mv[gi] * 64 + c8 + q);
                        const float4 ts = *reinterpret_cast<const float4*>(p.rope_sin + (long)mv[gi] * 64 + c8 + q);
                        c[q] = tc.x; c[q + 1] = tc.y; c[q + 2] = tc.z; c[q + 3] = tc.w;
                        sn[q] = ts.x; sn[q + 1] = ts.y; sn[q + 2] = ts.z; sn[q + 3] = ts.w;
                    }
#pragma unroll
                    for (int q = 0; q < 8; q += 2) {
                        const float e = x[q], o = x[q + 1];
                        x[q] = e * c[q] - o * sn[q];
                        x[q + 1] = o * c[q + 1] + e * sn[q + 1];
                    }
                }
                if constexpr (sizeof(TO) == 4) if (p.kv_planes && which == 1) {
                    if (p.kv_planes == 2) {
                        x3_u4 pl[2];
                        {
                            unsigned wh[4], wl[4];
#pragma unroll
                            for (int q = 0; q < 4; ++q) x2u_split_pair(x[2 * q], x[2 * q + 1], wh[q], wl[q]);
                            pl[0] = x3_u4{wh[0], wh[1], wh[2], wh[3]}; pl[1] = x3_u4{wl[0], wl[1], wl[2], wl[3]};
                            qkv_sat |= x2_sat_word(wh[0]) | x2_sat_word(wh[1]) | x2_sat_word(wh[2]) | x2_sat_word(wh[3]);
                        }
                        bf16* kp = (bf16*)p.out2 + ((((long)b + biv[gi]) * p.heads + hh) * 2 * p.k_ld + mv[gi]) * 64 + c8;
                        if (okv[gi]) {
                            *reinterpret_cast<x3_u4*>(kp) = pl[0];
                            *reinterpret_cast<x3_u4*>(kp + p.k_ld * 64) = pl[1];
                        }
                        continue;
                    }
                    unsigned p1[4], p2[4], p3[4];
#pragma unroll
                    for (int q = 0; q < 4; ++q) x3_split_pair(x[2 * q], x[2 * q + 1], p1[q], p2[q], p3[q]);
                    bf16* kp = (bf16*)p.out2 + ((((long)b + biv[gi]) * p.heads + hh) * 3 * p.k_ld + mv[gi]) * 64 + c8;
                    if (okv[gi]) {
                        *reinterpret_cast<x3_u4*>(kp) = x3_u4{p1[0], p1[1], p1[2], p1[3]};
                        *reinterpret_cast<x3_u4*>(kp + p.k_ld * 64) = x3_u4{p2[0], p2[1], p2[2], p2[3]};
                        *reinterpret_cast<x3_u4*>(kp + 2 * p.k_ld * 64) = x3_u4{p3[0], p3[1], p3[2], p3[3]};
                    }
                    continue;
                }
                if constexpr (sizeof(TO) == 4) if (p.kv_planes == 2 && which == 0) {
#pragma unroll
                    for (int q = 0; q < 8; ++q) qkv_sat |= (fabsf(x[q]) * 1.4426950408889634f >= 65504.f || x[q] != x[q]) ? 1u : 0u;
                }
                Pk o8;
#pragma unroll
                for (int q = 0; q < 8; ++q) o8.v[q] = from_f32<TO>(x[q]);
                if (okv[gi]) *reinterpret_cast<Pk*>(base + (((long)b + biv[gi]) * p.heads + hh) * Mb * 64 + (long)mv[gi] * 64 + c8) = o8;
            }
        }
        __builtin_amdgcn_fence(__ATOMIC_ACQUIRE, "wavefront");
        __builtin_amdgcn_wave_barrier();
    } else {
        const int row = lane & 31, dh = lane >> 5;
        float ln_pl = 0.f, ln_cl = 0.f;
        if constexpr (LN) { ln_pl = p.ln_p[nbase + lane]; ln_cl = p.ln_c[nbase + lane]; }
#pragma unroll
        for (int i = 0; i < TMQ; ++i) {
#pragma unroll
            for (int j = 0; j < 2; ++j) {
                const float bv = (!LN && p.bias) ? p.bias[nbase + j * 32 + lr] : 0.f;
#pragma unroll
                for (int r = 0; r < 16; ++r)
                    stage[((r & 3) + 8 * (r >> 2) + 4 * lk) * 65 + j * 32 + lr] = acc[i][j][r] + bv;
            }
            auto vt_val = [&](int dd) __attribute__((always_inline)) -> float {
                const float a = stage[row * 65 + dd];
                if constexpr (LN) return __builtin_fmaf(ln_rs[i], a, __builtin_fmaf(-ln_mr[i], __shfl(ln_pl, dd), __shfl(ln_cl, dd)));
                else return a;
            };
            __builtin_amdgcn_fence(__ATOMIC_RELEASE, "wavefront");
            __builtin_amdgcn_wave_barrier();
            const int rr = i * 32 + row;
            const bool ok = mrow + rr < Mlim;
            int m = mloc0 + rr, bi = bi0;
            if (m >= Mb) { m -= Mb; ++bi; }
            TO* dst = base + (((long)b + bi) * p.heads + hh) * 64 * p.v_ld + m;
            if (sizeof(TO) == 4 && p.kv_planes) {
                const long pstride = 64 * p.v_ld;
                if (p.kv_planes == 2) {
                    unsigned short* vp = (unsigned short*)p.out3 + (((long)b + bi) * p.heads + hh) * 2 * 64 * p.v_ld + m;
#pragma unroll 8
                    for (int d = 0; d < 32; ++d) {
                        const int dd = dh * 32 + d;
                        unsigned ph, pl;
                        x2u_split_pair(vt_val(dd), 0.f, ph, pl);
                        qkv_sat |= x2_sat_word(ph);
                        if (ok) {
                            vp[(long)dd * p.v_ld] = (unsigned short)ph;
                            vp[pstride + (long)dd * p.v_ld] = (unsigned short)pl;
                        }
                    }
                } else {
                unsigned short* vp = (unsigned short*)p.out3 + (((long)b + bi) * p.heads + hh) * 3 * 64 * p.v_ld + m;
#pragma unroll 8
                for (int d = 0; d < 32; ++d) {
                    const int dd = dh * 32 + d;
                    unsigned p1, p2, p3;
                    x3_split_pair(vt_val(dd), 0.f, p1, p2, p3);
                    if (ok) {
                        vp[(long)dd * p.v_ld] = (unsigned short)p1;
                        vp[pstride + (long)dd * p.v_ld] = (unsigned short)p2;
                        vp[2 * pstride + (long)dd * p.v_ld] = (unsigned short)p3;
                    }
                }
                }
            } else {
#pragma unroll 8
                for (int d = 0; d < 32; ++d) {
                    const int dd = dh * 32 + d;
                    const float v = vt_val(dd);
                    if (ok) dst[(long)dd * p.v_ld] = from_f32<TO>(v);
                }
            }
            __builtin_amdgcn_fence(__ATOMIC_ACQUIRE, "wavefront");
            __builtin_amdgcn_wave_barrier();
        }
    }
    if constexpr (sizeof(TO) == 4) sat_publish(p.sat, qkv_sat);
}


template <typename TO> __device__ __forceinline__ void ln_act8(float (&x)[8], int act) {
    switch (act) {
        case ACT_GELU_TANH:
#pragma unroll
            for (int q = 0; q < 8; ++q) x[q] = gelu_tanh_fast(x[q]);
            break;
        case ACT_GELU_ERF:
#pragma unroll
            for (int q = 0; q < 8; ++q) x[q] = act_apply(x[q], ACT_GELU_ERF);
            break;
        case ACT_MISH:
#pragma unroll
            for (int q = 0; q < 8; ++q) x[q] = act_apply(x[q], ACT_MISH);
            break;
        case ACT_SILU:
#pragma unroll
            for (int q = 0; q < 8; ++q) x[q] = act_apply(x[q], ACT_SILU);
            break;
        default: break;
    }
}

template <typename TO, int TM, int TN, int NP, bool PRE = false>
__device__ __forceinline__ void gemm_epilogue_ln_in(f32x16 (&acc)[TM][TN], const ConvGemmDev& p, int mw, int nc0, int lr, int lk, float* stage,
                                                    const float* pre_rs = nullptr, const float* pre_mr = nullptr, int m_end = -1) {
    const int Mlim = m_end >= 0 ? m_end : p.M;
    constexpr int WN = 32 * TN, LPR = WN / 8, RPI = 64 / LPR, NIT = 32 / RPI;
    const int lane = lk * 32 + lr;
    const int c8 = (lane % LPR) * 8, rl0 = lane / LPR;
    const int col = nc0 + c8;
    float pv[8], cv[8];
    {
        const float4 a0 = *reinterpret_cast<const float4*>(p.ln_p + col), a1 = *reinterpret_cast<const float4*>(p.ln_p + col + 4);
        const float4 b0 = *reinterpret_cast<const float4*>(p.ln_c + col), b1 = *reinterpret_cast<const float4*>(p.ln_c + col + 4);
        pv[0] = a0.x; pv[1] = a0.y; pv[2] = a0.z; pv[3] = a0.w; pv[4] = a1.x; pv[5] = a1.y; pv[6] = a1.z; pv[7] = a1.w;
        cv[0] = b0.x; cv[1] = b0.y; cv[2] = b0.z; cv[3] = b0.w; cv[4] = b1.x; cv[5] = b1.y; cv[6] = b1.z; cv[7] = b1.w;
    }
    unsigned sat = 0;
    struct alignas(16) Pk { TO v[8]; };
    float rs_all[TM], mr_all[TM];
#pragma unroll
    for (int i = 0; i < TM; ++i) {
        if constexpr (PRE) { rs_all[i] = pre_rs[i]; mr_all[i] = pre_mr[i]; }
        else ln_rows32(p, (long)mw + i * 32, (long)p.M - 1, lr, lk, rs_all[i], mr_all[i]);
    }
#pragma unroll
    for (int i = 0; i < TM; ++i) {
        const float rstd = rs_all[i], mrstd = mr_all[i];
#pragma unroll
        for (int j = 0; j < TN; ++j)
#pragma unroll
            for (int r = 0; r < 16; ++r) stage[((r & 3) + 8 * (r >> 2) + 4 * lk) * WN + j * 32 + lr] = acc[i][j][r];
        __builtin_amdgcn_fence(__ATOMIC_RELEASE, "wavefront");
        __builtin_amdgcn_wave_barrier();
#pragma unroll
        for (int it = 0; it < NIT; ++it) {
            const int rr = rl0 + it * RPI;
            const int m = mw + i * 32 + rr;
            const float rs = __shfl(rstd, rr), mr = __shfl(mrstd, rr);
            const float4 t0 = *reinterpret_cast<const float4*>(&stage[rr * WN + c8]);
            const float4 t1 = *reinterpret_cast<const float4*>(&stage[rr * WN + c8 + 4]);
            float x[8] = {t0.x, t0.y, t0.z, t0.w, t1.x, t1.y, t1.z, t1.w};
#pragma unroll
            for (int q = 0; q < 8; ++q) x[q] = __builtin_fmaf(rs, x[q], __builtin_fmaf(-mr, pv[q], cv[q]));
// ... 167 lines not shown
```

### text-to-speech-tts-onnx_amd/csrc/options.h

```cpp
#pragma once
#include <atomic>
#include <shared_mutex>

namespace mi {

#define MI_OPTIONS(X)                                                                                                   \
                                   \
    X(GEMM_BIG_TILE_MIN, "gemm_big_tile_min", "MI355TTS_BIG_TILE_MIN", ENV_INT, 160, STORE, 0, 0)                       \
    X(GEMM_N192_MIN, "gemm_n192_min", nullptr, ENV_INT, 160, STORE, 0, 0)                                               \
    X(GEMM_MID_TILE_MIN, "gemm_mid_tile_min", nullptr, ENV_INT, 160, STORE, 0, 0)                                       \
    X(GEMM_DMA3_K_MIN, "gemm_dma3_k_min", "MI355TTS_DMA3_K_MIN", ENV_INT, 2048, STORE, 0, 0)                            \
    X(GEMM_USE_DMA3, "gemm_use_dma3", "MI355TTS_NO_DMA3_GEMM", ENV_ONE_OFF, 1, BOOL, 0, 1)                              \
    X(GEMM_USE_DMA, "gemm_use_dma", "MI355TTS_NO_DMA_GEMM", ENV_ONE_OFF, 1, BOOL, 0, 1)                                 \
    X(GEMM_BIG_TILES, "gemm_big_tiles", "MI355TTS_NO_BIG_TILES", ENV_ONE_OFF, 1, BOOL, 0, 1)                            \
    X(GEMM_N192, "gemm_n192", "MI355TTS_NO_N192", ENV_ONE_OFF, 1, BOOL, 0, 1)                                           \
    X(GEMM_F32_DMA, "gemm_f32_dma", nullptr, ENV_INT, 1, BOOL, 0, 1)                                                    \
    X(GEMM_RING4, "gemm_ring4", "MI355TTS_NO_RING4", ENV_ONE_OFF, 1, BOOL, 0, 1)                                        \
    X(GEMM_RING4_MAX, "gemm_ring4_max", "MI355TTS_RING4_MAX", ENV_INT, 256, STORE, 0, 0)                                \
    X(GEMM_BUF, "gemm_buf", "MI355TTS_NO_BUF", ENV_ONE_OFF, 1, BOOL, 0, 1)                                              \
    X(GEMM_F32_SMALL, "gemm_f32_small", "MI355TTS_NO_F32_SMALL", ENV_ONE_OFF, 1, BOOL, 0, 1)                            \
    X(GEMM_F32_SMALL_MAX, "gemm_f32_small_max", "MI355TTS_F32_SMALL_MAX", ENV_INT, 1024, STORE, 0, 0)                   \
    X(GEMM_SMALL16_MAX, "gemm_small16_max", "MI355TTS_SMALL16_MAX", ENV_INT, 256, STORE, 0, 0)                          \
    X(GEMM_F32_N64_DMA, nullptr, "MI355TTS_F32_N64_DMA", ENV_INT, 1, STORE, 0, 0)                                       \
    X(GEMM_N64_DMA16, nullptr, "MI355TTS_N64_DMA16", ENV_INT, 0, STORE, 0, 0)  \
    X(GEMM_XCD_ORDER, nullptr, "MI355TTS_XCD_ORDER", ENV_ONE_ON, 0, BOOL, 0, 1)                                         \
    X(GEMM_LDS_EPI, nullptr, "MI355TTS_NO_LDS_EPI", ENV_ONE_OFF, 1, BOOL, 0, 1)                                         \
    X(GEMM_ROW_SPLIT, "gemm_row_split", nullptr, ENV_INT, 1, STORE, 0, 0)  \
     \
    X(GEMM_SK, "gemm_sk", "MI355TTS_SK", ENV_INT, 1, STORE, 0, 0)                                                       \
    X(GEMM_SK_STAGES, "gemm_sk_stages", "MI355TTS_SK_STAGES", ENV_INT, 0, STORE, 0, 0)                                  \
    X(GEMM_SK_ORDER, nullptr, "MI355TTS_SK_ORDER", ENV_INT, -1, STORE, 0, 0)                                            \
     \
     \
    X(GEMM_SK_QKV32, nullptr, "MI355TTS_SK_QKV32", ENV_INT, 0, STORE, 0, 0)                                             \
     \
    X(GEMM_F32_X3, "gemm_f32_x3", "MI355TTS_F32_X3", ENV_INT, 1, STORE, 0, 0)                                           \
    X(GEMM_F32_X3P, "gemm_f32_x3p", "MI355TTS_F32_X3P", ENV_INT, 1, STORE, 0, 0)                                        \
    X(GEMM_F32_PLANES, "gemm_f32_planes", "MI355TTS_F32_PLANES", ENV_INT, 2, REJECT, 2, 3)  \
    X(GEMM_F32_N64_PAIRS, "gemm_f32_n64_pairs", nullptr, ENV_INT, 1, STORE, 0, 0)  \
    X(GEMM_F32_GCONV, "gemm_f32_gconv", nullptr, ENV_INT, 1, STORE, 0, 0)  \
    X(GEMM_X3P_NOALIGN, "gemm_x3p_noalign", "MI355TTS_X3P_NOALIGN", ENV_INT, 0, STORE, 0, 0)  \
    X(GEMM_X3P_GRID, "gemm_x3p_grid", "MI355TTS_X3P_GRID", ENV_INT, 0, STORE, 0, 0)  \
    X(GEMM_X3D, "gemm_x3d", "MI355TTS_X3D", ENV_INT, 1, STORE, 0, 0)                            \
    X(GEMM_X3D_MIN_EFF, "gemm_x3d_min_eff", "MI355TTS_X3D_MIN_EFF", ENV_INT, 90, STORE, 0, 0)  \
       \
    X(GEMM_PH8, "gemm_ph8", "MI355TTS_PH8", ENV_INT, 1, STORE, 0, 0)                                                    \
    X(GEMM_PH8_MIN_TILES, "gemm_ph8_min_tiles", "MI355TTS_PH8_MIN", ENV_INT, 200, STORE, 0, 0)                          \
    X(GEMM_PH8_ORDER, "gemm_ph8_order", "MI355TTS_PH8_ORDER", ENV_INT, 1, STORE, 0, 0)                                  \
     \
    X(GEMM_PH8_SPLIT_MAX, "gemm_ph8_split_max", "MI355TTS_PH8_SPLIT", ENV_INT, 2, CLAMP, 1, 4)                          \
    X(GEMM_PH8_SPLIT_MIN_NK, "gemm_ph8_split_min_nk", nullptr, ENV_INT, 24, STORE, 0, 0)                                \
                                                                            \
    X(GCONV_TWO_TAPS, "gconv_two_taps", "MI355TTS_GCONV2", ENV_ZERO_OFF, 1, BOOL, 0, 1)                                 \
    X(GCONV16, "gconv16", "MI355TTS_GCONV16", ENV_ZERO_OFF, 1, BOOL, 0, 1)                                              \
                                                                                         \
    X(ATTN_F32_X3, "attn_f32_x3", "MI355TTS_ATTN_X3", ENV_INT, 2, CLAMP, 0, 2)                                          \
    X(ATTN_F32_PLANES, "attn_f32_planes", "MI355TTS_ATTN_PLANES", ENV_INT, 2, REJECT, 2, 3)  \
    X(ATTN_SPLIT, "attn_split", "MI355TTS_ATTN_NO_SPLIT", ENV_ONE_OFF, 2, CLAMP, 0, 2)  \
    X(ATTN_XCD_MAP, "attn_xcd_map", nullptr, ENV_INT, 1, BOOL, 0, 1)  \
    X(ATTN_KV_PLANES, "attn_kv_planes", "MI355TTS_ATTN_KVP", ENV_INT, 1, BOOL, 0, 1)  \
    X(ATTN_LPT, "attn_lpt", "MI355TTS_ATTN_LPT", ENV_INT, 1, BOOL, 0, 1)  \
    X(ATTN_Z_FORCE, "attn_z_force", nullptr, ENV_INT, 0, CLAMP, 0, 4)  \
            \
    X(ATTN_Z, nullptr, "MI355TTS_ATTN_Z", ENV_INT, 4, CLAMP, 1, 4)                                                      \
    X(ATTN_Z16, nullptr, "MI355TTS_ATTN_Z16", ENV_INT, 1, CLAMP, 1, 4)                                                  \
    X(ATTN_CUTS, nullptr, "MI355TTS_ATTN_CUTS", ENV_CUTS, 0, STORE, 0, 0)  \
                                                                                              \
    X(GPT_MFMA_MIN, "gpt_mfma_min", nullptr, ENV_INT, 9, STORE, 0, 0)  \
    X(GPT_MFMA, nullptr, "MI355TTS_GPT_NO_MFMA", ENV_ONE_OFF, 1, BOOL, 0, 1)                                            \
                                                                    \
    X(BIGVGAN_STREAMS, "bigvgan_streams", nullptr, ENV_INT, 3, CLAMP, 1, 3)                                             \
    X(BV_SYNC, nullptr, "MI355TTS_BV_SYNC", ENV_ONE_ON, 0, BOOL, 0, 1)                                                  \
    X(AA_TILE, nullptr, "MI355TTS_AA_TILE", ENV_INT, 8192, STORE, 0, 0)    \
    X(AA_PIPE, nullptr, "MI355TTS_AA_PIPE", ENV_ZERO_OFF, 1, BOOL, 0, 1)                                                \
    X(AA_R, nullptr, "MI355TTS_AA_R", ENV_INT, 16, STORE, 0, 0)  \
    X(AACONV_LDS_MIN, nullptr, "MI355TTS_AACONV_LDS_MIN", ENV_INT, 0, STORE, 0, 0)

#define MI_OPT_ENUM(name, key, env, conv, dflt, policy, lo, hi) OPT_##name,
enum Opt : int { MI_OPTIONS(MI_OPT_ENUM) OPT_COUNT };

extern std::atomic<long> g_opt[OPT_COUNT];
static inline long opt(Opt o) { return g_opt[o].load(std::memory_order_relaxed); }

void options_init();
bool options_set(const char* key, long v);
bool options_get(const char* key, long* v);
struct AttnCuts { int n = 0; int c[3] = {0, 0, 0}; };
const AttnCuts& opt_attn_cuts();

long env_int(const char* name, long dflt);
bool env_first_is(const char* name, char c);

long option_epoch();
void option_epoch_bump();
std::shared_mutex& option_lock();
}
```

Measured before the change: 40.99.

## Store pre-split V planes row-major and read them with LDS transpose loads

The QKV GEMM epilogue now writes the V bf16/f16 planes key-major (same layout as K) instead of transposed. The attention kernel stages them into swizzled LDS rows and builds the PV MFMA operand with ds_read_b64_tr_b16 transpose reads. This removes the transposed V write in the epilogue and the padded column layout. It relies on the gfx950 transpose-read instruction and inline asm waits. The softmax exp loop is also rewritten from paired-vector to scalar form with asm barriers, and the path is on by default behind a new option.

```diff
diff --git a/text-to-speech-tts-onnx_amd/csrc/attention.hip b/text-to-speech-tts-onnx_amd/csrc/attention.hip
--- a/text-to-speech-tts-onnx_amd/csrc/attention.hip
+++ b/text-to-speech-tts-onnx_amd/csrc/attention.hip
@@ -402,6 +402,35 @@
     }
 }
 
+typedef unsigned attn_u2 __attribute__((ext_vector_type(2)));
+__device__ __forceinline__ unsigned attn_lds_addr(const void* p) {
+    return (unsigned)(unsigned long)(const __attribute__((address_space(3))) void*)p;
+}
+template <int OFF> __device__ __forceinline__ void attn_lds_rd64_tr16(attn_u2& d, unsigned a) {
+#if defined(__HIP_DEVICE_COMPILE__)
+    asm volatile("ds_read_b64_tr_b16 %0, %1 offset:%2" : "=v"(d) : "v"(a), "n"(OFF) : "memory");
+#endif
+}
+__device__ __forceinline__ void attn_tr_wait() {
+#if defined(__HIP_DEVICE_COMPILE__)
+    asm volatile("s_waitcnt lgkmcnt(0)" ::: "memory");
+#endif
+}
+__device__ __forceinline__ void attn_tr_use(attn_u2& d) {
+#if defined(__HIP_DEVICE_COMPILE__)
+    asm volatile("" : "+v"(d));
+#endif
+}
+template <int N, int I = 0, typename F> __device__ __forceinline__ void attn_unroll(F&& f) {
+    if constexpr (I < N) { f(std::integral_constant<int, I>{}); attn_unroll<N, I + 1>(f); }
+}
+template <int NP, int PLB, int S2> __device__ __forceinline__ void attn_v_tr_read(attn_u2 (&t)[2][NP][2], unsigned a0, unsigned a1) {
+    attn_unroll<NP>([&](auto PL) {
+        constexpr int pl = NP - 1 - decltype(PL)::value, o = pl * PLB + S2 * 16 * 128;
+        attn_lds_rd64_tr16<o>(t[0][pl][0], a0); attn_lds_rd64_tr16<o + 8 * 128>(t[0][pl][1], a0);
+        attn_lds_rd64_tr16<o>(t[1][pl][0], a1); attn_lds_rd64_tr16<o + 8 * 128>(t[1][pl][1], a1);
+    });
+}
 #if defined(MI355TTS_ATTN_TRACE)
 #define TSTAMP(v) do { __builtin_amdgcn_sched_barrier(0); asm volatile("s_memtime %0\n\ts_waitcnt lgkmcnt(0)" : "=s"(v) :: "memory"); __builtin_amdgcn_sched_barrier(0); } while (0)
 #define TACC(k, t1, t0) tr_[k] += (t1) - (t0)
@@ -409,7 +438,7 @@
 #define TSTAMP(v) do { } while (0)
 #define TACC(k, t1, t0) do { } while (0)
 #endif
-template <bool SPLIT2, bool KVP = false, int NP = 3, bool VARLEN = false>
+template <bool SPLIT2, bool KVP = false, int NP = 3, bool VARLEN = false, bool VROWS = false>
 __global__ __launch_bounds__(256, NP == 2 ? 3 : 2) void attn_x3f_kernel(const float* __restrict__ q, const float* __restrict__ k,
                                                        const float* __restrict__ v, float* __restrict__ o, int H, int N,
                                                        float* __restrict__ ws, int* __restrict__ cnt,
@@ -417,11 +446,13 @@
                                                        int cut1 = 0, int cut2 = 0, int cut3 = 0, const int* __restrict__ lens = nullptr) {
     ATTN_XCD_MAP
     static_assert(NP == 3 || (NP == 2 && KVP), "attn_x3f: the two-plane form reads pre-split K / V");
+    static_assert(!VROWS || KVP, "attn_x3f: V as rows is a layout of the pre-split planes");
     using MF = std::conditional_t<NP == 3, Mfma<bf16>, Mfma<f16>>;
     using Frag = typename MF::Frag;
     constexpr int D = 64, KT = 64;
-    constexpr int LDK = D + 8, LDV = KT + 4;
-    constexpr int KPL = KT * LDK, VPL = D * LDV;
+    constexpr int LDK = D + 8, LDV = VROWS ? D : KT + 4;
+    constexpr int KPL = KT * LDK, VPL = VROWS ? KT * LDV : D * LDV;
+    static_assert((NP * KPL * 2) % 16 == 0 && (VPL * 2) % 16 == 0, "attn_x3f: 16-byte aligned V planes");
     __shared__ __attribute__((aligned(16))) bf16 smem[NP * KPL + NP * VPL];
     static_assert(sizeof(smem) >= (2 * 32 * 64 + 2 * 64 * 2 + 4) * sizeof(float), "merge buffer fits the stage");
     bf16* Ks = smem;
@@ -491,9 +522,14 @@
             for (int i = 0; i < NU; ++i) {
                 const int u = tid + i * 256, pl = u >> 9, r = (u & 511) >> 3, c = u & 7;
                 kpl[i] = *reinterpret_cast<const x3_u4*>(kpb + ((long)pl * vld + key0 + r) * D + c * 8);
-                vpl[i] = *reinterpret_cast<const x3_u4*>(vpb + ((long)pl * D + r) * vld + key0 + c * 8);
-            }
-            if (key0 + KT > NL) {
+                if constexpr (VROWS) vpl[i] = *reinterpret_cast<const x3_u4*>(vpb + ((long)pl * vld + key0 + r) * D + c * 8);
+                else vpl[i] = *reinterpret_cast<const x3_u4*>(vpb + ((long)pl * D + r) * vld + key0 + c * 8);
+            }
+            if (VROWS && key0 + KT > NL) {
+#pragma unroll
+                for (int i = 0; i < NU; ++i)
+                    if (key0 + (((tid + i * 256) & 511) >> 3) >= NL) vpl[i] = x3_u4{0u, 0u, 0u, 0u};
+            } else if (key0 + KT > NL) {
 #pragma unroll
                 for (int i = 0; i < NU; ++i) {
                     const int keep = NL - (key0 + ((tid + i * 256) & 7) * 8);
@@ -530,8 +566,12 @@
             for (int i = 0; i < NU; ++i) {
                 const int u = tid + i * 256, pl = u >> 9, r = (u & 511) >> 3, c = u & 7;
                 *reinterpret_cast<x3_u4*>(Ks + pl * KPL + r * LDK + c * 8) = kpl[i];
+                if constexpr (VROWS) {
+                    *reinterpret_cast<x3_u4*>(Vs + pl * VPL + r * LDV + ((c ^ ((r & 2) << 1)) * 8)) = vpl[i];
+                } else {
                 uint2* vd = reinterpret_cast<uint2*>(Vs + pl * VPL + r * LDV + c * 8);
                 vd[0] = uint2{vpl[i].x, vpl[i].y}; vd[1] = uint2{vpl[i].z, vpl[i].w};
+                }
             }
         } else {
 #pragma unroll
@@ -551,6 +591,13 @@
         }
     };
 
+    unsigned vtr[2] = {0u, 0u};
+    if constexpr (VROWS) {
+        const int q4 = (lane >> 2) & 3;
+        const unsigned a = attn_lds_addr(Vs) + (4 * hi + q4) * (LDV * 2) + ((lane >> 4) & 1) * 32 + (lane & 3) * 8;
+        vtr[0] = a + (q4 >> 1) * 64;
+        vtr[1] = a + ((q4 >> 1) ^ 1) * 64;
+    }
     f32x16 oacc[2];
 #pragma unroll
     for (int r = 0; r < 16; ++r) { oacc[0][r] = 0.f; oacc[1][r] = 0.f; }
@@ -621,18 +668,17 @@
 #pragma unroll
                 for (int r = 0; r < 16; ++r) { oacc[0][r] *= alpha; oacc[1][r] *= alpha; }
             }
-            typedef float f2 __attribute__((ext_vector_type(2)));
             float p[16];
-            f2 ls2 = f2{0.f, 0.f};
-            const f2 m2 = f2{m_run, m_run};
+            float ls0 = 0.f, ls1 = 0.f;
 #pragma unroll
             for (int r = 0; r < 16; r += 2) {
-                const f2 dd = f2{sacc[r], sacc[r + 1]} - m2;
-                const f2 e = f2{__builtin_amdgcn_exp2f(dd.x), __builtin_amdgcn_exp2f(dd.y)};
-                p[r] = e.x; p[r + 1] = e.y;
-                ls2 += e;
-            }
-            float lsum = ls2.x + ls2.y;
+                float d0 = sacc[r] - m_run, d1 = sacc[r + 1] - m_run;
+                asm("" : "+v"(d0)); asm("" : "+v"(d1));
+                p[r] = __builtin_amdgcn_exp2f(d0); p[r + 1] = __builtin_amdgcn_exp2f(d1);
+                ls0 += p[r]; ls1 += p[r + 1];
+                asm("" : "+v"(ls0)); asm("" : "+v"(ls1));
+            }
+            float lsum = ls0 + ls1;
             lsum = xor32_sum(lsum);
             l_run = l_run * alpha + lsum;
 #if defined(MI355TTS_ATTN_TRACE)
@@ -649,6 +695,19 @@
                     split8p(float4{p[8 * s2], p[8 * s2 + 1], p[8 * s2 + 2], p[8 * s2 + 3]},
                             float4{p[8 * s2 + 4], p[8 * s2 + 5], p[8 * s2 + 6], p[8 * s2 + 7]}, pf[0], pf[1]);
                 Frag vf[2][NP];
+                if constexpr (VROWS) {
+                    attn_u2 t[2][NP][2];
+                    const unsigned a0 = vtr[0] + kt * (32 * LDV * 2), a1 = vtr[1] + kt * (32 * LDV * 2);
+                    if (s2 == 0) attn_v_tr_read<NP, VPL * 2, 0>(t, a0, a1); else attn_v_tr_read<NP, VPL * 2, 1>(t, a0, a1);
+                    attn_tr_wait();
+#pragma unroll
+                    for (int dt = 0; dt < 2; ++dt)
+#pragma unroll
+                        for (int pl = 0; pl < NP; ++pl) {
+                            attn_tr_use(t[dt][pl][0]); attn_tr_use(t[dt][pl][1]);
+                            vf[dt][pl] = __builtin_bit_cast(Frag, x3_u4{t[dt][pl][0].x, t[dt][pl][0].y, t[dt][pl][1].x, t[dt][pl][1].y});
+                        }
+                } else {
 #pragma unroll
                 for (int dt = 0; dt < 2; ++dt)
 #pragma unroll
@@ -659,6 +718,7 @@
                         a2[1] = *reinterpret_cast<const uint2*>(row + 8);
                         vf[dt][pl] = __builtin_bit_cast(Frag, x3_u4{a2[0].x, a2[0].y, a2[1].x, a2[1].y});
                     }
+                }
                 if constexpr (NP == 3) {
 #pragma unroll
                     for (int t = 0; t < 6; ++t)
@@ -848,6 +908,7 @@
 }
 
 int attention_kv_planes_format() { return opt_attn_np(); }
+bool attention_kv_v_rows() { return opt(OPT_ATTN_V_ROWS) != 0; }
 
 bool attention_can_write_planes(int N, int BH, int dtype) {
     (void)N; (void)BH;
@@ -902,9 +963,17 @@
 
 template <bool SPLIT2, bool KVP, int NP>
 static void go_x3f(dim3 grid, hipStream_t s, const void* q, const void* k, const void* v, void* o, int H, int N, float* ws, int* cnt,
-                   void* o_planes, int o_np, int xm, int c1, int c2, int c3, const int* lens) {
+                   void* o_planes, int o_np, int xm, int c1, int c2, int c3, const int* lens, bool v_rows) {
     const float *qf = (const float*)q, *kf = (const float*)k, *vf = (const float*)v;
     if (lens) prof_kernel_suffix(" + lengths");
+    if constexpr (KVP) {
+        if (v_rows) {
+            if (lens) hipLaunchKernelGGL((attn_x3f_kernel<SPLIT2, KVP, NP, true, true>), grid, dim3(256), 0, s, qf, kf, vf, (float*)o, H, N, ws, cnt, (unsigned char*)o_planes, o_np, xm, c1, c2, c3, lens);
+            else hipLaunchKernelGGL((attn_x3f_kernel<SPLIT2, KVP, NP, false, true>), grid, dim3(256), 0, s, qf, kf, vf, (float*)o, H, N, ws, cnt, (unsigned char*)o_planes, o_np, xm, c1, c2, c3);
+            return;
+        }
+    }
+    MI_REQUIRE(!v_rows, "attention: V as rows is a layout of the pre-split planes");
     if (lens) hipLaunchKernelGGL((attn_x3f_kernel<SPLIT2, KVP, NP, true>), grid, dim3(256), 0, s, qf, kf, vf, (float*)o, H, N, ws, cnt, (unsigned char*)o_planes, o_np, xm, c1, c2, c3, lens);
     else hipLaunchKernelGGL((attn_x3f_kernel<SPLIT2, KVP, NP>), grid, dim3(256), 0, s, qf, kf, vf, (float*)o, H, N, ws, cnt, (unsigned char*)o_planes, o_np, xm, c1, c2, c3);
 }
@@ -919,7 +988,8 @@
 
 void launch_attention(const void* q, const void* k, const void* v, void* o, int BH, int H, int N, int dtype, hipStream_t s,
                       float* ws, long ws_floats, int* cnt, long cnt_n, void* o_planes, int kv_planes, int o_np, float ref_fp16_scale,
-                      const int* lens) {
+                      const int* lens, int v_rows) {
+    MI_REQUIRE(!v_rows || kv_planes, "attention: V as rows comes with pre-split K / V");
     MI_REQUIRE(ref_fp16_scale == 0.f || (dtype == MI_F16 && ref_fp16_scale > 0.f), "attention: the reference-fp16 score form needs f16 operands");
     MI_REQUIRE(o_np == 2 || o_np == 3, "attention: 2 or 3 output planes");
     MI_REQUIRE(!o_planes || attention_can_write_planes(N, BH, dtype), "attention: panel-plane output needs the fp32 split kernel");
@@ -994,17 +1064,17 @@
                 }
                 prof_set_kernel("attn_x3f_kernel<false, pre-split K V, fp16 pairs> + key slices", "", "");
                 go_x3f<false, true, 2>(dim3((N + 127) / 128, BH, sl.Z), s, q, k, v, o, H, N, ws, cnt, o_planes, o_np, xm,
-                                       sl.Z > 1 ? sl.cut[0] : 0, sl.cut[1], sl.cut[2], lens);
+                                       sl.Z > 1 ? sl.cut[0] : 0, sl.cut[1], sl.cut[2], lens, v_rows != 0);
             } else if (opt_attn_x3() == 2) {
                 if (kv_planes == 2) {
                     prof_set_kernel("attn_x3f_kernel<true, pre-split K V, fp16 pairs>", "", "");
-                    go_x3f<true, true, 2>(dim3((N + 63) / 64, BH, Z), s, q, k, v, o, H, N, ws, cnt, o_planes, o_np, xm, 0, 0, 0, lens);
+                    go_x3f<true, true, 2>(dim3((N + 63) / 64, BH, Z), s, q, k, v, o, H, N, ws, cnt, o_planes, o_np, xm, 0, 0, 0, lens, v_rows != 0);
                 } else if (kv_planes) {
                     prof_set_kernel("attn_x3f_kernel<true, pre-split K V>", "", "");
-                    go_x3f<true, true, 3>(dim3((N + 63) / 64, BH, Z), s, q, k, v, o, H, N, ws, cnt, o_planes, o_np, 0, 0, 0, 0, lens);
+                    go_x3f<true, true, 3>(dim3((N + 63) / 64, BH, Z), s, q, k, v, o, H, N, ws, cnt, o_planes, o_np, 0, 0, 0, 0, lens, v_rows != 0);
                 } else {
                 prof_set_kernel("attn_x3f_kernel<true>", "", "");
-                go_x3f<true, false, 3>(dim3((N + 63) / 64, BH, Z), s, q, k, v, o, H, N, ws, cnt, o_planes, o_np, 0, 0, 0, 0, lens);
+                go_x3f<true, false, 3>(dim3((N + 63) / 64, BH, Z), s, q, k, v, o, H, N, ws, cnt, o_planes, o_np, 0, 0, 0, 0, lens, v_rows != 0);
                 }
             } else if (opt_attn_x3() == 1) {
                 prof_set_kernel("attn_kernel<float, true, x3>", "", "");
@@ -1014,13 +1084,13 @@
         } else if (opt_attn_x3() == 2) {
             if (kv_planes == 2) {
                 prof_set_kernel("attn_x3f_kernel<false, pre-split K V, fp16 pairs>", "", "");
-                go_x3f<false, true, 2>(dim3((N + 127) / 128, BH), s, q, k, v, o, H, N, ws, cnt, o_planes, o_np, xm, 0, 0, 0, lens);
+                go_x3f<false, true, 2>(dim3((N + 127) / 128, BH), s, q, k, v, o, H, N, ws, cnt, o_planes, o_np, xm, 0, 0, 0, lens, v_rows != 0);
             } else if (kv_planes) {
                 prof_set_kernel("attn_x3f_kernel<false, pre-split K V>", "", "");
-                go_x3f<false, true, 3>(dim3((N + 127) / 128, BH), s, q, k, v, o, H, N, ws, cnt, o_planes, o_np, 0, 0, 0, 0, lens);
+                go_x3f<false, true, 3>(dim3((N + 127) / 128, BH), s, q, k, v, o, H, N, ws, cnt, o_planes, o_np, 0, 0, 0, 0, lens, v_rows != 0);
             } else {
             prof_set_kernel("attn_x3f_kernel<false>", "", "");
-            go_x3f<false, false, 3>(dim3((N + 127) / 128, BH), s, q, k, v, o, H, N, ws, cnt, o_planes, o_np, 0, 0, 0, 0, lens);
+            go_x3f<false, false, 3>(dim3((N + 127) / 128, BH), s, q, k, v, o, H, N, ws, cnt, o_planes, o_np, 0, 0, 0, 0, lens, v_rows != 0);
             }
         } else if (opt_attn_x3() == 1) {
             prof_set_kernel("attn_kernel<float, false, x3>", "", "");
diff --git a/text-to-speech-tts-onnx_amd/csrc/capi.hip b/text-to-speech-tts-onnx_amd/csrc/capi.hip
--- a/text-to-speech-tts-onnx_amd/csrc/capi.hip
+++ b/text-to-speech-tts-onnx_amd/csrc/capi.hip
@@ -297,6 +297,7 @@
         if (k == "f32_arithmetic") v = e.dtype != MI_F32 ? -1 : !gemm_x3_enabled() ? ARITH_NATIVE : (gemm_x3p_enabled() ? e.np : ARITH_BF16X3);
         else if (k == "saturation_events") v = e.sat_events;
         else if (k == "adaln_fold") v = (e.fold_built && e.cfg.ln_fold != 0) ? 1 : 0;
+        else if (k == "attn_v_rows") v = (e.dtype == MI_F32 && attention_takes_kv_planes(0, 0, MI_F32) && attention_kv_v_rows()) ? 1 : 0;
         else MI_REQUIRE(false, "mi_f5_info: unknown key");
     });
     return rc == MI_OK ? v : (int64_t)rc;
diff --git a/text-to-speech-tts-onnx_amd/csrc/common.h b/text-to-speech-tts-onnx_amd/csrc/common.h
--- a/text-to-speech-tts-onnx_amd/csrc/common.h
+++ b/text-to-speech-tts-onnx_amd/csrc/common.h
@@ -132,6 +132,7 @@
     int m_off = 0;
     long v_ld = 0;
     int kv_planes = 0; long k_ld = 0;
+    int v_rows = 0;
     float* sk_ws = nullptr; int* sk_flags = nullptr; int sk_slots = 0;
     const void* w3 = nullptr;
     const void* xp = nullptr; const void* w3p = nullptr; int np = 3;
diff --git a/text-to-speech-tts-onnx_amd/csrc/f5.hip b/text-to-speech-tts-onnx_amd/csrc/f5.hip
--- a/text-to-speech-tts-onnx_amd/csrc/f5.hip
+++ b/text-to-speech-tts-onnx_amd/csrc/f5.hip
@@ -701,6 +701,7 @@
         return g;
     };
     const int kvp_fmt = attention_kv_planes_format();
+    const int v_rows = attention_kv_v_rows() ? 1 : 0;
     bool planes = false, fold = false;
     {
         const Block& b0 = blocks[0];
@@ -740,11 +741,11 @@
                 g.x = Ub.p; g.bias = nullptr;
                 if (f32) with_planes(g, bk.qkv, ApN.p);
                 consume(g); g.ln_p = lt; g.ln_c = lt + 3 * d;
-                if (kvp) { g.kv_planes = kvp_fmt; g.k_ld = g.v_ld = (long)((N + 63) / 64 * 64); }
+                if (kvp) { g.kv_planes = kvp_fmt; g.k_ld = g.v_ld = (long)((N + 63) / 64 * 64); g.v_rows = v_rows; }
                 launch_conv_gemm(g, s);
             }
             launch_attention(qb.p, kb.p, vb.p, Ob.p, B * H, H, N, dtype, s, attn_ws.as<float>(), attn_ws_floats, attn_cnt.as<int>(), attn_cnt_n,
-                             f32 ? Ap.p : nullptr, kvp ? kvp_fmt : 0, np, cfg.score_scale != 1.f ? cfg.score_scale : 0.f, lens);
+                             f32 ? Ap.p : nullptr, kvp ? kvp_fmt : 0, np, cfg.score_scale != 1.f ? cfg.score_scale : 0.f, lens, kvp ? v_rows : 0);
             {
                 ConvGemm g = lin(bk.o, d, MI_F32, X.p);
                 g.x = Ob.p; g.res = X.p; g.gate = m + 2 * d;
@@ -778,12 +779,12 @@
             {
                 ConvGemm g = qkv_gemm(bk);
                 g.x = Ub.p; with_planes(g, bk.qkv, Ap.p);
-                if (kvp) { g.kv_planes = kvp_fmt; g.k_ld = g.v_ld = (long)((N + 63) / 64 * 64); }
+                if (kvp) { g.kv_planes = kvp_fmt; g.k_ld = g.v_ld = (long)((N + 63) / 64 * 64); g.v_rows = v_rows; }
                 MI_REQUIRE(gemm_x3p_would_run(g), "f5: the QKV layer left the panel-plane kernel between the decision and the launch");
                 launch_conv_gemm(g, s);
             }
             launch_attention(qb.p, kb.p, vb.p, Ob.p, B * H, H, N, dtype, s, attn_ws.as<float>(), attn_ws_floats, attn_cnt.as<int>(), attn_cnt_n,
-                             Ap.p, kvp ? kvp_fmt : 0, np, 0.f, lens);
+                             Ap.p, kvp ? kvp_fmt : 0, np, 0.f, lens, kvp ? v_rows : 0);
             {
                 ConvGemm g = lin(bk.o, d, MI_F32, X.p);
                 g.x = Ob.p; g.res = X.p; g.gate = m + 2 * d; with_planes(g, bk.o, Ap.p);
diff --git a/text-to-speech-tts-onnx_amd/csrc/f5_kernels.h b/text-to-speech-tts-onnx_amd/csrc/f5_kernels.h
--- a/text-to-speech-tts-onnx_amd/csrc/f5_kernels.h
+++ b/text-to-speech-tts-onnx_amd/csrc/f5_kernels.h
@@ -37,8 +37,9 @@
 
 void launch_attention(const void* q, const void* k, const void* v, void* o, int BH, int H, int N, int dtype, hipStream_t s,
                       float* ws = nullptr, long ws_floats = 0, int* cnt = nullptr, long cnt_n = 0, void* o_planes = nullptr,
-                      int kv_planes = 0, int o_np = 3, float ref_fp16_scale = 0.f, const int* lens = nullptr);
+                      int kv_planes = 0, int o_np = 3, float ref_fp16_scale = 0.f, const int* lens = nullptr, int v_rows = 0);
 bool attention_takes_kv_planes(int N, int BH, int dtype);
+bool attention_kv_v_rows();
 int attention_kv_planes_format();
 bool attention_can_write_planes(int N, int BH, int dtype);
 long attention_v_ld(int N, int dtype);
diff --git a/text-to-speech-tts-onnx_amd/csrc/gemm_conv.hip b/text-to-speech-tts-onnx_amd/csrc/gemm_conv.hip
--- a/text-to-speech-tts-onnx_amd/csrc/gemm_conv.hip
+++ b/text-to-speech-tts-onnx_amd/csrc/gemm_conv.hip
@@ -777,7 +777,7 @@
     d.rope_cos = p.rope_cos; d.rope_sin = p.rope_sin; d.rope_pack = p.rope_pack; d.heads = p.heads; d.head_dim = p.head_dim;
     d.out2 = p.out2; d.out3 = p.out3; d.v_ld = p.v_ld; d.Mb = p.rows_per_item; d.m_off = p.m_off;
     MI_REQUIRE(p.m_off == 0 || (p.epi == EPI_QKV_ROPE && p.rows_per_item >= 32), "conv_gemm: a row offset needs the flattened QKV epilogue");
-    d.kv_planes = p.kv_planes; d.k_ld = p.k_ld;
+    d.kv_planes = p.kv_planes; d.k_ld = p.k_ld; d.v_rows = p.kv_planes ? p.v_rows : 0;
     d.sk_ws = p.sk_ws; d.sk_flags = p.sk_flags; d.sk_slots = p.sk_slots;
     const bool use_x3p = x3p_eligible(p);
     const bool use_x3 = use_x3p || x3_eligible(p);
@@ -829,7 +829,7 @@
     if (p.ln_stats_in || p.ln_stats_out)
         MI_REQUIRE(d.lds_epi && (p.dtype != MI_F32 || use_x3p), "conv_gemm: the AdaLN fold lives in the LDS-staged epilogues of linear_x3p / linear_ph8 / conv_gemm_dma (gemm_ln_fold_ok)");
     if (p.kv_planes) MI_REQUIRE(p.epi == EPI_QKV_ROPE && p.dtype == MI_F32 && d.lds_epi && p.v_ld > 0 && p.k_ld > 0 && p.v_ld % 8 == 0,
-                                "conv_gemm: kv_planes needs the fp32 LDS-staged QKV epilogue with transposed V");
+                                "conv_gemm: kv_planes needs the fp32 LDS-staged QKV epilogue and the padded key axes k_ld / v_ld");
     if (p.epi == EPI_CONVT) MI_REQUIRE(p.Cout > 0 && p.N == p.u * p.Cout, "conv_gemm: convT shape");
     if (p.epi == EPI_QKV_ROPE)
         MI_REQUIRE((p.rows_per_item == 0 || p.rows_per_item >= 32) && p.G == 1 && p.heads > 0 && p.head_dim % 2 == 0 && p.N == 3 * p.heads * p.head_dim && p.N % 32 == 0 &&
diff --git a/text-to-speech-tts-onnx_amd/csrc/gemm_epilogue.h b/text-to-speech-tts-onnx_amd/csrc/gemm_epilogue.h
--- a/text-to-speech-tts-onnx_amd/csrc/gemm_epilogue.h
+++ b/text-to-speech-tts-onnx_amd/csrc/gemm_epilogue.h
@@ -43,6 +43,7 @@
     const void* xp; const void* w3p; int np;
     void* out_planes;
     int kv_planes; long k_ld;
+    int v_rows;
     int tail_tiles, tail_split;
     const float* ln_scale = nullptr; void* ln_out = nullptr; float* ln_stats_out = nullptr; int ln_out_np = 0;
     const float* ln_stats_in = nullptr; const float* ln_p = nullptr; const float* ln_c = nullptr; int ln_dim = 0; float ln_eps = 0.f;
@@ -329,7 +330,8 @@
     const int mrow = m0 + wm * (32 * TMQ);
     const int mbase = mrow + p.m_off;
     const int bi0 = mbase / Mb, mloc0 = mbase - bi0 * Mb;
-    const bool vt = which == 2 && p.v_ld > 0;
+    const bool vrow = sizeof(TO) == 4 && p.kv_planes && p.v_rows && which == 2;
+    const bool vt = which == 2 && p.v_ld > 0 && !vrow;
     TO* base = (TO*)(which == 0 ? p.out : which == 1 ? p.out2 : p.out3);
     struct alignas(16) Pk { TO v[8]; };
     unsigned qkv_sat = 0;
@@ -420,7 +422,8 @@
                         x[q + 1] = o * c[q + 1] + e * sn[q + 1];
                     }
                 }
-                if constexpr (sizeof(TO) == 4) if (p.kv_planes && which == 1) {
+                if constexpr (sizeof(TO) == 4) if (p.kv_planes && (which == 1 || vrow)) {
+                    bf16* kvo = (bf16*)(which == 1 ? p.out2 : p.out3);
                     if (p.kv_planes == 2) {
                         x3_u4 pl[2];
                         {
@@ -430,7 +433,7 @@
                             pl[0] = x3_u4{wh[0], wh[1], wh[2], wh[3]}; pl[1] = x3_u4{wl[0], wl[1], wl[2], wl[3]};
                             qkv_sat |= x2_sat_word(wh[0]) | x2_sat_word(wh[1]) | x2_sat_word(wh[2]) | x2_sat_word(wh[3]);
                         }
-                        bf16* kp = (bf16*)p.out2 + ((((long)b + biv[gi]) * p.heads + hh) * 2 * p.k_ld + mv[gi]) * 64 + c8;
+                        bf16* kp = kvo + ((((long)b + biv[gi]) * p.heads + hh) * 2 * p.k_ld + mv[gi]) * 64 + c8;
                         if (okv[gi]) {
                             *reinterpret_cast<x3_u4*>(kp) = pl[0];
                             *reinterpret_cast<x3_u4*>(kp + p.k_ld * 64) = pl[1];
@@ -440,7 +443,7 @@
                     unsigned p1[4], p2[4], p3[4];
 #pragma unroll
                     for (int q = 0; q < 4; ++q) x3_split_pair(x[2 * q], x[2 * q + 1], p1[q], p2[q], p3[q]);
-                    bf16* kp = (bf16*)p.out2 + ((((long)b + biv[gi]) * p.heads + hh) * 3 * p.k_ld + mv[gi]) * 64 + c8;
+                    bf16* kp = kvo + ((((long)b + biv[gi]) * p.heads + hh) * 3 * p.k_ld + mv[gi]) * 64 + c8;
                     if (okv[gi]) {
                         *reinterpret_cast<x3_u4*>(kp) = x3_u4{p1[0], p1[1], p1[2], p1[3]};
                         *reinterpret_cast<x3_u4*>(kp + p.k_ld * 64) = x3_u4{p2[0], p2[1], p2[2], p2[3]};
diff --git a/text-to-speech-tts-onnx_amd/csrc/options.h b/text-to-speech-tts-onnx_amd/csrc/options.h
--- a/text-to-speech-tts-onnx_amd/csrc/options.h
+++ b/text-to-speech-tts-onnx_amd/csrc/options.h
@@ -59,6 +59,7 @@
     X(ATTN_SPLIT, "attn_split", "MI355TTS_ATTN_NO_SPLIT", ENV_ONE_OFF, 2, CLAMP, 0, 2)  \
     X(ATTN_XCD_MAP, "attn_xcd_map", nullptr, ENV_INT, 1, BOOL, 0, 1)  \
     X(ATTN_KV_PLANES, "attn_kv_planes", "MI355TTS_ATTN_KVP", ENV_INT, 1, BOOL, 0, 1)  \
+    X(ATTN_V_ROWS, nullptr, "MI355TTS_ATTN_V_ROWS", ENV_ZERO_OFF, 1, BOOL, 0, 1)  \
     X(ATTN_LPT, "attn_lpt", "MI355TTS_ATTN_LPT", ENV_INT, 1, BOOL, 0, 1)  \
     X(ATTN_Z_FORCE, "attn_z_force", nullptr, ENV_INT, 0, CLAMP, 0, 4)  \
             \
```

New measurement: 41.85 (median of 6 runs). 1.02x the previous value.
